# kangxiongbin/HyLight

Hardware: AMD Instinct MI355X
Metric: long-read all-vs-all overlaps/sec (higher is better)
Workload: dtype u8/int32

## Files before the change

hylight_amd/csrc/ava_align.hip:

```cpp
#include <algorithm>
#include <memory>
#include <type_traits>

#include "ava_internal.h"
#include "dev_prims.h"
#include "wave_ops.h"

namespace hlmi {

namespace {
constexpr int WG = 256;
constexpr int WAVES = WG / 64;
constexpr int SEQ_T_MAX = EXT_MAX + BAND_W;
constexpr int NR_SHORT = 128;
constexpr int WIDE_SHORT = 128;
inline dim3 grid1(size_t n) { return grid_for(n, WG); }

struct Task {
    uint32_t piece;
    uint16_t kind;
    uint16_t narrow;
    uint64_t qa, ta;
    int16_t m, n;
    int16_t dlo;
    int16_t trim;
};
constexpr uint16_t TASK_REV = 4;
constexpr uint16_t TASK_ONE = 8;
struct TaskOut {
    int32_t score;
    int32_t bi, bj;
    uint32_t runs_off, n_runs;
    uint32_t pad;
};
__device__ __forceinline__ uint32_t end_codes(uint32_t first_run, uint32_t last_run) { return (first_run & 15u) | (last_run & 15u) << 4; }

__global__ void piece_task_count_kernel(const Piece *pieces, size_t n, uint32_t *cnt) {
    size_t i = blockIdx.x * (size_t)blockDim.x + threadIdx.x;
    if (i < n) cnt[i] = pieces[i].n_fp + 1;
}

struct TaskRef { uint32_t pk, fp; };
struct PieceGeom {
    uint64_t qo, to;
    uint32_t ql, tl;
    uint32_t strand;
    uint32_t stub_cand;
};
struct TaskGeom {
    const TaskRef *ref;
    const PieceGeom *pg;
    const FixPt *fps;
};
__device__ __forceinline__ Task build_task(const PieceGeom &p, uint32_t piece, uint32_t kind, FixPt f0, FixPt f1, int ext_max) {
    const int ql = (int)p.ql, tl = (int)p.tl;
    const uint64_t qo = p.qo, to = p.to;
    const uint16_t rev = p.strand ? TASK_REV : 0;
    auto qaddr = [&](int pos) { return p.strand ? qo + (uint64_t)(ql - 1 - pos) : qo + (uint64_t)pos; };
    if (kind == 1) {
        const int qs = (int)f0.q, ts = (int)f0.t;
        const int m = qs < ext_max ? qs : ext_max, n2 = ts < m + BAND_W ? ts : m + BAND_W;
        return Task{piece, (uint16_t)(1u | rev), (uint16_t)(qs <= ext_max ? (qs + 1) << 1 : 0), qaddr(qs - 1),
                    to + (uint64_t)(ts - 1), (int16_t)m, (int16_t)n2, (int16_t)(-(BAND_W / 2 - 1)), 0};
    }
    if (kind == 2) {
        const int qe = (int)f0.q, te = (int)f0.t;
        const int m = ql - qe < ext_max ? ql - qe : ext_max, n2 = tl - te < m + BAND_W ? tl - te : m + BAND_W;
        return Task{piece, (uint16_t)(2u | rev), (uint16_t)(ql - qe <= ext_max ? (ql - qe + 1) << 1 : 0), qaddr(qe),
                    to + (uint64_t)te, (int16_t)m, (int16_t)n2, (int16_t)(-(BAND_W / 2 - 1)), 0};
    }
    const int q0 = (int)f0.q, t0 = (int)f0.t, m = (int)f1.q - q0, n2 = (int)f1.t - t0;
    const int delta = n2 - m, ad = delta < 0 ? -delta : delta;
    const bool lng = m > BLOCK_MAX || n2 > BLOCK_MAX;
    const bool narrow = !lng && ad <= NARROW_DELTA;
    const int lw = ad <= HALF_DELTA ? HALF_W : BAND_W;
    return Task{piece, rev, (uint16_t)(narrow ? 1 : 0), qaddr(q0), to + (uint64_t)t0, (int16_t)m, (int16_t)n2,
                (int16_t)((delta < 0 ? delta : 0) - (narrow ? NARROW_PAD : lng ? (lw - 1 - ad) / 2 : BAND_PAD)), 0};
}
__global__ __launch_bounds__(WG) void task_ref_kernel(const Piece *pieces, const uint32_t *task_off, size_t n, const uint32_t *qlen,
                                                       const uint32_t *tlen, const uint64_t *qoff, const uint64_t *toff,
                                                       const FixPt *fps, int stub_oh, int ext_max, TaskRef *task_ref, PieceGeom *pg) {
    const int lane = threadIdx.x & 63;
    const size_t wave = (blockIdx.x * (size_t)blockDim.x + threadIdx.x) >> 6;
    const size_t n_waves = ((size_t)gridDim.x * blockDim.x) >> 6;
    for (size_t i = wave; i < n; i += n_waves) {
        const Piece p = pieces[i];
        const uint32_t n_tasks = p.n_fp + 1;
        TaskRef *out = task_ref + task_off[i];
        for (uint32_t k = (uint32_t)lane; k < n_tasks; k += 64) {
            const uint32_t kind = k == 0 ? 1u : (k == p.n_fp ? 2u : 0u);
            out[k] = TaskRef{(uint32_t)i | kind << 30, p.fp_off + (k == 0 ? 0u : k - 1)};
        }
        if (lane == 0) {
            const uint32_t ql = qlen[p.q], tl = tlen[p.t];
            uint32_t cand = 0;
            if (stub_oh >= 0) {
                const FixPt a = fps[p.fp_off], b = fps[p.fp_off + p.n_fp - 1];
                const uint32_t dq = (uint32_t)(ext_max + stub_oh), dt = (uint32_t)(ext_max + BAND_W + stub_oh);
                cand = ((a.q > dq && a.t > dt) || (ql - b.q > dq && tl - b.t > dt)) ? 1u : 0u;
            }
            pg[i] = PieceGeom{qoff[p.q], toff[p.t], ql, tl, p.strand, cand};
        }
    }
}

__global__ __launch_bounds__(WG) void task_ref_lane_kernel(const Piece *pieces, const uint32_t *task_off, size_t n, const uint32_t *qlen,
                                                            const uint32_t *tlen, const uint64_t *qoff, const uint64_t *toff,
                                                            const FixPt *fps, int stub_oh, int ext_max, TaskRef *task_ref, PieceGeom *pg) {
    const size_t i = blockIdx.x * (size_t)blockDim.x + threadIdx.x;
    if (i >= n) return;
    const Piece p = pieces[i];
    const uint32_t n_tasks = p.n_fp + 1;
    TaskRef *out = task_ref + task_off[i];
    for (uint32_t k = 0; k < n_tasks; ++k) {
        const uint32_t kind = k == 0 ? 1u : (k == p.n_fp ? 2u : 0u);
        out[k] = TaskRef{(uint32_t)i | kind << 30, p.fp_off + (k == 0 ? 0u : k - 1)};
    }
    const uint32_t ql = qlen[p.q], tl = tlen[p.t];
    uint32_t cand = 0;
    if (stub_oh >= 0) {
        const FixPt a = fps[p.fp_off], b = fps[p.fp_off + p.n_fp - 1];
        const uint32_t dq = (uint32_t)(ext_max + stub_oh), dt = (uint32_t)(ext_max + BAND_W + stub_oh);
        cand = ((a.q > dq && a.t > dt) || (ql - b.q > dq && tl - b.t > dt)) ? 1u : 0u;
    }
    pg[i] = PieceGeom{qoff[p.q], toff[p.t], ql, tl, p.strand, cand};
}

struct AlignArgs {
    Task *tasks;
    TaskGeom geom;
    size_t n_tasks;
    const uint32_t *list;
    size_t n_list;
    const uint8_t *qcodes, *tcodes;
    long long q_total, t_total;
    const uint8_t *qpacked, *tpacked;
    const uint32_t *qnflag, *tnflag;
    int match, mismatch, go, ge, ambi;
    int go2, ge2;
    int end_bonus;
    int ext_max;
    int ext_all_long;
    int ungapped;
    int kmax;
    int kgap1;
    int kgap2;
    int one_ok;
    int kext_plain;
    int kext_bonus;
    int trim_ok;
    int kshift;
    TaskOut *out;
    uint32_t *runs;
    uint32_t cap_runs;
    uint32_t *counters;
    uint32_t run_buf_cap;
    uint8_t *cls_bare;
    uint8_t *defer_flag;
    const uint32_t *defer_list, *defer_count;
};

__device__ __forceinline__ uint32_t wave_excl_sum_u32(uint32_t v, int lane, uint32_t &total) {
    (void)lane;
    const uint32_t x = wave_prefix_sum_incl_dpp(v);
    total = (uint32_t)__builtin_amdgcn_readlane((int)x, 63);
    return x - v;
}

constexpr uint32_t RUN_CHUNK = 4096;
constexpr uint32_t RUN_CHUNK_SMALL = 256;
__device__ __forceinline__ uint32_t pool_take(const AlignArgs &a, uint32_t n, uint32_t &chunk_off, uint32_t &chunk_left,
                                              bool &ok, uint32_t chunk = RUN_CHUNK) {
    if (n > chunk_left) {
        const uint32_t want = n > chunk ? n : chunk;
        chunk_off = atomicAdd(&a.counters[0], want);
        chunk_left = want;
        if ((unsigned long long)chunk_off + want > a.cap_runs) { a.counters[1] = 1; chunk_left = 0; ok = false; return 0; }
    }
    const uint32_t off = chunk_off;
    chunk_off += n;
    chunk_left -= n;
    return off;
}

__device__ __forceinline__ uint32_t load_codes4(const uint8_t *base, long long idx, long long total) {
    if (idx >= 0 && idx + 4 <= total) {
        uint32_t v;
        __builtin_memcpy(&v, base + idx, 4);
        return v;
    }
    uint32_t v = 0;
    for (int k = 0; k < 4; ++k) v |= (uint32_t)(idx + k >= 0 && idx + k < total ? base[idx + k] : 4) << (8 * k);
    return v;
}
__device__ __forceinline__ uint32_t comp_codes4(uint32_t x) {
    const uint32_t n = x & 0x04040404u;
    return (x ^ 0x03030303u) & ~((n >> 1) | (n >> 2));
}
__device__ __forceinline__ uint32_t load_window4(const uint8_t *codes, long long total, long long a0, bool down, bool comp, int x) {
    uint32_t v = down ? __builtin_bswap32(load_codes4(codes, a0 - x - 3, total)) : load_codes4(codes, a0 + x, total);
    if (comp) v = comp_codes4(v);
    return v;
}

__device__ __forceinline__ uint32_t load_window4p(const uint8_t *codes, long long a0, bool down, bool comp, int x) {
    uint32_t v;
    __builtin_memcpy(&v, codes + (down ? a0 - x - 3 : a0 + x), 4);
    if (down) v = __builtin_bswap32(v);
    if (comp) v = comp_codes4(v);
    return v;
}


enum { ST_BASES = 0, ST_BASES_SQUARE, ST_BASES_NARROW, ST_BASES_WIDE, ST_FAST, ST_DP, ST_DP_ROWS, ST_NARROW_SMALL, ST_WIDE_ONE, ST_STUB_EXT, ST_EXT_CERT, ST_EXT_DP_ROW, ST_EXT_DP_K, ST_LONG, ST_BASES_LONG, ST_PACKED, N_ALIGN_STATS };
constexpr int NR_SMALL = 64;
constexpr uint8_t CLS_LONG = 5;
constexpr uint8_t CLS_LONG32 = 7;
constexpr uint8_t CLS_UNGAPPED = 6;

__device__ __forceinline__ uint64_t load_codes8(const uint8_t *base, long long idx, long long total) {
    if (idx >= 0 && idx + 8 <= total) {
        uint64_t v;
        __builtin_memcpy(&v, base + idx, 8);
        return v;
    }
    uint64_t v = 0;
    for (int k = 0; k < 8; ++k) v |= (uint64_t)(idx + k >= 0 && idx + k < total ? base[idx + k] : 4) << (8 * k);
    return v;
}
__device__ __forceinline__ uint64_t load_window8(const uint8_t *codes, long long total, long long a0, bool down, bool comp, int x) {
    uint64_t v = down ? __builtin_bswap64(load_codes8(codes, a0 - x - 7, total)) : load_codes8(codes, a0 + x, total);
    if (comp) {
        const uint64_t n = v & 0x0404040404040404ull;
        v = (v ^ 0x0303030303030303ull) & ~((n >> 1) | (n >> 2));
    }
    return v;
}

__device__ __forceinline__ uint64_t load_window8p(const uint8_t *codes, long long a0, bool down, bool comp, int x) {
    uint64_t v;
    __builtin_memcpy(&v, codes + (down ? a0 - x - 7 : a0 + x), 8);
    if (down) v = __builtin_bswap64(v);
    if (comp) {
        const uint64_t n = v & 0x0404040404040404ull;
        v = (v ^ 0x0303030303030303ull) & ~((n >> 1) | (n >> 2));
    }
    return v;
}

__device__ __forceinline__ uint64_t load_window32p(const uint8_t *packed, long long a0, bool down, bool comp, int x) {
    const long long s = down ? a0 - x - 31 : a0 + x;
    const uint8_t *p = packed + (s >> 2);
    uint64_t lo;
    __builtin_memcpy(&lo, p, 8);
    const int sh = 2 * (int)(s & 3);
    uint64_t v = lo >> sh | (uint64_t)p[8] << 1 << (63 - sh);
    if (down) {
        v = __builtin_bitreverse64(v);
        v = (v >> 1 & 0x5555555555555555ull) | (v & 0x5555555555555555ull) << 1;
    }
    return comp ? ~v : v;
}
__device__ __forceinline__ uint32_t ne_bits32(uint64_t q, uint64_t t) {
    const uint64_t d = q ^ t;
    auto even = [](uint32_t x) {
        x = (x | x >> 1) & 0x55555555u;
        x = (x | x >> 1) & 0x33333333u;
        x = (x | x >> 2) & 0x0f0f0f0fu;
        x = (x | x >> 4) & 0x00ff00ffu;
        return (x | x >> 8) & 0xffffu;
    };
    return even((uint32_t)d) | even((uint32_t)(d >> 32)) << 16;
}
__device__ __forceinline__ uint32_t squeeze8(uint64_t f) {
    return (((uint32_t)f * 0x10204080u) >> 28) | (((uint32_t)(f >> 32) * 0x10204080u) >> 28) << 4;
}
__device__ __forceinline__ uint32_t ne_bits8(uint64_t q, uint64_t t) {
    const uint64_t d = q ^ t;
    return squeeze8((d | d >> 1 | d >> 2) & 0x0101010101010101ull);
}
__device__ __forceinline__ uint32_t amb_bits8(uint64_t q, uint64_t t) { return squeeze8((q | t) >> 2 & 0x0101010101010101ull); }
__device__ __forceinline__ bool range_flagged(const uint32_t *nflag, long long lo, long long hi) {
    const uint32_t g0 = (uint32_t)((lo + (long long)DevReads::PAD) >> 5), g1 = (uint32_t)((hi + (long long)DevReads::PAD) >> 5);
    uint32_t any = 0;
    for (uint32_t w = g0 >> 5; w <= g1 >> 5; ++w) {
        uint32_t keep = ~0u;
        if (w == g0 >> 5) keep &= ~0u << (g0 & 31);
        if (w == g1 >> 5) keep &= ~0u >> (31 - (g1 & 31));
        any |= nflag[w] & keep;
    }
    return any != 0;
}
__device__ __forceinline__ bool window_flagged(const uint32_t *nflag, long long a0, bool down, int len) {
    return down ? range_flagged(nflag, a0 - (len - 1), a0) : range_flagged(nflag, a0, a0 + (len - 1));
}

template <int PASS>
__global__ __launch_bounds__(WG) __attribute__((amdgpu_waves_per_eu(PASS == 1 ? 4 : 5))) void classify_kernel(AlignArgs a, uint8_t *cls, unsigned long long *stats) {
    __shared__ unsigned long long s_stat[WAVES][N_ALIGN_STATS];
    constexpr int CMP_WORDS = PASS == 1 ? 64 * (BLOCK_MAX / 32) : 1;
    __shared__ uint32_t s_mm[WAVES][CMP_WORDS], s_up[WAVES][CMP_WORDS], s_dn[WAVES][CMP_WORDS];
    __shared__ uint64_t s_qa[WAVES][PASS == 1 ? 64 : 1], s_ta[WAVES][PASS == 1 ? 64 : 1];
    __shared__ uint32_t s_geo[WAVES][PASS == 1 ? 64 : 1], s_amb[WAVES][2];
    const int lane = threadIdx.x & 63;
    const size_t tid = blockIdx.x * (size_t)blockDim.x + threadIdx.x;
    const size_t n_thr = (size_t)gridDim.x * blockDim.x;
    uint32_t chunk_off = 0, chunk_left = 0;
    uint32_t st[N_ALIGN_STATS] = {};
    const size_t n_units = PASS == 1 ? a.n_tasks : (size_t)*a.defer_count;
    const size_t rounds = (n_units + n_thr - 1) / n_thr;
    TaskRef ref_n{0, 0};
    uint32_t ti_n = 0;
    if (PASS == 1) { if (tid < n_units) ref_n = a.geom.ref[tid]; }
    else if (tid < n_units) ti_n = a.defer_list[tid];
    for (size_t r = 0; r < rounds; ++r) {
        const size_t u = r * n_thr + tid;
        bool live = u < n_units;
        const size_t ti = PASS == 1 || !live ? u : (size_t)ti_n;
        TaskRef ref = ref_n;
        if (PASS == 2 && live) ref = a.geom.ref[ti];
        {
            const size_t un = u + n_thr;
            if (PASS == 1) { if (un < n_units) ref_n = a.geom.ref[un]; }
            else if (un < n_units) ti_n = a.defer_list[un];
        }
        Task tk{};
        bool held = false;
        bool bare = false;
        if (live) {
            const uint32_t pc = ref.pk & 0x3fffffffu, kind = ref.pk >> 30;
            const PieceGeom pg = a.geom.pg[pc];
            held = PASS == 1 && kind != 0 && pg.stub_cand != 0;
            bare = a.cls_bare != nullptr && pg.stub_cand != 0;
            const FixPt f0 = a.geom.fps[ref.fp];
            FixPt f1{0, 0};
            if (kind == 0) f1 = a.geom.fps[ref.fp + 1];
            tk = build_task(pg, pc, kind, f0, f1, a.ext_max);
        }
        const int m = tk.m, n = tk.n;
        uint8_t c = 2;
        bool try_fast = false;
        if (live) {
            if (m <= 0 || n <= 0 || held) c = 0;
            else if ((tk.kind & 3) == 0) {
                if (m > BLOCK_MAX || n > BLOCK_MAX)
                    c = (n > m ? n - m : m - n) <= HALF_DELTA ? CLS_LONG32 : CLS_LONG;
                else { c = tk.narrow ? (m <= NR_SHORT ? 1 : 3) : 2; try_fast = (m == n); }
            } else if ((m < n - tk.dlo ? m : n - tk.dlo) > EXT_MAX) { c = CLS_LONG32; tk.dlo = (int16_t)(-(HALF_W / 2 - 1)); }
            else if (a.ext_all_long) c = CLS_LONG;
            if (c == 2 && (m < n - tk.dlo ? m : n - tk.dlo) <= WIDE_SHORT) c = 4;
        }
        if (PASS == 1 && live) {
            const bool defer = c != 0 && a.kmax >= 0 && ((tk.kind & 3) != 0 || (m != n && c != CLS_LONG && c != CLS_LONG32));
            a.defer_flag[ti] = defer ? 1 : 0;
            if (defer) { live = false; try_fast = false; }
        }
        int k = 0, mpos[3] = {0, 0, 0}, last_x = -1;
        bool ambig = false, shift_ok = false;
        if constexpr (PASS == 1) {
            const int wv = threadIdx.x >> 6;
            bool flagged = false;
            if (try_fast && a.qpacked)
                flagged = window_flagged(a.qnflag, (long long)tk.qa, (tk.kind & TASK_REV) != 0, m) || window_flagged(a.tnflag, (long long)tk.ta, false, m);
            const bool use_packed = a.qpacked != nullptr && __ballot(flagged) == 0;
            uint32_t *mm = s_mm[wv], *mup = s_up[wv], *mdn = s_dn[wv];
            const uint32_t nch = try_fast ? (uint32_t)(m + 31) >> 5 : 0u;
            const uint32_t incl = wave_prefix_sum_incl_dpp(nch), tot = (uint32_t)__builtin_amdgcn_readlane((int)incl, 63);
            const uint32_t st0 = incl - nch;
            if (lane < 2) s_amb[wv][lane] = 0;
            s_qa[wv][lane] = tk.qa; s_ta[wv][lane] = tk.ta;
            auto compare = [&](auto packed_form) {
                constexpr bool PK = decltype(packed_form)::value;
                constexpr int PB = PK ? 32 : 8, PW = 32 / PB;
                constexpr uint32_t FIRST = PK ? 3u : 0xffu;
                using piece_t = std::conditional_t<PK, uint32_t, uint8_t>;
                piece_t *own = (piece_t *)mm, *pm = (piece_t *)mm, *pup = (piece_t *)mup, *pdn = (piece_t *)mdn;
                const uint32_t ptot = tot * PW, pst0 = st0 * PW;
                auto window = [&](bool query, int o, bool rv, int x) {
                    if constexpr (PK) return query ? load_window32p(a.qpacked, (long long)s_qa[wv][o], rv, rv, x) : load_window32p(a.tpacked, (long long)s_ta[wv][o], false, false, x);
                    else return query ? load_window8p(a.qcodes, (long long)s_qa[wv][o], rv, rv, x) : load_window8p(a.tcodes, (long long)s_ta[wv][o], false, false, x);
                };
                for (uint32_t c = (uint32_t)lane; c < ptot; c += 64) own[c] = 0;
                s_geo[wv][lane] = pst0 | (uint32_t)m << 16 | ((tk.kind & TASK_REV) ? 0x80000000u : 0u);
                __builtin_amdgcn_s_waitcnt(0xc07f);
                __builtin_amdgcn_wave_barrier();
                if (nch) own[pst0] = (piece_t)lane;
                __builtin_amdgcn_s_waitcnt(0xc07f);
                __builtin_amdgcn_wave_barrier();
                int carry = 0;
                constexpr int CU = 4;
                for (uint32_t c0 = 0; c0 < ptot; c0 += 64 * CU) {
                    int ow[CU], xs[CU], left[CU];
                    bool rv[CU];
#pragma unroll
                    for (int u = 0; u < CU; ++u) {
                        const uint32_t c = c0 + 64u * u + (uint32_t)lane;
                        int o = c < ptot ? (int)own[c] : 0;
                        o = wave_prefix_max_incl_dpp(o);
                        o = o > carry ? o : carry;
                        carry = __builtin_amdgcn_readlane(o, 63);
                        const uint32_t geo = s_geo[wv][o];
                        ow[u] = o;
                        xs[u] = (int)(c - (geo & 0xffffu)) * PB;
                        left[u] = c < ptot ? (int)(geo >> 16 & 0x7fffu) - xs[u] : 0;
                        rv[u] = (geo >> 31) != 0;
                    }
                    uint64_t qw[CU], tw[CU];
                    uint32_t q_end = 0, t_end = 0;
#pragma unroll
                    for (int u = 0; u < CU; ++u) {
                        qw[u] = tw[u] = 0;
                        if (left[u] > 0) {
                            qw[u] = window(true, ow[u], rv[u], xs[u]);
                            tw[u] = window(false, ow[u], false, xs[u]);
                            if (u == CU - 1 && lane == 63 && a.kshift) {
                                q_end = (uint32_t)window(true, ow[u], rv[u], xs[u] + PB) & FIRST;
                                t_end = (uint32_t)window(false, ow[u], false, xs[u] + PB) & FIRST;
                            }
                        }
                    }
                    int nq[CU], nt[CU];
                    if (a.kshift) {
#pragma unroll
                        for (int u = 0; u < CU; ++u) {
                            const int q_after = u + 1 < CU ? __builtin_amdgcn_readlane((int)((uint32_t)qw[u + 1 < CU ? u + 1 : u] & FIRST), 0) : (int)q_end;
                            const int t_after = u + 1 < CU ? __builtin_amdgcn_readlane((int)((uint32_t)tw[u + 1 < CU ? u + 1 : u] & FIRST), 0) : (int)t_end;
                            nq[u] = wave_shl1((int)((uint32_t)qw[u] & FIRST), q_after);
                            nt[u] = wave_shl1((int)((uint32_t)tw[u] & FIRST), t_after);
                        }
                    }
#pragma unroll
                    for (int u = 0; u < CU; ++u) {
                        if (left[u] <= 0) continue;
                        const uint32_t c = c0 + 64u * u + (uint32_t)lane;
                        if constexpr (PK) {
                            pm[c] = ne_bits32(qw[u], tw[u]) & (left[u] >= 32 ? ~0u : (1u << left[u]) - 1u);
                            if (a.kshift) {
                                const uint64_t q9 = qw[u] >> 2 | (uint64_t)(uint32_t)nq[u] << 62, t9 = tw[u] >> 2 | (uint64_t)(uint32_t)nt[u] << 62;
                                pup[c] = ne_bits32(q9, tw[u]);
                                pdn[c] = ne_bits32(qw[u], t9);
                            }
                        } else {
                            const uint64_t keep = left[u] >= 8 ? ~0ull : (1ull << (8 * left[u])) - 1ull;
                            if ((qw[u] | tw[u]) & keep & 0x0404040404040404ull) atomicOr(&s_amb[wv][ow[u] >> 5], 1u << (ow[u] & 31));
                            pm[c] = (uint8_t)ne_bits8(qw[u] & keep, tw[u] & keep);
                            if (a.kshift) {
                                const uint64_t q9 = qw[u] >> 8 | (uint64_t)(uint32_t)nq[u] << 56, t9 = tw[u] >> 8 | (uint64_t)(uint32_t)nt[u] << 56;
                                pup[c] = (uint8_t)ne_bits8(q9, tw[u]);
                                pdn[c] = (uint8_t)ne_bits8(qw[u], t9);
                            }
                        }
                    }
                }
            };
            if (use_packed) { compare(std::true_type{}); if (try_fast) ++st[ST_PACKED]; }
            else compare(std::false_type{});
            __builtin_amdgcn_s_waitcnt(0xc07f);
            __builtin_amdgcn_wave_barrier();
            if (try_fast) {
                ambig = (s_amb[wv][lane >> 5] >> (lane & 31)) & 1u;
                for (uint32_t j = 0; j < nch && k <= a.kmax + a.kshift; ++j) {
                    uint32_t bits = mm[st0 + j];
                    while (bits) {
                        const int y = __ffs((int)bits) - 1;
                        bits &= bits - 1;
                        if (k < 3) mpos[k] = (int)(32 * j) + y;
                        ++k;
                    }
                }
            }
            if (try_fast && !ambig && a.kshift && k == a.kmax + 1) {
                const int p1 = mpos[0], pk = mpos[k - 1];
                uint32_t any_up = 0, any_dn = 0;
                for (int j = p1 >> 5; j <= (pk - 1) >> 5; ++j) {
                    uint32_t keepb = ~0u;
                    if (j == p1 >> 5) keepb &= ~0u << (p1 & 31);
                    if (j == (pk - 1) >> 5) keepb &= ~0u >> (31 - ((pk - 1) & 31));
                    any_up |= mup[st0 + (uint32_t)j] & keepb;
                    any_dn |= mdn[st0 + (uint32_t)j] & keepb;
                }
                shift_ok = any_up != 0 && any_dn != 0;
            }
            if (try_fast && k > 0 && !ambig) {
                for (int j = (int)nch - 1; j >= 0; --j) {
                    const uint32_t bits = mm[st0 + (uint32_t)j];
                    if (bits) { last_x = 32 * j + 31 - __clz((int)bits); break; }
                }
            }
            __builtin_amdgcn_wave_barrier();
        }
        bool fast = try_fast && !ambig && k <= a.kmax;
        if (shift_ok) fast = true;
        uint32_t runs[7];
        uint32_t nr = 0;
        int fast_score = a.match * (m - k) - a.mismatch * k;
        uint32_t ext_flag = 0;
        int ext_take = -1;
        auto pairs = [&](auto packed_form, bool q_down, bool t_down, int xq, int xt, uint32_t &ne, uint32_t &amb) {
            const bool rev = (tk.kind & TASK_REV) != 0;
            if constexpr (decltype(packed_form)::value) {
                ne = ne_bits32(load_window32p(a.qpacked, (long long)tk.qa, q_down, rev, xq), load_window32p(a.tpacked, (long long)tk.ta, t_down, false, xt));
                amb = 0;
            } else {
                const uint64_t q8 = load_window8p(a.qcodes, (long long)tk.qa, q_down, rev, xq), t8 = load_window8p(a.tcodes, (long long)tk.ta, t_down, false, xt);
                ne = ne_bits8(q8, t8);
                amb = amb_bits8(q8, t8);
            }
        };
        auto low_bits = [](int n, int w) { return n >= w ? ~0u >> (32 - w) : (1u << n) - 1u; };
        if (PASS == 2 && live && c != 0 && (tk.kind & 3) != 0 && a.kmax >= 0) {
            const bool rev = (tk.kind & TASK_REV) != 0, left = (tk.kind & 3) == 1;
            const int L = m < n ? m : n;
            const int end_row = (int)(tk.narrow >> 1) - 1;
            const bool bonus_row = a.end_bonus != 0 && end_row >= 0 && end_row <= n + (BAND_W / 2 - 1);
            bool same = !bonus_row || L == end_row;
            int allow = -1, k_ext = 0;
            bool amb_ext = false;
            if (a.go2 > 0 && a.ge > a.ge2 && a.end_bonus == 0 && a.one_ok) {
                int g = (a.go2 - a.go + (a.ge - a.ge2) - 1) / (a.ge - a.ge2);
                g = g < 1 ? 1 : g;
                allow = (a.go2 + a.ge2 * g - 1) / (a.match + a.mismatch);
            }
            const int k_want = bonus_row ? (L == end_row ? a.kext_bonus : 0) : a.kext_plain;
            int x1 = -1, x2 = -1;
            auto more = [&]() { return same || (!amb_ext && (k_ext <= allow || k_ext <= k_want)); };
            auto scan = [&](auto packed_form) {
                constexpr int W = decltype(packed_form)::value ? 32 : 8;
                auto take = [&](int x, uint32_t ne, uint32_t amb) {
                    const uint32_t keep = low_bits(L - x, W);
                    ne &= keep;
                    amb_ext |= (amb & keep) != 0;
                    if (ne && x2 < 0) {
                        const int y1 = __ffs((int)ne) - 1;
                        if (x1 < 0) { x1 = x + y1; const uint32_t d2 = ne & (ne - 1); if (d2) x2 = x + __ffs((int)d2) - 1; }
                        else x2 = x + y1;
                    }
                    k_ext += __popc(ne);
                    same = same && ne == 0 && !amb_ext;
                };
                for (int x = 0; x < L && more(); x += 2 * W) {
                    uint32_t ne0, amb0, ne1 = 0, amb1 = 0;
                    pairs(packed_form, left != rev, left, x, x, ne0, amb0);
                    if (x + W < L) pairs(packed_form, left != rev, left, x + W, x + W, ne1, amb1);
                    take(x, ne0, amb0);
                    if (x + W < L && more()) take(x + W, ne1, amb1);
                }
            };
            if (a.qpacked && !window_flagged(a.qnflag, (long long)tk.qa, left != rev, L) && !window_flagged(a.tnflag, (long long)tk.ta, left, L)) { scan(std::true_type{}); ++st[ST_PACKED]; }
            else scan(std::false_type{});
            if (!same && !amb_ext && k_ext <= allow) { tk.kind |= TASK_ONE; ++st[ST_WIDE_ONE]; }
            if (same) {
                runs[nr++] = (uint32_t)L << 4 | OP_EQ;
                fast_score = a.match * L;
                ext_flag = L == end_row ? 0x80000000u : 0u;
                fast = true;
                c = 0;
            } else if (!amb_ext && k_ext >= 1 && k_ext <= k_want) {
                int take = L;
                if (!bonus_row && a.match * x1 >= a.match * (L - 1) - a.mismatch) take = x1;
                const int subs = take == L ? k_ext : 0;
                int prev = 0;
                if (take > 0) {
                    if (subs >= 1) {
                        if (x1 > 0) runs[nr++] = (uint32_t)x1 << 4 | OP_EQ;
                        if (subs == 2 && x2 == x1 + 1) { runs[nr++] = 2u << 4 | OP_X; prev = x2 + 1; }
                        else {
                            runs[nr++] = 1u << 4 | OP_X; prev = x1 + 1;
                            if (subs == 2) {
                                runs[nr++] = (uint32_t)(x2 - prev) << 4 | OP_EQ;
                                runs[nr++] = 1u << 4 | OP_X; prev = x2 + 1;
                            }
                        }
                    }
                    if (take > prev) runs[nr++] = (uint32_t)(take - prev) << 4 | OP_EQ;
                }
                if (left) for (uint32_t i = 0; i < nr / 2; ++i) { const uint32_t v = runs[i]; runs[i] = runs[nr - 1 - i]; runs[nr - 1 - i] = v; }
                fast_score = a.match * (take - subs) - a.mismatch * subs;
                ext_flag = bonus_row && take == end_row ? 0x80000000u : 0u;
                ext_take = take;
                fast = true;
                c = 0;
                ++st[ST_EXT_CERT];
            } else if (bonus_row && L != end_row) ++st[ST_EXT_DP_ROW];
            else ++st[ST_EXT_DP_K];
        } else if (PASS == 2 && live && c != 0 && (tk.kind & 3) == 0 && m != n && a.kmax >= 0) {
            const bool rev = (tk.kind & TASK_REV) != 0;
            const int mn = m < n ? m : n, gap = n > m ? n - m : m - n;
            const bool del = n > m;
            const int want = a.kgap1 && gap == 1 ? (a.kgap2 ? 3 : 2) : 1;
            int found_a = 0, found_b = 0, a1 = mn, a2 = mn, a3 = mn, b1 = -1, b2 = -1, b3 = -1;
            bool amb = false;
            const int sq = m > n ? m - n : 0, st_ = n > m ? n - m : 0;
            auto scan = [&](auto packed_form) {
                constexpr int W = decltype(packed_form)::value ? 32 : 8;
                for (int x = 0; x < mn && (found_a < want || found_b < want); x += W) {
                    const bool da = found_a < want, db = found_b < want;
                    const int e0 = mn - W - x;
                    uint32_t ne_a = 0, amb_a = 0, ne_b = 0, amb_b = 0;
                    if (da) pairs(packed_form, rev, false, x, x, ne_a, amb_a);
                    if (db) pairs(packed_form, rev, false, e0 + sq, e0 + st_, ne_b, amb_b);
                    const int left = mn - x;
                    if (da) {
                        const uint32_t keep = low_bits(left, W);
                        amb |= (amb_a & keep) != 0;
                        uint32_t d = ne_a & keep;
                        while (d && found_a < want) {
                            const int y = __ffs((int)d) - 1;
                            d &= d - 1;
                            if (found_a == 0) a1 = x + y; else if (found_a == 1) a2 = x + y; else a3 = x + y;
                            ++found_a;
                        }
                    }
                    if (db) {
                        const uint32_t keep = left >= W ? ~0u : low_bits(W, W) & ~low_bits(W - left, W);
                        amb |= (amb_b & keep) != 0;
                        uint32_t d = ne_b & keep;
                        while (d && found_b < want) {
                            const int z = 31 - __clz((int)d);
                            d &= ~(1u << z);
                            if (found_b == 0) b1 = e0 + z; else if (found_b == 1) b2 = e0 + z; else b3 = e0 + z;
                            ++found_b;
                        }
                    }
                }
            };
            const bool use_packed = a.qpacked && !window_flagged(a.qnflag, (long long)tk.qa, rev, m) && !window_flagged(a.tnflag, (long long)tk.ta, false, n);
            if (use_packed) { scan(std::true_type{}); ++st[ST_PACKED]; }
            else scan(std::false_type{});
            int p_star = -1, xpos = -1, xpos2 = -1;
            if (!amb) {
                if (b1 < a1) p_star = b1 + 1;
                else if (want >= 2 && b2 < a1) { p_star = b2 + 1; xpos = b1; }
                else if (want >= 2 && b1 < a2) { p_star = b1 + 1; xpos = a1; }
            }
            if (p_star < 0 && !amb && want == 3) {
                int ps = -1, x1 = -1, x2 = -1;
                const int mab = a1 < b2 ? a1 : b2, Mab = a1 > b2 ? a1 : b2, m2 = a2 < b1 ? a2 : b1, M2 = a2 > b1 ? a2 : b1;
                if (b2 >= 0 && b3 < mab) { ps = b3 + 1; x1 = b2; x2 = b1; }
                else if (a1 < mn && b1 >= 0 && Mab < m2) { ps = Mab + 1; x1 = a1; x2 = b1; }
                else if (a2 < mn && M2 < a3) { ps = M2 + 1; x1 = a1; x2 = a2; }
                if (ps >= 0 && a1 < b1) {
                    bool far_ne = false, near_ne = false, ambx = false;
                    auto shifted = [&](auto packed_form) {
                        constexpr int W = decltype(packed_form)::value ? 32 : 8;
                        uint32_t ne, ab;
                        for (int x = a1; x < b1 && !far_ne; x += W) {
                            pairs(packed_form, rev, false, del ? x : x + 2, del ? x + 2 : x, ne, ab);
                            const uint32_t keep = low_bits(b1 - x, W);
                            ambx |= (ab & keep) != 0;
                            far_ne = (ne & keep) != 0;
                        }
                        for (int x = a1 + 1; x <= b1 && !near_ne; x += W) {
                            pairs(packed_form, rev, false, del ? x : x - 1, del ? x - 1 : x, ne, ab);
                            const uint32_t keep = low_bits(b1 + 1 - x, W);
                            ambx |= (ab & keep) != 0;
                            near_ne = (ne & keep) != 0;
                        }
                    };
                    if (use_packed) shifted(std::true_type{});
                    else shifted(std::false_type{});
                    if (far_ne && near_ne && !ambx) { p_star = ps; xpos = x1; xpos2 = x2; }
                }
            }
            if (p_star < 0 && !amb && b1 >= 0) last_x = b1;
            if (p_star >= 0) {
                auto seg = [&](int from, int to) {
                    int prev = from;
                    for (int k = 0; k < 2; ++k) {
                        const int xp = k ? xpos2 : xpos;
                        if (xp < from || xp >= to) continue;
                        if (xp > prev) runs[nr++] = (uint32_t)(xp - prev) << 4 | OP_EQ;
                        if (nr && xp == prev && prev > from && (runs[nr - 1] & 15u) == OP_X) runs[nr - 1] += 1u << 4;
                        else runs[nr++] = 1u << 4 | OP_X;
                        prev = xp + 1;
                    }
                    if (to > prev) runs[nr++] = (uint32_t)(to - prev) << 4 | OP_EQ;
                };
                seg(0, p_star);
                runs[nr++] = (uint32_t)gap << 4 | (del ? OP_D : OP_I);
                seg(p_star, mn);
                const int subs = (xpos >= 0 ? 1 : 0) + (xpos2 >= 0 ? 1 : 0);
                int gap_cost = a.go + a.ge * gap;
                if (a.go2 && a.go2 + a.ge2 * gap < gap_cost) gap_cost = a.go2 + a.ge2 * gap;
                fast_score = a.match * (mn - subs) - a.mismatch * subs - gap_cost;
                fast = true;
                c = 0;
            }
        } else if (fast) {
            c = 0;
            int prev = 0, xs = -1, xe = -1;
            for (int i = 0; i < k; ++i) {
                const int x = mpos[i];
                if (x == xe) { xe = x + 1; continue; }
                if (xs >= 0) { runs[nr++] = (uint32_t)(xe - xs) << 4 | OP_X; prev = xe; }
                if (x > prev) runs[nr++] = (uint32_t)(x - prev) << 4 | OP_EQ;
                xs = x; xe = x + 1;
            }
            if (xs >= 0) { runs[nr++] = (uint32_t)(xe - xs) << 4 | OP_X; prev = xe; }
            if (m > prev) runs[nr++] = (uint32_t)(m - prev) << 4 | OP_EQ;
        }
        if (bare) nr = 0;
        uint32_t wave_total;
        const uint32_t mine = wave_excl_sum_u32(nr, lane, wave_total);
        uint32_t base = 0;
        bool ok = true;
        if (wave_total) {
            if (lane == 0) base = pool_take(a, wave_total, chunk_off, chunk_left, ok);
            base = (uint32_t)__shfl((int)base, 0, 64);
            ok = __shfl((int)ok, 0, 64) != 0;
        }
        if (fast) {
            if (ok) for (uint32_t q = 0; q < nr; ++q) a.runs[base + mine + q] = runs[q];
            const bool ext = (tk.kind & 3) != 0;
            const int L = ext_take >= 0 ? ext_take : (m < n ? m : n);
            a.out[ti] = TaskOut{fast_score, ext ? L : m, ext ? L : n, base + mine, ok ? nr : 0, (nr ? end_codes(runs[0], runs[nr - 1]) : 0u) | ext_flag};
        } else if (live && c == 0) {
            a.out[ti] = TaskOut{0, 0, 0, 0, 0, 0};
        }
        int m_dp = m;
        if (live && !fast && (c == 1 || c == 3) && a.kmax >= 0 && last_x >= 0 && a.trim_ok && !a.ungapped) {
            const int mn = m < n ? m : n;
            int T = mn - 1 - last_x;
            T = T < mn - 1 ? T : mn - 1;
            if (T > 0) {
                tk.m = (int16_t)(m - T); tk.n = (int16_t)(n - T); tk.trim = (int16_t)T;
                m_dp = m - T;
                c = m_dp <= NR_SHORT ? 1 : 3;
            }
        }
        if (live) {
            if (a.ungapped && c != 0) c = CLS_UNGAPPED;
            cls[ti] = bare ? 0 : c;
            if (a.cls_bare) a.cls_bare[ti] = bare ? c : 0;
            if (c != 0) a.tasks[ti] = tk;
            if (held) ++st[ST_STUB_EXT];
            else if (m > 0 && n > 0) {
                const uint32_t bases = (uint32_t)(m + n);
                st[ST_BASES] += bases;
                if ((tk.kind & 3) == 0 && m == n) st[ST_BASES_SQUARE] += bases;
                if (c == 0) ++st[ST_FAST];
                else {
                    ++st[ST_DP];
                    if (c == CLS_LONG || c == CLS_LONG32) { ++st[ST_LONG]; st[ST_BASES_LONG] += bases; st[ST_DP_ROWS] += (uint32_t)(m < n - tk.dlo ? m : n - tk.dlo); }
                    else if (c == 2 || c == 4) { st[ST_BASES_WIDE] += bases; st[ST_DP_ROWS] += (uint32_t)(m < n - tk.dlo ? m : n - tk.dlo); }
                    else { st[ST_BASES_NARROW] += bases; st[ST_DP_ROWS] += (uint32_t)m_dp; if (c == 1 && m_dp < NR_SMALL && !bare) ++st[ST_NARROW_SMALL]; }
                }
            }
        }
    }
#pragma unroll
    for (int k = 0; k < N_ALIGN_STATS; ++k) {
        unsigned long long v = st[k];
#pragma unroll
        for (int o = 32; o > 0; o >>= 1) v += __shfl_xor(v, o, 64);
        if (lane == 0) s_stat[threadIdx.x >> 6][k] = v;
    }
    __syncthreads();
    if (threadIdx.x < N_ALIGN_STATS) {
        unsigned long long v = 0;
        for (int w = 0; w < WAVES; ++w) v += s_stat[w][threadIdx.x];
        if (v) atomicAdd(&stats[threadIdx.x], v);
    }
}

__global__ void task_rows_key_kernel(const Task *tasks, const uint32_t *list, size_t n, uint32_t *key) {
    size_t i = blockIdx.x * (size_t)blockDim.x + threadIdx.x;
    if (i < n) key[i] = (uint32_t)tasks[list[i]].m >> 2;
}


__global__ void task_rows_desc_key_kernel(const Task *tasks, const uint32_t *list, size_t n, uint32_t *key) {
    size_t i = blockIdx.x * (size_t)blockDim.x + threadIdx.x;
    if (i >= n) return;
    const Task &t = tasks[list[i]];
    const int rows = (int)t.m < (int)t.n - (int)t.dlo ? (int)t.m : (int)t.n - (int)t.dlo;
    key[i] = 0xffffu - (uint32_t)(rows < 0 ? 0 : rows);
}

constexpr int DP_BIAS = 1 << 24;
constexpr int NT_PAD = 16;
constexpr int NT_EXTRA = NT_PAD + NARROW_DELTA + NARROW_W + 7;
enum { PL_DIAG = 0, PL_EGEF, PL_EEXT, PL_FEXT, PL_NE, N_PLANES };

__device__ __forceinline__ uint32_t shift_in(uint32_t acc, bool bit) {
#if defined(__HIP_DEVICE_COMPILE__)
    const unsigned long long m = __ballot(bit);
    unsigned long long co;
    asm("v_addc_co_u32 %0, %1, %2, %2, %3" : "=v"(acc), "=s"(co) : "v"(acc), "s"(m));
#endif
    return acc;
}

struct NarrowWalk {
    const uint32_t *pl;
    int chunks;
    int lb;
    int m, n, dlo;
    int wmask;
    bool keep_order;
    int trim;
    __device__ __forceinline__ uint32_t word(int plane, int c, int lane) const { return pl[(plane * chunks + c) * 64 + lane]; }
};
struct WalkScore {
    int match, mismatch, go, ge;
    int total;
};
__device__ uint32_t narrow_walk(const NarrowWalk &w, uint32_t *out, uint32_t total, uint32_t *buf = nullptr, uint32_t cap = 0,
                                WalkScore *ws = nullptr, uint32_t *ends = nullptr) {
    int i = w.m, j = w.n, state = 0;
    uint32_t cur_op = OP_EQ, cur_len = (uint32_t)w.trim, n_runs = 0, e_first = 0, e_last = 0;
    auto put = [&]() {
        if (!n_runs) e_first = cur_op;
        e_last = cur_op;
        if (out) out[w.keep_order ? n_runs : total - 1 - n_runs] = cur_len << 4 | cur_op;
        else if (n_runs < cap) buf[n_runs] = cur_len << 4 | cur_op;
        ++n_runs;
        if (ws) ws->total += cur_op == OP_EQ ? ws->match * (int)cur_len
                           : (cur_op == OP_X ? -ws->mismatch * (int)cur_len : -(ws->go + ws->ge * (int)cur_len));
    };
    for (int it = 0; (i > 0 || j > 0) && it < 4 * (EXT_MAX + SEQ_T_MAX); ++it) {
        uint32_t op, len;
        if (i == 0) {
            op = OP_D; len = (uint32_t)j; j = 0;
        } else {
            const int d = w.lb + ((j - i - w.dlo) & w.wmask);
            const int c = (i - 1) >> 5, sh = 31 - ((i - 1) & 31);
            const uint32_t dg = w.word(PL_DIAG, c, d) >> sh;
            const uint32_t ne = w.word(PL_NE, c, d) >> sh;
            const uint32_t eg = w.word(PL_EGEF, c, d) >> sh;
            const uint32_t ee = w.word(PL_EEXT, c, (d - 1) & 63) >> sh;
            const int i2 = i > 1 ? i - 2 : 0;
            const uint32_t fe = w.word(PL_FEXT, i2 >> 5, (d + 1) & 63) >> (31 - (i2 & 31));
            const int st = state != 0 ? state : ((dg & 1u) ? 0 : ((eg & 1u) ? 1 : 2));
            if (st == 0) {
                const uint32_t inv = ~dg;
                const int r = inv ? __ffs((int)inv) - 1 : 32;
                const bool isx = (ne & 1u) != 0;
                const uint32_t flip = isx ? ~ne : ne;
                int l = flip ? __ffs((int)flip) - 1 : 32;
                l = l < r ? l : r;
                op = isx ? OP_X : OP_EQ; len = (uint32_t)l;
                i -= l; j -= l;
                state = 0;
            } else if (st == 1) {
                op = OP_D; len = 1;
                state = (ee & 1u) ? 1 : 0;
                --j;
            } else {
                op = OP_I; len = 1;
                state = (i > 1 && (fe & 1u)) ? 2 : 0;
                --i;
            }
        }
        if (op == cur_op) cur_len += len;
        else { if (cur_len) put(); cur_op = op; cur_len = len; }
    }
    if (cur_len) put();
    if (ends) *ends = w.keep_order ? end_codes(e_first, e_last) : end_codes(e_last, e_first);
    return n_runs;
}
constexpr int RUN_BUF_NARROW = 48, RUN_BUF_WIDE = 128;

template <bool AMBI, int NR_CHUNKS>
__device__ __forceinline__ void narrow_rows(const AlignArgs &a, int rows, int m, int dlo, int l, const uint8_t *sq,
                                            const uint8_t *st, uint32_t (*pl)[NR_CHUNKS][64], int lane, int &Hend) {
    const int go = a.go, ge = a.ge, goe = go + ge, gel = ge * l, goel = go + ge * l;
    const int j0 = dlo + l;
    int H = j0 == 0 ? DP_BIAS : (j0 > 0 ? DP_BIAS - (go + ge * j0) : 0);
    int G = H - goe;
    uint32_t a0 = 0, a1 = 0, a2 = 0, a3 = 0, a4 = 0;
    const uint8_t *tp = st + NT_PAD + dlo + l - 1;
    int v_match = a.match, v_mis = -a.mismatch;
    asm volatile("" : "+v"(v_match), "+v"(v_mis));
    auto row = [&](int i, int qa, int t2) {
        const bool ne = qa != t2;
        int s = ne ? v_mis : v_match;
        if (AMBI) s = (qa | t2) > 3 ? -a.ambi : s;
        const int mm = H + s;
        const int f = row_shl1_z(G);
        const int ht = mm > f ? mm : f;
        const int e = row_shr1(row_prefix_max_incl_dpp(ht + gel), 0) - goel;
        const int h = ht > e ? ht : e;
        const int fo = h - goe, fe = f - ge;
        a0 = shift_in(a0, mm == h);
        a1 = shift_in(a1, e >= f);
        a2 = shift_in(a2, e + go > h);
        a3 = shift_in(a3, fe > fo);
        a4 = shift_in(a4, ne);
        G = fo > fe ? fo : fe;
        H = h;
        if (i == m) Hend = h;
    };
    int qa = sq[0], t2 = tp[1];
    int i = 1;
    for (; i < rows; i += 2) {
        const int qb = sq[i], tb = tp[i + 1], qc = sq[i + 1], tc = tp[i + 2];
        row(i, qa, t2);
        row(i + 1, qb, tb);
        qa = qc; t2 = tc;
        if (((i + 1) & 31) == 0) {
            const int c = ((i + 1) >> 5) - 1;
            pl[PL_DIAG][c][lane] = a0; pl[PL_EGEF][c][lane] = a1; pl[PL_EEXT][c][lane] = a2; pl[PL_FEXT][c][lane] = a3;
            pl[PL_NE][c][lane] = a4;
        }
    }
    if (i == rows) row(i, qa, t2);
    if (rows & 31) {
        const int c = rows >> 5, up = 32 - (rows & 31);
        pl[PL_DIAG][c][lane] = a0 << up; pl[PL_EGEF][c][lane] = a1 << up; pl[PL_EEXT][c][lane] = a2 << up;
        pl[PL_FEXT][c][lane] = a3 << up; pl[PL_NE][c][lane] = a4 << up;
    }
}

template <int NR_MAX>
__global__ __launch_bounds__(WG) void align_narrow_kernel(AlignArgs a) {
    constexpr int NR_CHUNKS = NR_MAX / 32, NQ_STEPS = NR_MAX / 64, NT_STEPS = NR_MAX / 64 + 1;
    __shared__ uint32_t s_pl[WAVES][N_PLANES][NR_CHUNKS][64];
    __shared__ __attribute__((aligned(4))) uint8_t s_q[WAVES * 4][NR_MAX + 4];
    __shared__ __attribute__((aligned(4))) uint8_t s_t[WAVES * 4][NR_MAX + NT_EXTRA];
    __shared__ uint32_t s_runs[WAVES * 4][RUN_BUF_NARROW];
    const int lane = threadIdx.x & 63, g = lane >> 4, l = lane & 15, wv = threadIdx.x >> 6;
    const size_t wave = (blockIdx.x * (size_t)blockDim.x + threadIdx.x) >> 6;
    const size_t n_waves = ((size_t)gridDim.x * blockDim.x) >> 6;
    uint32_t (*pl)[NR_CHUNKS][64] = s_pl[wv];
    uint8_t *sq = s_q[wv * 4 + g], *st = s_t[wv * 4 + g];
    uint32_t chunk_off = 0, chunk_left = 0;
    const size_t n_quads = (a.n_list + 3) / 4;
    for (size_t qd = wave; qd < n_quads; qd += n_waves) {
        const size_t li = qd * 4 + g;
        const bool live = li < a.n_list;
        size_t ti = 0;
        Task tk{};
        if (live) { ti = a.list[li]; tk = a.tasks[ti]; }
        const int m = tk.m, n = tk.n, dlo = tk.dlo;
        bool ambig = false;
        if (live) {
            const bool rev = (tk.kind & TASK_REV) != 0;
            uint32_t vq[NQ_STEPS], vt[NT_STEPS];
#pragma unroll
            for (int r = 0; r < NQ_STEPS; ++r) {
                const int x = 4 * (l + 16 * r);
                vq[r] = 0;
                if (x < m) vq[r] = load_window4p(a.qcodes, (long long)tk.qa, rev, rev, x);
            }
#pragma unroll
            for (int r = 0; r < NT_STEPS; ++r) {
                const int x = 4 * (l + 16 * r);
                vt[r] = 0;
                if (x < n) vt[r] = load_window4p(a.tcodes, (long long)tk.ta, false, false, x);
            }
#pragma unroll
            for (int r = 0; r < NQ_STEPS; ++r) {
                const int x = 4 * (l + 16 * r);
                if (x < m) { *(uint32_t *)(sq + x) = vq[r]; ambig |= (vq[r] & 0x04040404u) != 0; }
            }
#pragma unroll
            for (int r = 0; r < NT_STEPS; ++r) {
                const int x = 4 * (l + 16 * r);
                if (x < n) { *(uint32_t *)(st + NT_PAD + x) = vt[r]; ambig |= (vt[r] & 0x04040404u) != 0; }
            }
        }
        __builtin_amdgcn_s_waitcnt(0);
        __builtin_amdgcn_wave_barrier();
        const int rows = (int)wave_max_u32_dpp(live ? (uint32_t)m : 0u);
        int Hend = 0;
        if (__any(ambig)) narrow_rows<true, NR_CHUNKS>(a, rows, m, dlo, l, sq, st, pl, lane, Hend);
        else narrow_rows<false, NR_CHUNKS>(a, rows, m, dlo, l, sq, st, pl, lane, Hend);
        const int score = __shfl(Hend, g * 16 + ((n - m - dlo) & (NARROW_W - 1)), 64) - DP_BIAS + a.match * tk.trim;
        __builtin_amdgcn_s_waitcnt(0);
        __builtin_amdgcn_wave_barrier();
        uint32_t *rbuf = s_runs[wv * 4 + g];
        const uint32_t rcap = a.run_buf_cap < (uint32_t)RUN_BUF_NARROW ? a.run_buf_cap : (uint32_t)RUN_BUF_NARROW;
        uint32_t cp_n = 0, cp_off = 0;
        if (live && l == 0) {
            const NarrowWalk w{&pl[0][0][0], NR_CHUNKS, g * 16, m, n, dlo, NARROW_W - 1, false, tk.trim};
            uint32_t ends = 0;
            const uint32_t n_runs = narrow_walk(w, nullptr, 0, rbuf, rcap, nullptr, &ends);
            uint32_t off = 0;
            bool ok = true;
            if (n_runs) off = pool_take(a, n_runs, chunk_off, chunk_left, ok, RUN_CHUNK_SMALL);
            if (ok && n_runs) {
                if (n_runs <= rcap) { cp_n = n_runs; cp_off = off; }
                else narrow_walk(w, a.runs + off, n_runs);
            }
            a.out[ti] = TaskOut{score, m, n, off, ok ? n_runs : 0, ends};
        }
        __builtin_amdgcn_s_waitcnt(0);
        __builtin_amdgcn_wave_barrier();
        cp_n = (uint32_t)__shfl((int)cp_n, g * 16, 64); cp_off = (uint32_t)__shfl((int)cp_off, g * 16, 64);
        for (uint32_t k = (uint32_t)l; k < cp_n; k += 16) a.runs[cp_off + k] = rbuf[cp_n - 1 - k];
        __builtin_amdgcn_wave_barrier();
    }
}

typedef short s2 __attribute__((ext_vector_type(2)));
__device__ __forceinline__ s2 s2_of(int x) { return __builtin_bit_cast(s2, x); }
__device__ __forceinline__ int int_of(s2 x) { return __builtin_bit_cast(int, x); }
__device__ __forceinline__ s2 splat2(int v) { return s2{(short)v, (short)v}; }
__device__ __forceinline__ s2 max2(s2 a, s2 b) { return __builtin_elementwise_max(a, b); }
__device__ __forceinline__ s2 pk_min_u16(s2 x, s2 y) {
    s2 r = x;
#if defined(__HIP_DEVICE_COMPILE__)
    asm("v_pk_min_u16 %0, %1, %2" : "=v"(r) : "v"(x), "v"(y));
#endif
    return r;
}
__device__ __forceinline__ s2 pk_mad_i16(s2 x, s2 y, s2 z) {
    s2 r = x;
#if defined(__HIP_DEVICE_COMPILE__)
    asm("v_pk_mad_i16 %0, %1, %2, %3" : "=v"(r) : "v"(x), "v"(y), "v"(z));
#endif
    return r;
}
template <int CTRL>
__device__ __forceinline__ int dpp_z(int x) { return __builtin_amdgcn_mov_dpp(x, CTRL, 0xf, 0xf, true); }
constexpr int DP_BIAS16 = 1 << 13;
constexpr int PK_T0 = 12;

template <bool AMBI, int NR_CHUNKS, bool TB = true>
__device__ __forceinline__ void narrow_rows_pk(const AlignArgs &a, int rows, int mA, int mB, int dloA, int dloB, int l,
                                               const uint16_t *sq2, const uint16_t *st2, uint32_t (*plA)[NR_CHUNKS][64],
                                               uint32_t (*plB)[NR_CHUNKS][64], int lane, int &HendA, int &HendB) {
    const int go = a.go, ge = a.ge, goe = go + ge;
    const s2 v_goe = splat2(goe), v_ge = splat2(ge), v_go = splat2(go), v_gel = splat2(ge * l), v_goel = splat2(go + ge * l);
    auto h0 = [&](int j0) { return j0 == 0 ? DP_BIAS16 : (j0 > 0 ? DP_BIAS16 - (go + ge * j0) : 0); };
    s2 H = s2{(short)h0(dloA + l), (short)h0(dloB + l)};
    s2 G = H - v_goe;
    uint32_t a0A = 0, a1A = 0, a2A = 0, a3A = 0, a4A = 0, a0B = 0, a1B = 0, a2B = 0, a3B = 0, a4B = 0;
    const uint16_t *tp = st2 + PK_T0 + l - 1;
    s2 v_match = splat2(a.match), v_dm = splat2(-(a.match + a.mismatch)), v_one = splat2(1);
    const s2 v_ambi = splat2(a.ambi);
    asm volatile("" : "+v"(v_match), "+v"(v_dm), "+v"(v_one));
    auto row = [&](int i, int qb, int tb) {
        const s2 x = s2_of((int)__builtin_amdgcn_perm(0u, (uint32_t)(qb ^ tb), 0x0c010c00u));
        s2 s = pk_mad_i16(pk_min_u16(x, v_one), v_dm, v_match);
        if (AMBI) {
            const s2 amb01 = s2_of((int)__builtin_amdgcn_perm(0u, (uint32_t)(((qb | tb) >> 2) & 0x0101), 0x0c010c00u));
            s = s - amb01 * (s + v_ambi);
        }
        const s2 mm = H + s;
        const s2 f = s2_of(dpp_z<0x101>(int_of(G)));
        const s2 ht = max2(mm, f);
        s2 p = ht + v_gel;
        p = max2(p, s2_of(dpp_z<0x111>(int_of(p))));
        p = max2(p, s2_of(dpp_z<0x112>(int_of(p))));
        p = max2(p, s2_of(dpp_z<0x114>(int_of(p))));
        p = max2(p, s2_of(dpp_z<0x118>(int_of(p))));
        const s2 e = s2_of(dpp_z<0x111>(int_of(p))) - v_goel;
        const s2 h = max2(ht, e);
        const s2 fo = h - v_goe, fe = f - v_ge, eo = e + v_go;
        if (TB) {
            a0A = shift_in(a0A, mm.x == h.x);   a0B = shift_in(a0B, mm.y == h.y);
            a1A = shift_in(a1A, e.x >= f.x);    a1B = shift_in(a1B, e.y >= f.y);
            a2A = shift_in(a2A, eo.x > h.x);    a2B = shift_in(a2B, eo.y > h.y);
            a3A = shift_in(a3A, fe.x > fo.x);   a3B = shift_in(a3B, fe.y > fo.y);
            a4A = shift_in(a4A, x.x != 0);      a4B = shift_in(a4B, x.y != 0);
        }
        G = max2(fo, fe);
        H = h;
        if (AMBI || !TB) { if (i == mA) HendA = h.x; if (i == mB) HendB = h.y; }
    };
    auto flush = [&](int c, int up) {
        if (!TB) return;
        plA[PL_DIAG][c][lane] = a0A << up; plA[PL_EGEF][c][lane] = a1A << up; plA[PL_EEXT][c][lane] = a2A << up;
        plA[PL_FEXT][c][lane] = a3A << up; plA[PL_NE][c][lane] = a4A << up;
        plB[PL_DIAG][c][lane] = a0B << up; plB[PL_EGEF][c][lane] = a1B << up; plB[PL_EEXT][c][lane] = a2B << up;
        plB[PL_FEXT][c][lane] = a3B << up; plB[PL_NE][c][lane] = a4B << up;
    };
    int qa = sq2[0], ta = tp[1];
    int i = 1;
    for (; i < rows; i += 2) {
        const int qb = sq2[i], tb = tp[i + 1], qc = sq2[i + 1], tc = tp[i + 2];
        row(i, qa, ta);
        row(i + 1, qb, tb);
        qa = qc; ta = tc;
        if (((i + 1) & 31) == 0) flush(((i + 1) >> 5) - 1, 0);
    }
    if (i == rows) row(i, qa, ta);
    if (rows & 31) flush(rows >> 5, 32 - (rows & 31));
}

constexpr int PK_WAVES = 1;
template <int NR_MAX, bool TB = true>
__global__ __launch_bounds__(64 * PK_WAVES) void align_narrow_pk_kernel(AlignArgs a) {
    constexpr int NR_CHUNKS = TB ? NR_MAX / 32 : 1, NQ_STEPS = NR_MAX / 64, NT_STEPS = NR_MAX / 64 + 1;
    constexpr int T2_LEN = NR_MAX + PK_T0 + NARROW_W + NARROW_DELTA + 12;
    constexpr int Q2_LEN = NR_MAX + 4, RUN_BUF = NR_MAX >= 128 ? RUN_BUF_NARROW : 40;
    constexpr int SEQ_WORDS = 4 * (Q2_LEN + T2_LEN + 1) / 2 + 2;
    static_assert(8 * RUN_BUF <= SEQ_WORDS, "run buffers do not fit the sequence area");
    __shared__ uint32_t s_pl[PK_WAVES][2][N_PLANES][NR_CHUNKS][64];
    __shared__ uint32_t s_seq[PK_WAVES][SEQ_WORDS];
    const int lane = threadIdx.x & 63, g = lane >> 4, l = lane & 15, wv = threadIdx.x >> 6;
    uint16_t *const q2 = (uint16_t *)s_seq[wv] + g * Q2_LEN, *const t2 = (uint16_t *)s_seq[wv] + 4 * Q2_LEN + g * T2_LEN;
    uint32_t (*const s_runs)[RUN_BUF] = (uint32_t (*)[RUN_BUF])s_seq[wv];
    const size_t wave = (blockIdx.x * (size_t)blockDim.x + threadIdx.x) >> 6;
    const size_t n_waves = ((size_t)gridDim.x * blockDim.x) >> 6;
    uint32_t chunk_off = 0, chunk_left = 0;
    const size_t n_octs = (a.n_list + 7) / 8;
    uint8_t *q2b = (uint8_t *)q2, *t2b = (uint8_t *)t2;
    for (size_t oc = wave; oc < n_octs; oc += n_waves) {
        const size_t liA = oc * 8 + (size_t)g * 2, liB = liA + 1;
        const bool liveA = liA < a.n_list, liveB = liB < a.n_list;
        size_t tiA = 0, tiB = 0;
        Task tA{}, tB{};
        if (liveA) { tiA = a.list[liA]; tA = a.tasks[tiA]; }
        if (liveB) { tiB = a.list[liB]; tB = a.tasks[tiB]; }
        bool ambig = false;
        auto stage = [&](const Task &t, int hf) {
            const bool rev = (t.kind & TASK_REV) != 0;
            uint32_t vq[NQ_STEPS], vt[NT_STEPS];
#pragma unroll
            for (int r = 0; r < NQ_STEPS; ++r) {
                const int x = 4 * (l + 16 * r);
                vq[r] = 0;
                if (x < t.m) vq[r] = load_window4p(a.qcodes, (long long)t.qa, rev, rev, x);
            }
#pragma unroll
            for (int r = 0; r < NT_STEPS; ++r) {
                const int x = 4 * (l + 16 * r);
                vt[r] = 0;
                if (x < t.n) vt[r] = load_window4p(a.tcodes, (long long)t.ta, false, false, x);
            }
#pragma unroll
            for (int r = 0; r < NQ_STEPS; ++r) {
                const int x = 4 * (l + 16 * r);
                if (x < t.m) {
#pragma unroll
                    for (int k = 0; k < 4; ++k) q2b[2 * (x + k) + hf] = (uint8_t)(vq[r] >> (8 * k));
                    ambig |= (vq[r] & 0x04040404u) != 0;
                }
            }
            const int t0 = PK_T0 - t.dlo;
#pragma unroll
            for (int r = 0; r < NT_STEPS; ++r) {
                const int x = 4 * (l + 16 * r);
                if (x < t.n) {
#pragma unroll
                    for (int k = 0; k < 4; ++k) t2b[2 * (t0 + x + k) + hf] = (uint8_t)(vt[r] >> (8 * k));
                    ambig |= (vt[r] & 0x04040404u) != 0;
                }
            }
        };
        if (liveA) stage(tA, 0);
        if (liveB) stage(tB, 1);
        __builtin_amdgcn_s_waitcnt(0);
        __builtin_amdgcn_wave_barrier();
        const int mA = tA.m, mB = tB.m;
        const int rows = (int)wave_max_u32_dpp((uint32_t)(mA > mB ? mA : mB));
        int HendA = 0, HendB = 0;
        const bool amb = __any(ambig);
        if (amb) narrow_rows_pk<true, NR_CHUNKS, TB>(a, rows, mA, mB, tA.dlo, tB.dlo, l, q2, t2, s_pl[wv][0], s_pl[wv][1], lane, HendA, HendB);
        else narrow_rows_pk<false, NR_CHUNKS, TB>(a, rows, mA, mB, tA.dlo, tB.dlo, l, q2, t2, s_pl[wv][0], s_pl[wv][1], lane, HendA, HendB);
        const int endA = __shfl(HendA, g * 16 + ((tA.n - mA - tA.dlo) & (NARROW_W - 1)), 64) - DP_BIAS16;
        const int endB = __shfl(HendB, g * 16 + ((tB.n - mB - tB.dlo) & (NARROW_W - 1)), 64) - DP_BIAS16;
        __builtin_amdgcn_s_waitcnt(0);
        __builtin_amdgcn_wave_barrier();
        if constexpr (!TB) {
            const int hf = l & 1;
            if (l < 2 && (hf ? liveB : liveA)) {
                const Task &t = hf ? tB : tA;
                a.out[hf ? tiB : tiA] = TaskOut{(hf ? endB : endA) + a.match * t.trim, t.m, t.n, 0, 0, 0};
            }
            __builtin_amdgcn_wave_barrier();
            continue;
        }
        const int hf = l & 1;
        const bool walker = l < 2 && (hf ? liveB : liveA);
        const int wm = hf ? tB.m : tA.m, wn = hf ? tB.n : tA.n, wd = hf ? tB.dlo : tA.dlo, wtrim = hf ? tB.trim : tA.trim;
        uint32_t *rbuf = s_runs[g * 2 + hf];
        const uint32_t rcap = a.run_buf_cap < (uint32_t)RUN_BUF ? a.run_buf_cap : (uint32_t)RUN_BUF;
        uint32_t cp_n = 0, cp_off = 0;
        if (walker) {
            const NarrowWalk w{&s_pl[wv][0][0][0][0] + hf * (N_PLANES * NR_CHUNKS * 64), NR_CHUNKS, g * 16, wm, wn, wd, NARROW_W - 1, false, wtrim};
            WalkScore ws{a.match, a.mismatch, a.go, a.ge, 0};
            uint32_t ends = 0;
            const uint32_t n_runs = narrow_walk(w, nullptr, 0, rbuf, rcap, &ws, &ends);
            uint32_t off = 0;
            bool ok = true;
            if (n_runs) off = pool_take(a, n_runs, chunk_off, chunk_left, ok, RUN_CHUNK_SMALL);
            if (ok && n_runs) {
                if (n_runs <= rcap) { cp_n = n_runs; cp_off = off; }
                else narrow_walk(w, a.runs + off, n_runs);
            }
            const int score = amb ? (hf ? endB : endA) + a.match * wtrim : ws.total;
            a.out[hf ? tiB : tiA] = TaskOut{score, wm, wn, off, ok ? n_runs : 0, ends};
        }
        __builtin_amdgcn_s_waitcnt(0);
        __builtin_amdgcn_wave_barrier();
#pragma unroll
        for (int h2 = 0; h2 < 2; ++h2) {
            const uint32_t n2 = (uint32_t)__shfl((int)cp_n, g * 16 + h2, 64), o2 = (uint32_t)__shfl((int)cp_off, g * 16 + h2, 64);
            const uint32_t *rb = s_runs[g * 2 + h2];
            for (uint32_t k = (uint32_t)l; k < n2; k += 16) a.runs[o2 + k] = rb[n2 - 1 - k];
        }
        __builtin_amdgcn_s_waitcnt(0);
        __builtin_amdgcn_wave_barrier();
    }
}

constexpr int WT_PAD = 64;
constexpr int WT_LEN = WT_PAD + SEQ_T_MAX + 64;

enum { WP_DIAG = 0, WP_EGEF, WP_EP, WP_FP, WP_EX1, WP_EX2, WP_FX1, WP_FX2, WP_NE, N_WPLANES };

template <bool AMBI, bool EXT, bool TWO, int W_CHUNKS, bool TB = true>
__device__ __forceinline__ void wide_rows(const AlignArgs &a, int m, int n, int dlo, int lane, int end_row,
                                          const uint8_t *sq, const uint8_t *st, uint32_t (*pl)[W_CHUNKS][64], int &Hend,
                                          int &best_h, int &best_i) {
    const int go = a.go, ge = a.ge, goe = go + ge, gel = ge * lane, goel = go + ge * lane;
    const int go2 = a.go2, ge2 = a.ge2, goe2 = go2 + ge2, gel2 = ge2 * lane, goel2 = go2 + ge2 * lane;
    const int j0 = dlo + lane;
    int gap0 = go + ge * j0;
    if (TWO && go2 + ge2 * j0 < gap0) gap0 = go2 + ge2 * j0;
    int H = j0 == 0 ? DP_BIAS : (j0 > 0 ? DP_BIAS - gap0 : 0);
    int G = H - goe, G2 = TWO ? H - goe2 : 0;
    uint32_t a0 = 0, a1 = 0, a2 = 0, a3 = 0, a4 = 0, b0 = 0, b1 = 0, b2 = 0, b3 = 0;
    int v_match = a.match, v_mis = -a.mismatch;
    asm volatile("" : "+v"(v_match), "+v"(v_mis));
    const uint8_t *tp = st + WT_PAD + dlo + lane - 1;
    const int imin = -j0, span = n - j0 - imin;
    best_h = 0; best_i = 0;
    if (EXT && j0 >= 0 && j0 <= n) best_h = H;
    int qa = sq[0], t2 = tp[1];
    for (int i = 1; i <= m; ++i) {
        const int qa_next = sq[i], t2_next = tp[i + 1];
        const bool ne = qa != t2;
        int s = ne ? v_mis : v_match;
        if (AMBI) s = (qa | t2) > 3 ? -a.ambi : s;
        const int mm = H + s;
        const int f1 = wave_shl1_z(G);
        const int f2 = TWO ? wave_shl1_z(G2) : 0;
        const int f = TWO && f2 > f1 ? f2 : f1;
        const int ht = mm > f ? mm : f;
        const int e1 = wave_shr1(wave_prefix_max_incl_dpp(ht + gel), 0) - goel;
        const int e2 = TWO ? wave_shr1(wave_prefix_max_incl_dpp(ht + gel2), 0) - goel2 : 0;
        const int e = TWO && e2 > e1 ? e2 : e1;
        const int h = ht > e ? ht : e;
        const int fo = h - goe, fe = f1 - ge;
        if (TB) {
            a0 = shift_in(a0, mm == h);
            a1 = shift_in(a1, e >= f);
            a2 = shift_in(a2, e1 + go > h);
            a3 = shift_in(a3, fe > fo);
            a4 = shift_in(a4, ne);
        }
        G = fo > fe ? fo : fe;
        if (TWO) {
            const int fo2 = h - goe2, fe2 = f2 - ge2;
            if (TB) {
                b0 = shift_in(b0, e2 > e1);
                b1 = shift_in(b1, f2 > f1);
                b2 = shift_in(b2, e2 + go2 > h);
                b3 = shift_in(b3, fe2 > fo2);
            }
            G2 = fo2 > fe2 ? fo2 : fe2;
        }
        H = h;
        qa = qa_next; t2 = t2_next;
        if (EXT) {
            const int hb = h + (i == end_row ? a.end_bonus : 0);
            if ((uint32_t)(i - imin) <= (uint32_t)span && span >= 0 && hb > best_h) { best_h = hb; best_i = i; }
        }
        if (TB && (i & 31) == 0) {
            const int c = (i >> 5) - 1;
            pl[WP_DIAG][c][lane] = a0; pl[WP_EGEF][c][lane] = a1; pl[WP_EX1][c][lane] = a2; pl[WP_FX1][c][lane] = a3;
            pl[WP_NE][c][lane] = a4;
            if (TWO) { pl[WP_EP][c][lane] = b0; pl[WP_FP][c][lane] = b1; pl[WP_EX2][c][lane] = b2; pl[WP_FX2][c][lane] = b3; }
        }
    }
    Hend = H;
    if (TB && (m & 31)) {
        const int c = m >> 5, up = 32 - (m & 31);
        pl[WP_DIAG][c][lane] = a0 << up; pl[WP_EGEF][c][lane] = a1 << up; pl[WP_EX1][c][lane] = a2 << up;
        pl[WP_FX1][c][lane] = a3 << up; pl[WP_NE][c][lane] = a4 << up;
        if (TWO) { pl[WP_EP][c][lane] = b0 << up; pl[WP_FP][c][lane] = b1 << up; pl[WP_EX2][c][lane] = b2 << up; pl[WP_FX2][c][lane] = b3 << up; }
    }
}

template <bool TWO>
__device__ uint32_t wide_walk(const uint32_t *pl, int chunks, int m0, int n0, int dlo, bool keep_order, uint32_t *out, uint32_t total,
                              uint32_t *buf, uint32_t cap, uint32_t *ends = nullptr, int max_it = 4 * (EXT_MAX + SEQ_T_MAX)) {
    auto word = [&](int plane, int c, int lane) { return pl[(plane * chunks + c) * 64 + lane]; };
    int i = m0, j = n0, state = 0;
    uint32_t cur_op = 0, cur_len = 0, n_runs = 0, e_first = 0, e_last = 0;
    auto put = [&]() {
        if (!n_runs) e_first = cur_op;
        e_last = cur_op;
        if (out) out[keep_order ? n_runs : total - 1 - n_runs] = cur_len << 4 | cur_op;
        else if (n_runs < cap) buf[n_runs] = cur_len << 4 | cur_op;
        ++n_runs;
    };
    for (int it = 0; (i > 0 || j > 0) && it < max_it; ++it) {
        uint32_t op, len;
        if (i == 0) {
            op = OP_D; len = (uint32_t)j; j = 0;
        } else {
            const int d = (j - i - dlo) & (BAND_W - 1);
            const int c = (i - 1) >> 5, sh = 31 - ((i - 1) & 31);
            const int i2 = i > 1 ? i - 2 : 0, c2 = i2 >> 5, sh2 = 31 - (i2 & 31);
            int st = state;
            if (st == 0) {
                const uint32_t dg = word(WP_DIAG, c, d) >> sh;
                if (dg & 1u) st = 0;
                else if ((word(WP_EGEF, c, d) >> sh) & 1u) st = TWO && ((word(WP_EP, c, d) >> sh) & 1u) ? 3 : 1;
                else st = TWO && ((word(WP_FP, c, d) >> sh) & 1u) ? 4 : 2;
                if (st == 0) {
                    const uint32_t ne = word(WP_NE, c, d) >> sh;
                    const uint32_t inv = ~dg;
                    const int r = inv ? __ffs((int)inv) - 1 : 32;
                    const bool isx = (ne & 1u) != 0;
                    const uint32_t flip = isx ? ~ne : ne;
                    int l = flip ? __ffs((int)flip) - 1 : 32;
                    l = l < r ? l : r;
                    op = isx ? OP_X : OP_EQ; len = (uint32_t)l;
                    i -= l; j -= l;
                    state = 0;
                    if (op == cur_op) cur_len += len;
                    else { if (cur_len) put(); cur_op = op; cur_len = len; }
                    continue;
                }
            }
            if (st == 1 || st == 3) {
                const uint32_t ex = word(st == 1 ? WP_EX1 : WP_EX2, c, (d - 1) & 63) >> sh;
                op = OP_D; len = 1;
                state = (ex & 1u) ? st : 0;
                --j;
            } else {
                const uint32_t fx = word(st == 2 ? WP_FX1 : WP_FX2, c2, (d + 1) & 63) >> sh2;
                op = OP_I; len = 1;
                state = (i > 1 && (fx & 1u)) ? st : 0;
                --i;
            }
        }
        if (op == cur_op) cur_len += len;
        else { if (cur_len) put(); cur_op = op; cur_len = len; }
    }
    if (cur_len) put();
    if (ends) *ends = keep_order ? end_codes(e_first, e_last) : end_codes(e_last, e_first);
    return n_runs;
}

template <bool TWO, int W = BAND_W>
__device__ uint32_t long_walk(const uint32_t *pl, int chunks, int m0, int n0, int dlo, bool keep_order, uint32_t *buf, uint32_t cap,
                              uint32_t *ends, int max_it) {
    auto word = [&](int plane, int c, int lane) { return pl[((size_t)plane * chunks + c) * W + lane]; };
    int i = m0, j = n0, state = 0;
    uint32_t cur_op = 0, cur_len = 0, n_runs = 0, e_first = 0, e_last = 0;
    auto put = [&]() {
        if (!n_runs) e_first = cur_op;
        e_last = cur_op;
        if (n_runs < cap) buf[n_runs] = cur_len << 4 | cur_op;
        ++n_runs;
    };
    for (int it = 0; (i > 0 || j > 0) && it < max_it; ++it) {
        uint32_t op, len;
        if (i == 0) {
            op = OP_D; len = (uint32_t)j; j = 0;
        } else {
            const int d = (j - i - dlo) & (W - 1);
            const int c = (i - 1) >> 5, sh = 31 - ((i - 1) & 31);
            const int i2 = i > 1 ? i - 2 : 0, c2 = i2 >> 5, sh2 = 31 - (i2 & 31);
            const int dl = (d - 1) & (W - 1), dr = (d + 1) & (W - 1);
            const uint32_t w_dg = word(WP_DIAG, c, d), w_ne = word(WP_NE, c, d), w_eg = word(WP_EGEF, c, d);
            const uint32_t w_ep = TWO ? word(WP_EP, c, d) : 0u, w_fp = TWO ? word(WP_FP, c, d) : 0u;
            const uint32_t w_ex1 = word(WP_EX1, c, dl), w_ex2 = TWO ? word(WP_EX2, c, dl) : 0u;
            const uint32_t w_fx1 = word(WP_FX1, c2, dr), w_fx2 = TWO ? word(WP_FX2, c2, dr) : 0u;
            int st = state;
            if (st == 0) {
                const uint32_t dg = w_dg >> sh;
                if (dg & 1u) st = 0;
                else if ((w_eg >> sh) & 1u) st = TWO && ((w_ep >> sh) & 1u) ? 3 : 1;
                else st = TWO && ((w_fp >> sh) & 1u) ? 4 : 2;
                if (st == 0) {
                    const uint32_t ne = w_ne >> sh;
                    const uint32_t inv = ~dg;
                    const int r = inv ? __ffs((int)inv) - 1 : 32;
                    const bool isx = (ne & 1u) != 0;
                    const uint32_t flip = isx ? ~ne : ne;
                    int l = flip ? __ffs((int)flip) - 1 : 32;
                    l = l < r ? l : r;
                    op = isx ? OP_X : OP_EQ; len = (uint32_t)l;
                    i -= l; j -= l;
                    state = 0;
                    if (op == cur_op) cur_len += len;
                    else { if (cur_len) put(); cur_op = op; cur_len = len; }
                    continue;
                }
            }
            if (st == 1 || st == 3) {
                const uint32_t ex = (st == 1 ? w_ex1 : w_ex2) >> sh;
                op = OP_D; len = 1;
                state = (ex & 1u) ? st : 0;
                --j;
            } else {
                const uint32_t fx = (st == 2 ? w_fx1 : w_fx2) >> sh2;
                op = OP_I; len = 1;
                state = (i > 1 && (fx & 1u)) ? st : 0;
                --i;
            }
        }
        if (op == cur_op) cur_len += len;
        else { if (cur_len) put(); cur_op = op; cur_len = len; }
    }
    if (cur_len) put();
    if (ends) *ends = keep_order ? end_codes(e_first, e_last) : end_codes(e_last, e_first);
    return n_runs;
}

template <int ROWS_MAX, bool TB = true>
__global__ __launch_bounds__(WG) __attribute__((amdgpu_waves_per_eu(TB && ROWS_MAX <= 128 ? 4 : 1, 8))) void align_kernel(AlignArgs a) {
    constexpr int RUN_BUF = TB && ROWS_MAX <= 128 ? 96 : RUN_BUF_WIDE;
    constexpr int W_CHUNKS = TB ? ROWS_MAX / 32 : 1;
    __shared__ uint32_t s_pl[WAVES][TB ? N_WPLANES : 1][W_CHUNKS][64];
    __shared__ __attribute__((aligned(4))) uint8_t s_q[WAVES][ROWS_MAX + 4];
    __shared__ __attribute__((aligned(4))) uint8_t s_t[WAVES][WT_LEN];
    __shared__ uint32_t s_runs[WAVES][RUN_BUF];
    const int lane = threadIdx.x & 63, wv = threadIdx.x >> 6;
    const size_t wave = (blockIdx.x * (size_t)blockDim.x + threadIdx.x) >> 6;
    const size_t n_waves = ((size_t)gridDim.x * blockDim.x) >> 6;
    uint32_t (*pl)[W_CHUNKS][64] = s_pl[wv];
    uint8_t *sq = s_q[wv], *st = s_t[wv];
    uint32_t chunk_off = 0, chunk_left = 0;
    for (size_t li = wave; li < a.n_list; li += n_waves) {
        const size_t ti = a.list[li];
        const Task tk = a.tasks[ti];
        const int n = tk.n, dlo = tk.dlo;
        const int m = tk.m < n - dlo ? tk.m : n - dlo;
        if (m <= 0 || n <= 0) {
            if (lane == 0) a.out[ti] = TaskOut{0, 0, 0, 0, 0, 0};
            continue;
        }
        const int kind = tk.kind & 3;
        bool ambig = false;
        {
            const bool rev = (tk.kind & TASK_REV) != 0, left = kind == 1;
            uint32_t vq = 0, vt[2] = {0, 0};
            if (4 * lane < m) vq = load_window4p(a.qcodes, (long long)tk.qa, left != rev, rev, 4 * lane);
#pragma unroll
            for (int r = 0; r < 2; ++r)
                if (4 * (lane + 64 * r) < n) vt[r] = load_window4p(a.tcodes, (long long)tk.ta, left, false, 4 * (lane + 64 * r));
            if (4 * lane < m) { *(uint32_t *)(sq + 4 * lane) = vq; ambig |= (vq & 0x04040404u) != 0; }
#pragma unroll
            for (int r = 0; r < 2; ++r)
                if (4 * (lane + 64 * r) < n) {
                    *(uint32_t *)(st + WT_PAD + 4 * (lane + 64 * r)) = vt[r];
                    ambig |= (vt[r] & 0x04040404u) != 0;
                }
        }
        __builtin_amdgcn_s_waitcnt(0);
        __builtin_amdgcn_wave_barrier();
        const int end_row = kind != 0 ? (int)(tk.narrow >> 1) - 1 : -1;
        int Hend = 0, best_h = 0, best_i = 0;
        const bool amb = __any(ambig);
        const bool two = a.go2 > 0 && !(tk.kind & TASK_ONE);
        auto rows_of = [&](auto AMB, auto EXTN, auto TW) {
            wide_rows<decltype(AMB)::value, decltype(EXTN)::value, decltype(TW)::value, W_CHUNKS, TB>(a, m, n, dlo, lane, end_row, sq, st, pl, Hend,
                                                                                                    best_h, best_i);
        };
        using T_ = std::true_type; using F_ = std::false_type;
        if (kind == 0) {
            if (two) { if (amb) rows_of(T_{}, F_{}, T_{}); else rows_of(F_{}, F_{}, T_{}); }
            else { if (amb) rows_of(T_{}, F_{}, F_{}); else rows_of(F_{}, F_{}, F_{}); }
        } else {
            if (two) { if (amb) rows_of(T_{}, T_{}, T_{}); else rows_of(F_{}, T_{}, T_{}); }
            else { if (amb) rows_of(T_{}, T_{}, F_{}); else rows_of(F_{}, T_{}, F_{}); }
        }
        int ei, ej, score;
        if (kind == 0) {
            ei = m; ej = n;
            score = __shfl(Hend, n - m - dlo, 64) - DP_BIAS;
        } else {
            unsigned long long best = 0;
            if (best_h > DP_BIAS / 2)
                best = (unsigned long long)(uint32_t)(best_h - DP_BIAS + (1 << 20)) << 32 |
                       (unsigned long long)(0xffffu - (uint32_t)(2 * best_i + dlo + lane)) << 16 |
                       (unsigned long long)(0xffffu - (uint32_t)best_i);
#pragma unroll
            for (int o = 32; o > 0; o >>= 1) {
                const unsigned long long u = __shfl_xor(best, o, 64);
                best = u > best ? u : best;
            }
            ei = (int)(0xffffu - (uint32_t)(best & 0xffff));
            ej = (int)(0xffffu - (uint32_t)((best >> 16) & 0xffff)) - ei;
            score = (int)(uint32_t)(best >> 32) - (1 << 20) - (ei == end_row ? a.end_bonus : 0);
        }
        __builtin_amdgcn_s_waitcnt(0);
        __builtin_amdgcn_wave_barrier();
        if constexpr (!TB) {
            if (lane == 0) a.out[ti] = TaskOut{score, ei, ej, 0, 0, kind != 0 && ei == end_row ? 0x80000000u : 0u};
            continue;
        }
        uint32_t *rbuf = s_runs[wv];
        const uint32_t rcap = a.run_buf_cap < (uint32_t)RUN_BUF ? a.run_buf_cap : (uint32_t)RUN_BUF;
        uint32_t cp_n = 0, cp_off = 0;
        if (lane == 0) {
            const uint32_t *planes = &pl[0][0][0];
            uint32_t ends = 0;
            const uint32_t n_runs = two ? wide_walk<true>(planes, W_CHUNKS, ei, ej, dlo, kind == 1, nullptr, 0, rbuf, rcap, &ends)
                                        : wide_walk<false>(planes, W_CHUNKS, ei, ej, dlo, kind == 1, nullptr, 0, rbuf, rcap, &ends);
            uint32_t off = 0;
            bool ok = true;
            if (n_runs) off = pool_take(a, n_runs, chunk_off, chunk_left, ok);
            if (ok && n_runs) {
                if (n_runs <= rcap) { cp_n = n_runs; cp_off = off; }
                else if (two) wide_walk<true>(planes, W_CHUNKS, ei, ej, dlo, kind == 1, a.runs + off, n_runs, nullptr, 0);
                else wide_walk<false>(planes, W_CHUNKS, ei, ej, dlo, kind == 1, a.runs + off, n_runs, nullptr, 0);
            }
            a.out[ti] = TaskOut{score, ei, ej, off, ok ? n_runs : 0, ends | (kind != 0 && ei == end_row ? 0x80000000u : 0u)};
        }
        __builtin_amdgcn_s_waitcnt(0);
        __builtin_amdgcn_wave_barrier();
        cp_n = (uint32_t)__builtin_amdgcn_readfirstlane((int)cp_n); cp_off = (uint32_t)__builtin_amdgcn_readfirstlane((int)cp_off);
        for (uint32_t k = (uint32_t)lane; k < cp_n; k += 64)
            a.runs[cp_off + k] = rbuf[kind == 1 ? k : cp_n - 1 - k];
        __builtin_amdgcn_wave_barrier();
    }
}

constexpr int LONG_TILE = 256;
constexpr int LT_LEN = LONG_TILE + BAND_W + 8;
struct LongArgs {
    uint32_t *planes;
    uint32_t *run_scratch;
    uint32_t chunks_cap;
    uint32_t runs_cap;
    int zdrop;
    uint32_t *next;
    uint32_t *too_long;
    unsigned long long *rows_run;
};

template <bool TWO, bool TB>
__global__ __launch_bounds__(WG) void align_long_kernel(AlignArgs a, LongArgs la) {
    __shared__ __attribute__((aligned(4))) uint8_t s_q[WAVES][LONG_TILE + 8];
    __shared__ __attribute__((aligned(4))) uint8_t s_t[WAVES][LT_LEN];
    const int lane = threadIdx.x & 63, wv = threadIdx.x >> 6;
    const size_t wave = (blockIdx.x * (size_t)blockDim.x + threadIdx.x) >> 6;
    uint32_t *const pl = TB ? la.planes + wave * ((size_t)N_WPLANES * la.chunks_cap * 64) : nullptr;
    uint32_t *const rs = TB ? la.run_scratch + wave * (size_t)la.runs_cap : nullptr;
    uint8_t *sq = s_q[wv], *st = s_t[wv];
    uint32_t chunk_off = 0, chunk_left = 0;
    const int go = a.go, ge = a.ge, goe = go + ge, gel = ge * lane, goel = go + ge * lane;
    const int go2 = a.go2, ge2 = a.ge2, goe2 = go2 + ge2, gel2 = ge2 * lane, goel2 = go2 + ge2 * lane;
    __builtin_amdgcn_s_setprio(3);
    for (;;) {
        uint32_t li = 0;
        if (lane == 0) li = atomicAdd(la.next, 1u);
        li = (uint32_t)__builtin_amdgcn_readfirstlane((int)li);
        if (li >= a.n_list) break;
        const size_t ti = a.list[li];
        const Task tk = a.tasks[ti];
        const int n = tk.n, dlo = tk.dlo;
        const int m = tk.m < n - dlo ? tk.m : n - dlo;
        const int kind = tk.kind & 3;
        const int chunks = (m + 31) >> 5;
        if (m <= 0 || n <= 0 || (TB && ((uint32_t)chunks > la.chunks_cap || (uint32_t)(m + n + 2) > la.runs_cap))) {
            if (lane == 0) {
                a.out[ti] = TaskOut{0, 0, 0, 0, 0, 0};
                if (m > 0 && n > 0) *la.too_long = 1;
            }
            continue;
        }
        const bool ext = kind != 0, rev = (tk.kind & TASK_REV) != 0, left = kind == 1;
        const int end_row = ext ? (int)(tk.narrow >> 1) - 1 : -1;
        const int j0 = dlo + lane;
        int gap0 = go + ge * j0;
        if (TWO && go2 + ge2 * j0 < gap0) gap0 = go2 + ge2 * j0;
        int H = j0 == 0 ? DP_BIAS : (j0 > 0 ? DP_BIAS - gap0 : 0);
        int G = H - goe, G2 = TWO ? H - goe2 : 0;
        uint32_t a0 = 0, a1 = 0, a2 = 0, a3 = 0, a4 = 0, b0 = 0, b1 = 0, b2 = 0, b3 = 0;
        int best_h = 0, best_i = 0;
        if (ext && j0 >= 0 && j0 <= n) best_h = H;
        int rows_done = m;
        bool stop = false;
        for (int r0 = 0; r0 < m && !stop; r0 += LONG_TILE) {
            const int R = m - r0 < LONG_TILE ? m - r0 : LONG_TILE;
            {
                __builtin_amdgcn_wave_barrier();
                const int xq = r0 + 4 * lane;
                uint32_t vq = 0x04040404u;
                if (4 * lane < R) vq = load_window4p(a.qcodes, (long long)tk.qa, left != rev, rev, xq);
                const int eb = r0 + dlo;
                uint32_t vt[2];
#pragma unroll
                for (int r = 0; r < 2; ++r) {
                    const int k = 4 * (lane + 64 * r), x = eb + k;
                    vt[r] = 0x04040404u;
                    if (k < R + 64 && x + 3 >= 0 && x < n) vt[r] = load_window4p(a.tcodes, (long long)tk.ta, left, false, x);
                }
                *(uint32_t *)(sq + 4 * lane) = vq;
#pragma unroll
                for (int r = 0; r < 2; ++r) {
                    const int k = 4 * (lane + 64 * r);
                    if (k < LT_LEN - 3) *(uint32_t *)(st + k) = vt[r];
                }
                __builtin_amdgcn_s_waitcnt(0);
                __builtin_amdgcn_wave_barrier();
            }
            const uint8_t *tp = st + lane;
            int qa = sq[0], t2 = tp[0];
            for (int ii = 1; ii <= R; ++ii) {
                const int i = r0 + ii;
                const int qa_next = sq[ii], t2_next = tp[ii];
                const bool ne = qa != t2;
                int s = ne ? -a.mismatch : a.match;
                s = (qa | t2) > 3 ? -a.ambi : s;
                const int mm = H + s;
                const int f1 = wave_shl1_z(G);
                const int f2 = TWO ? wave_shl1_z(G2) : 0;
                const int f = TWO && f2 > f1 ? f2 : f1;
                const int ht = mm > f ? mm : f;
                const int e1 = wave_shr1(wave_prefix_max_incl_dpp(ht + gel), 0) - goel;
                const int e2 = TWO ? wave_shr1(wave_prefix_max_incl_dpp(ht + gel2), 0) - goel2 : 0;
                const int e = TWO && e2 > e1 ? e2 : e1;
                const int h = ht > e ? ht : e;
                const int fo = h - goe, fe = f1 - ge;
                if (TB) {
                    a0 = shift_in(a0, mm == h);
                    a1 = shift_in(a1, e >= f);
                    a2 = shift_in(a2, e1 + go > h);
                    a3 = shift_in(a3, fe > fo);
                    a4 = shift_in(a4, ne);
                }
                G = fo > fe ? fo : fe;
                if (TWO) {
                    const int fo2 = h - goe2, fe2 = f2 - ge2;
                    if (TB) {
                        b0 = shift_in(b0, e2 > e1);
                        b1 = shift_in(b1, f2 > f1);
                        b2 = shift_in(b2, e2 + go2 > h);
                        b3 = shift_in(b3, fe2 > fo2);
                    }
                    G2 = fo2 > fe2 ? fo2 : fe2;
                }
                H = h;
                qa = qa_next; t2 = t2_next;
                const bool inside = (uint32_t)(i + j0) <= (uint32_t)n;
                if (ext) {
                    const int hb = h + (i == end_row ? a.end_bonus : 0);
                    if (inside && hb > best_h) { best_h = hb; best_i = i; }
                }
                if ((i & 31) == 0) {
                    if (TB) {
                        const size_t c = (size_t)(i >> 5) - 1;
                        pl[((size_t)WP_DIAG * chunks + c) * 64 + lane] = a0; pl[((size_t)WP_EGEF * chunks + c) * 64 + lane] = a1;
                        pl[((size_t)WP_EX1 * chunks + c) * 64 + lane] = a2; pl[((size_t)WP_FX1 * chunks + c) * 64 + lane] = a3;
                        pl[((size_t)WP_NE * chunks + c) * 64 + lane] = a4;
                        if (TWO) {
                            pl[((size_t)WP_EP * chunks + c) * 64 + lane] = b0; pl[((size_t)WP_FP * chunks + c) * 64 + lane] = b1;
                            pl[((size_t)WP_EX2 * chunks + c) * 64 + lane] = b2; pl[((size_t)WP_FX2 * chunks + c) * 64 + lane] = b3;
                        }
                    }
                    if (ext && la.zdrop > 0) {
                        const int row_max = (int)wave_max_u32_dpp(inside ? (uint32_t)h : 0u);
                        const int so_far = (int)wave_max_u32_dpp((uint32_t)best_h);
                        if (row_max == 0 || so_far - row_max > la.zdrop) { rows_done = i; stop = true; break; }
                    }
                }
            }
        }
        if (TB && (rows_done & 31)) {
            const size_t c = (size_t)(rows_done >> 5);
            const int up = 32 - (rows_done & 31);
            pl[((size_t)WP_DIAG * chunks + c) * 64 + lane] = a0 << up; pl[((size_t)WP_EGEF * chunks + c) * 64 + lane] = a1 << up;
            pl[((size_t)WP_EX1 * chunks + c) * 64 + lane] = a2 << up; pl[((size_t)WP_FX1 * chunks + c) * 64 + lane] = a3 << up;
            pl[((size_t)WP_NE * chunks + c) * 64 + lane] = a4 << up;
            if (TWO) {
                pl[((size_t)WP_EP * chunks + c) * 64 + lane] = b0 << up; pl[((size_t)WP_FP * chunks + c) * 64 + lane] = b1 << up;
                pl[((size_t)WP_EX2 * chunks + c) * 64 + lane] = b2 << up; pl[((size_t)WP_FX2 * chunks + c) * 64 + lane] = b3 << up;
            }
        }
        int ei, ej, score;
        if (!ext) {
            ei = m; ej = n;
            score = __shfl(H, n - m - dlo, 64) - DP_BIAS;
        } else {
            unsigned long long best = 0;
            if (best_h > DP_BIAS / 2)
                best = (unsigned long long)(uint32_t)(best_h - DP_BIAS + (1 << 20)) << 32 |
                       (unsigned long long)(0xffffu - (uint32_t)(2 * best_i + dlo + lane)) << 16 |
                       (unsigned long long)(0xffffu - (uint32_t)best_i);
#pragma unroll
            for (int o = 32; o > 0; o >>= 1) {
                const unsigned long long u = __shfl_xor(best, o, 64);
                best = u > best ? u : best;
            }
            ei = (int)(0xffffu - (uint32_t)(best & 0xffff));
            ej = (int)(0xffffu - (uint32_t)((best >> 16) & 0xffff)) - ei;
            score = (int)(uint32_t)(best >> 32) - (1 << 20) - (ei == end_row ? a.end_bonus : 0);
        }
        const uint32_t flag = ext && ei == end_row ? 0x80000000u : 0u;
        if (lane == 0) atomicAdd(la.rows_run, (unsigned long long)rows_done);
        if constexpr (!TB) {
            if (lane == 0) a.out[ti] = TaskOut{score, ei, ej, 0, 0, flag};
            continue;
        } else {
            __threadfence_block();
            __builtin_amdgcn_wave_barrier();
            uint32_t n_runs = 0, off = 0, ends = 0;
            bool ok = true;
            if (lane == 0) {
                n_runs = long_walk<TWO>(pl, chunks, ei, ej, dlo, left, rs, la.runs_cap, &ends, 2 * (m + n) + 8);
                if (n_runs) off = pool_take(a, n_runs, chunk_off, chunk_left, ok);
                a.out[ti] = TaskOut{score, ei, ej, off, ok ? n_runs : 0, ends | flag};
            }
            __threadfence_block();
            __builtin_amdgcn_wave_barrier();
            n_runs = (uint32_t)__builtin_amdgcn_readfirstlane((int)n_runs);
            off = (uint32_t)__builtin_amdgcn_readfirstlane((int)off);
            ok = __builtin_amdgcn_readfirstlane((int)ok) != 0;
            if (ok) for (uint32_t k = (uint32_t)lane; k < n_runs; k += 64)
                a.runs[off + k] = rs[left ? k : n_runs - 1 - k];
            __builtin_amdgcn_s_waitcnt(0);
            __builtin_amdgcn_wave_barrier();
        }
    }
}

constexpr int LT32_LEN = LONG_TILE + HALF_W + 8;
__device__ __forceinline__ int half_prefix_max_incl_dpp(int x) {
    constexpr int ident = DPP_MAX_IDENT;
    auto mx = [](int a, int b) { return a > b ? a : b; };
    x = mx(x, dpp_i32<0x111>(ident, x));
    x = mx(x, dpp_i32<0x112>(ident, x));
    x = mx(x, dpp_i32<0x114>(ident, x));
    x = mx(x, dpp_i32<0x118>(ident, x));
    x = mx(x, dpp_i32<0x142, 0xa>(ident, x));
    return x;
}
__device__ __forceinline__ uint32_t half_max_u32(uint32_t v, int hf) {
    int x = (int)v;
    auto mx = [](int a, int b) { return (int)((uint32_t)a > (uint32_t)b ? (uint32_t)a : (uint32_t)b); };
    x = mx(x, dpp_i32<0x111>(0, x));
    x = mx(x, dpp_i32<0x112>(0, x));
    x = mx(x, dpp_i32<0x114>(0, x));
    x = mx(x, dpp_i32<0x118>(0, x));
    x = mx(x, dpp_i32<0x142, 0xa>(0, x));
    return (uint32_t)__shfl(x, 32 * hf + 31, 64);
}

template <bool TWO, bool TB>
__global__ __launch_bounds__(WG) void align_long32_kernel(AlignArgs a, LongArgs la) {
    __shared__ __attribute__((aligned(4))) uint8_t s_q[WAVES][2][LONG_TILE + 8];
    __shared__ __attribute__((aligned(4))) uint8_t s_t[WAVES][2][LT32_LEN];
    const int lane = threadIdx.x & 63, wv = threadIdx.x >> 6, hf = lane >> 5, hl = lane & 31;
    const size_t wave = (blockIdx.x * (size_t)blockDim.x + threadIdx.x) >> 6;
    uint32_t *const pl = TB ? la.planes + wave * ((size_t)N_WPLANES * la.chunks_cap * 64) + (size_t)hf * ((size_t)N_WPLANES * la.chunks_cap * 32) : nullptr;
    uint32_t *const rs = TB ? la.run_scratch + (wave * 2 + (size_t)hf) * (size_t)la.runs_cap : nullptr;
    uint8_t *sq = s_q[wv][hf], *st = s_t[wv][hf];
    uint32_t chunk_off = 0, chunk_left = 0;
    const int go = a.go, ge = a.ge, goe = go + ge, gel = ge * hl, goel = go + ge * hl;
    const int go2 = a.go2, ge2 = a.ge2, goe2 = go2 + ge2, gel2 = ge2 * hl, goel2 = go2 + ge2 * hl;
    __builtin_amdgcn_s_setprio(3);
    for (;;) {
        uint32_t pi = 0;
        if (lane == 0) pi = atomicAdd(la.next, 1u);
        pi = (uint32_t)__builtin_amdgcn_readfirstlane((int)pi);
        if (2 * (size_t)pi >= a.n_list) break;
        const size_t li = 2 * (size_t)pi + (size_t)hf;
        bool live = li < a.n_list;
        size_t ti = 0;
        Task tk{};
        if (live) { ti = a.list[li]; tk = a.tasks[ti]; }
        const int n = tk.n, dlo = tk.dlo;
        int m = live ? (tk.m < n - dlo ? (int)tk.m : n - dlo) : 0;
        if (m < 0) m = 0;
        const int kind = tk.kind & 3;
        const int chunks = (m + 31) >> 5;
        if (live && (m <= 0 || n <= 0 || (TB && ((uint32_t)chunks > la.chunks_cap || (uint32_t)(m + n + 2) > la.runs_cap)))) {
            if (hl == 0) {
                a.out[ti] = TaskOut{0, 0, 0, 0, 0, 0};
                if (m > 0 && n > 0) *la.too_long = 1;
            }
            live = false;
            m = 0;
        }
        const int m0 = m;
        const bool ext = kind != 0, rev = (tk.kind & TASK_REV) != 0, left = kind == 1;
        const int end_row = ext ? (int)(tk.narrow >> 1) - 1 : -1;
        const int j0 = dlo + hl;
        int gap0 = go + ge * j0;
        if (TWO && go2 + ge2 * j0 < gap0) gap0 = go2 + ge2 * j0;
        int H = j0 == 0 ? DP_BIAS : (j0 > 0 ? DP_BIAS - gap0 : 0);
        int G = H - goe, G2 = TWO ? H - goe2 : 0, Hend = 0;
        uint32_t a0 = 0, a1 = 0, a2 = 0, a3 = 0, a4 = 0, b0 = 0, b1 = 0, b2 = 0, b3 = 0;
        int best_h = 0, best_i = 0;
        if (live && ext && j0 >= 0 && j0 <= n) best_h = H;
        for (int r0 = 0;; r0 += LONG_TILE) {
            const int mA = __builtin_amdgcn_readlane(m, 0), mB = __builtin_amdgcn_readlane(m, 32);
            const int rows_max = mA > mB ? mA : mB;
            if (r0 >= rows_max) break;
            const int R_all = rows_max - r0 < LONG_TILE ? rows_max - r0 : LONG_TILE;
            {
                __builtin_amdgcn_wave_barrier();
                const int R = m - r0 < 0 ? 0 : (m - r0 < LONG_TILE ? m - r0 : LONG_TILE);
                uint32_t vq[2], vt[3];
#pragma unroll
                for (int r = 0; r < 2; ++r) {
                    const int k = 4 * (hl + 32 * r);
                    vq[r] = 0x04040404u;
                    if (k < R) vq[r] = load_window4p(a.qcodes, (long long)tk.qa, left != rev, rev, r0 + k);
                }
                const int eb = r0 + dlo;
#pragma unroll
                for (int r = 0; r < 3; ++r) {
                    const int k = 4 * (hl + 32 * r), x = eb + k;
                    vt[r] = 0x04040404u;
                    if (R > 0 && k < R + HALF_W && x + 3 >= 0 && x < n) vt[r] = load_window4p(a.tcodes, (long long)tk.ta, left, false, x);
                }
#pragma unroll
                for (int r = 0; r < 2; ++r) *(uint32_t *)(sq + 4 * (hl + 32 * r)) = vq[r];
#pragma unroll
                for (int r = 0; r < 3; ++r) {
                    const int k = 4 * (hl + 32 * r);
                    if (k < LT32_LEN - 3) *(uint32_t *)(st + k) = vt[r];
                }
                __builtin_amdgcn_s_waitcnt(0);
                __builtin_amdgcn_wave_barrier();
            }
            const uint8_t *tp = st + hl;
            int qa = sq[0], t2 = tp[0];
            for (int ii = 1; ii <= R_all; ++ii) {
                const int i = r0 + ii;
                const int qa_next = sq[ii], t2_next = tp[ii];
                const bool ne = qa != t2;
                int s = ne ? -a.mismatch : a.match;
                s = (qa | t2) > 3 ? -a.ambi : s;
                const int mm = H + s;
                int f1 = wave_shl1_z(G);
                f1 = hl == 31 ? 0 : f1;
                int f2 = 0;
                if (TWO) { f2 = wave_shl1_z(G2); f2 = hl == 31 ? 0 : f2; }
                const int f = TWO && f2 > f1 ? f2 : f1;
                const int ht = mm > f ? mm : f;
                int p1 = wave_shr1(half_prefix_max_incl_dpp(ht + gel), 0);
                p1 = hl == 0 ? 0 : p1;
                const int e1 = p1 - goel;
                int e2 = 0;
                if (TWO) {
                    int p2 = wave_shr1(half_prefix_max_incl_dpp(ht + gel2), 0);
                    p2 = hl == 0 ? 0 : p2;
                    e2 = p2 - goel2;
                }
                const int e = TWO && e2 > e1 ? e2 : e1;
                const int h = ht > e ? ht : e;
                const int fo = h - goe, fe = f1 - ge;
                if (TB) {
                    a0 = shift_in(a0, mm == h);
                    a1 = shift_in(a1, e >= f);
                    a2 = shift_in(a2, e1 + go > h);
                    a3 = shift_in(a3, fe > fo);
                    a4 = shift_in(a4, ne);
                }
                G = fo > fe ? fo : fe;
                if (TWO) {
                    const int fo2 = h - goe2, fe2 = f2 - ge2;
                    if (TB) {
                        b0 = shift_in(b0, e2 > e1);
                        b1 = shift_in(b1, f2 > f1);
                        b2 = shift_in(b2, e2 + go2 > h);
                        b3 = shift_in(b3, fe2 > fo2);
                    }
                    G2 = fo2 > fe2 ? fo2 : fe2;
                }
                H = h;
                qa = qa_next; t2 = t2_next;
                const bool run = i <= m;
                const bool inside = run && (uint32_t)(i + j0) <= (uint32_t)n;
                if (i == m0) Hend = h;
                if (ext) {
                    const int hb = h + (i == end_row ? a.end_bonus : 0);
                    if (inside && hb > best_h) { best_h = hb; best_i = i; }
                }
                if ((i & 31) == 0) {
                    if (TB && run) {
                        const size_t c = (size_t)(i >> 5) - 1;
                        pl[((size_t)WP_DIAG * chunks + c) * 32 + hl] = a0; pl[((size_t)WP_EGEF * chunks + c) * 32 + hl] = a1;
                        pl[((size_t)WP_EX1 * chunks + c) * 32 + hl] = a2; pl[((size_t)WP_FX1 * chunks + c) * 32 + hl] = a3;
                        pl[((size_t)WP_NE * chunks + c) * 32 + hl] = a4;
                        if (TWO) {
                            pl[((size_t)WP_EP * chunks + c) * 32 + hl] = b0; pl[((size_t)WP_FP * chunks + c) * 32 + hl] = b1;
                            pl[((size_t)WP_EX2 * chunks + c) * 32 + hl] = b2; pl[((size_t)WP_FX2 * chunks + c) * 32 + hl] = b3;
                        }
                    }
                    if (la.zdrop > 0) {
                        const int row_max = (int)half_max_u32(inside ? (uint32_t)h : 0u, hf);
                        const int so_far = (int)half_max_u32((uint32_t)best_h, hf);
                        if (ext && run && i < m && (row_max == 0 || so_far - row_max > la.zdrop)) m = i;
                    }
                } else if (TB && i == m) {
                    const size_t c = (size_t)(i >> 5);
                    const int up = 32 - (i & 31);
                    pl[((size_t)WP_DIAG * chunks + c) * 32 + hl] = a0 << up; pl[((size_t)WP_EGEF * chunks + c) * 32 + hl] = a1 << up;
                    pl[((size_t)WP_EX1 * chunks + c) * 32 + hl] = a2 << up; pl[((size_t)WP_FX1 * chunks + c) * 32 + hl] = a3 << up;
                    pl[((size_t)WP_NE * chunks + c) * 32 + hl] = a4 << up;
                    if (TWO) {
                        pl[((size_t)WP_EP * chunks + c) * 32 + hl] = b0 << up; pl[((size_t)WP_FP * chunks + c) * 32 + hl] = b1 << up;
                        pl[((size_t)WP_EX2 * chunks + c) * 32 + hl] = b2 << up; pl[((size_t)WP_FX2 * chunks + c) * 32 + hl] = b3 << up;
                    }
                }
            }
        }
        int ei, ej, score;
        if (!ext) {
            ei = m0; ej = n;
            score = __shfl(Hend, 32 * hf + ((n - m0 - dlo) & (HALF_W - 1)), 64) - DP_BIAS;
        } else {
            unsigned long long best = 0;
            if (best_h > DP_BIAS / 2)
                best = (unsigned long long)(uint32_t)(best_h - DP_BIAS + (1 << 20)) << 32 |
                       (unsigned long long)(0xffffu - (uint32_t)(2 * best_i + dlo + hl)) << 16 |
                       (unsigned long long)(0xffffu - (uint32_t)best_i);
#pragma unroll
            for (int o = 16; o > 0; o >>= 1) {
                const unsigned long long u = __shfl_xor(best, o, 64);
                best = u > best ? u : best;
            }
            ei = (int)(0xffffu - (uint32_t)(best & 0xffff));
            ej = (int)(0xffffu - (uint32_t)((best >> 16) & 0xffff)) - ei;
            score = (int)(uint32_t)(best >> 32) - (1 << 20) - (ei == end_row ? a.end_bonus : 0);
        }
        const uint32_t flag = ext && ei == end_row ? 0x80000000u : 0u;
        if (live && hl == 0) atomicAdd(la.rows_run, (unsigned long long)m);
        if constexpr (!TB) {
            if (live && hl == 0) a.out[ti] = TaskOut{score, ei, ej, 0, 0, flag};
            continue;
        } else {
            __threadfence_block();
            __builtin_amdgcn_wave_barrier();
            uint32_t n_runs = 0, off = 0, ends = 0;
            bool ok = true;
            if (live && hl == 0) {
                n_runs = long_walk<TWO, HALF_W>(pl, chunks, ei, ej, dlo, left, rs, la.runs_cap, &ends, 2 * (m0 + n) + 8);
                if (n_runs) off = pool_take(a, n_runs, chunk_off, chunk_left, ok);
                a.out[ti] = TaskOut{score, ei, ej, off, ok ? n_runs : 0, ends | flag};
            }
            __threadfence_block();
            __builtin_amdgcn_wave_barrier();
            n_runs = (uint32_t)__shfl((int)n_runs, 32 * hf, 64);
            off = (uint32_t)__shfl((int)off, 32 * hf, 64);
            ok = __shfl((int)ok, 32 * hf, 64) != 0;
            if (ok) for (uint32_t k = (uint32_t)hl; k < n_runs; k += 32)
                a.runs[off + k] = rs[left ? k : n_runs - 1 - k];
            __builtin_amdgcn_s_waitcnt(0);
            __builtin_amdgcn_wave_barrier();
        }
    }
}

template <bool TB>
__global__ __launch_bounds__(WG) void align_ungapped_kernel(AlignArgs a, int zdrop) {
    const int lane = threadIdx.x & 63;
    const size_t tid = blockIdx.x * (size_t)blockDim.x + threadIdx.x, n_thr = (size_t)gridDim.x * blockDim.x;
    const size_t rounds = (a.n_list + n_thr - 1) / n_thr;
    uint32_t chunk_off = 0, chunk_left = 0;
    for (size_t r = 0; r < rounds; ++r) {
        const size_t u = r * n_thr + tid;
        const bool live = u < a.n_list;
        size_t ti = 0;
        Task tk{};
        if (live) { ti = a.list[u]; tk = a.tasks[ti]; }
        const int kind = tk.kind & 3;
        const bool ext = kind != 0, rev = (tk.kind & TASK_REV) != 0, left = kind == 1;
        const int L = live ? (tk.m < tk.n ? tk.m : tk.n) : 0;
        const int end_row = ext ? (int)(tk.narrow >> 1) - 1 : -1;
        auto pair_at = [&](int x, uint64_t &q8, uint64_t &t8) {
            q8 = load_window8p(a.qcodes, (long long)tk.qa, left != rev, rev, x);
            t8 = load_window8p(a.tcodes, (long long)tk.ta, left, false, x);
        };
        int score = 0, best = 0, best_i = 0, best_s = 0, cur = -1;
        uint32_t nr = 0, nr_best = 0, first_op = 0, last_op_best = 0;
        bool stop = false;
        for (int x = 0; x < L && !stop; x += 8) {
            uint64_t q8, t8;
            pair_at(x, q8, t8);
            const int lim = L - x < 8 ? L - x : 8;
            for (int y = 0; y < lim; ++y) {
                const int qc = (int)(q8 >> (8 * y)) & 0xff, tc = (int)(t8 >> (8 * y)) & 0xff, i = x + y + 1;
                score += (qc | tc) > 3 ? -a.ambi : (qc == tc ? a.match : -a.mismatch);
                const int op = qc == tc ? (int)OP_EQ : (int)OP_X;
                if (op != cur) { if (!nr) first_op = (uint32_t)op; ++nr; cur = op; }
                if (ext) {
                    const int rank = score + (i == end_row ? a.end_bonus : 0);
                    if (rank > best) { best = rank; best_i = i; best_s = score; nr_best = nr; last_op_best = (uint32_t)op; }
                    if (zdrop > 0 && (i & (ZDROP_STEP - 1)) == 0 && best - score > zdrop) { stop = true; break; }
                }
            }
        }
        const int take = ext ? best_i : L;
        const int out_score = ext ? best_s : score;
        uint32_t n_runs = ext ? nr_best : nr, last_op = ext ? last_op_best : (uint32_t)cur;
        if (!TB || take == 0) n_runs = 0;
        uint32_t wave_total;
        const uint32_t mine = wave_excl_sum_u32(n_runs, lane, wave_total);
        uint32_t base = 0;
        bool ok = true;
        if (wave_total) {
            if (lane == 0) base = pool_take(a, wave_total, chunk_off, chunk_left, ok);
            base = (uint32_t)__shfl((int)base, 0, 64);
            ok = __shfl((int)ok, 0, 64) != 0;
        }
        if (live && ok && n_runs) {
            uint32_t k = 0, len = 0;
            int op_cur = -1;
            uint32_t *dst = a.runs + base + mine;
            auto put = [&]() { dst[left ? n_runs - 1 - k : k] = len << 4 | (uint32_t)op_cur; ++k; };
            for (int x = 0; x < take; x += 8) {
                uint64_t q8, t8;
                pair_at(x, q8, t8);
                const int lim = take - x < 8 ? take - x : 8;
                for (int y = 0; y < lim; ++y) {
                    const int op = ((q8 >> (8 * y)) & 0xff) == ((t8 >> (8 * y)) & 0xff) ? (int)OP_EQ : (int)OP_X;
                    if (op != op_cur) { if (len) put(); op_cur = op; len = 0; }
                    ++len;
                }
            }
            if (len) put();
        }
        if (live) {
            const uint32_t ends = n_runs ? (left ? end_codes(last_op, first_op) : end_codes(first_op, last_op)) : 0u;
            a.out[ti] = TaskOut{out_score, ext ? take : (int)tk.m, ext ? take : (int)tk.n, base + mine, ok ? n_runs : 0,
                                ends | (ext && take == end_row ? 0x80000000u : 0u)};
        }
    }
}

struct AsmArgs {
    const Piece *pieces;
    const FixPt *fps;
    const uint32_t *task_off;
    const TaskOut *tout;
    const uint32_t *runs;
    size_t n_pieces;
    const uint32_t *qlen, *tlen, *rank_q, *rank_t, *chunk_of_t;
    int min_dp_score, end_bonus;
    const uint32_t *plist;
    const PieceGeom *pg;
    uint8_t *late;
    int stub_score;
    int bare;
    uint32_t stage_cap;
};

constexpr uint32_t ASM_MID = 4;
constexpr int ASM_STAGE = 1024;
template <bool WRITE>
__global__ __launch_bounds__(WG) void assemble_kernel(AsmArgs a, uint32_t *n_ops, uint8_t *valid, const uint64_t *ops_off,
                                                       uint32_t *ops, PafRec *recs, uint64_t *ord_hi, uint64_t *ord_lo) {
    __shared__ uint32_t s_stage[WRITE ? WAVES : 1][WRITE ? ASM_STAGE : 1];
    uint32_t *const stage = s_stage[WRITE ? (threadIdx.x >> 6) : 0];
    const int lane = threadIdx.x & 63;
    const size_t wave = (blockIdx.x * (size_t)blockDim.x + threadIdx.x) >> 6;
    const size_t n_waves = ((size_t)gridDim.x * blockDim.x) >> 6;
    for (size_t idx = wave; idx < a.n_pieces; idx += n_waves) {
        const size_t i = !WRITE && a.plist ? (size_t)a.plist[idx] : idx;
        if (WRITE && !valid[i]) continue;
        const Piece p = a.pieces[i];
        const FixPt *fp = a.fps + p.fp_off;
        const TaskOut *to = a.tout + a.task_off[i];
        const uint32_t n_tasks = p.n_fp + 1;
        const bool bare = a.bare && a.pg[i].stub_cand != 0;
        uint32_t *w = WRITE ? ops + ops_off[i] : nullptr;
        long long score = 0;
        unsigned long long nmatch = 0, blen = 0;
        uint32_t slots = 0;
        uint32_t carry_code = 99;
        constexpr uint32_t NO_SLOT = 0xffffffffu;
        uint32_t open_idx = NO_SLOT, open_val = 0;
        int ext_l_i = 0, ext_l_j = 0, ext_r_i = 0, ext_r_j = 0;
        TaskOut r_next{0, 0, 0, 0, 0, 0};
        if ((uint32_t)lane < n_tasks) r_next = to[lane];
        for (uint32_t t0 = 0; t0 < n_tasks; t0 += 64) {
            const uint32_t t = t0 + (uint32_t)lane;
            TaskOut r = r_next;
            r_next = TaskOut{0, 0, 0, 0, 0, 0};
            if (t + 64 < n_tasks) r_next = to[t + 64];
            bool keep = false;
            if (t < n_tasks) {
                keep = true;
                if (t == 0 || t == n_tasks - 1)
                    keep = !(r.score + ((r.pad & 0x80000000u) ? a.end_bonus : 0) <= 0 || (r.n_runs == 0 && !bare));
            }
            if (keep && t == 0) { ext_l_i = r.bi; ext_l_j = r.bj; }
            if (keep && t == n_tasks - 1 && t != 0) { ext_r_i = r.bi; ext_r_j = r.bj; }
            long long sc = keep ? r.score : 0;
            const uint32_t nr = keep && !bare ? r.n_runs : 0;
            const uint32_t first = r.pad & 15u, last = (r.pad >> 4) & 15u;
            const unsigned long long ne_mask = __ballot(nr != 0);
            const unsigned long long below = ne_mask & ((1ull << lane) - 1ull);
            const int prev_lane = below ? 63 - __clzll((long long)below) : 0;
            const uint32_t prev_last = (uint32_t)__shfl((int)last, prev_lane, 64);
            const uint32_t prev_code = below ? (prev_last & 15u) : carry_code;
            const bool mrg = nr != 0 && (first & 15u) == prev_code;
            uint32_t tot_runs, tot_mrg;
            const uint32_t S = wave_excl_sum_u32(nr, lane, tot_runs);
            const uint32_t Mx = wave_excl_sum_u32(mrg ? 1u : 0u, lane, tot_mrg);
            if (WRITE) {
                const uint32_t F = nr ? a.runs[r.runs_off] : 0u;
                const uint32_t L = nr >= 2 ? a.runs[r.runs_off + nr - 1] : F;
                uint32_t mid[ASM_MID];
#pragma unroll
                for (uint32_t u = 0; u < ASM_MID; ++u) mid[u] = u + 3 <= nr ? a.runs[r.runs_off + 1 + u] : 0u;
                const uint32_t P = wave_prefix_sum_incl_dpp(mrg ? F >> 4 : 0u);
                const bool opens = nr != 0 && (!mrg || nr >= 2);
                const unsigned long long om = __ballot(opens);
                const uint32_t P_end = (uint32_t)__builtin_amdgcn_readlane((int)P, 63);
                const uint32_t T0 = om ? (uint32_t)__shfl((int)P, __ffsll((long long)om) - 1, 64) : P_end;
                open_val += T0 << 4;
                if (om && open_idx != NO_SLOT && lane == 0) w[open_idx] = open_val;
                const unsigned long long above = lane == 63 ? 0ull : om & ~((2ull << lane) - 1ull);
                const uint32_t P_next = (uint32_t)__shfl((int)P, above ? __ffsll((long long)above) - 1 : 63, 64);
                const uint32_t base = slots + S - (Mx + (mrg ? 1u : 0u));
                const uint32_t own_slot = base + (nr ? nr - 1 : 0u);
                const uint32_t own_val = L + ((P_next - P) << 4);
                const uint32_t n_out = tot_runs - tot_mrg;
                const bool staged = n_out <= a.stage_cap;
                auto put = [&](uint32_t slot, uint32_t v) { if (staged) stage[slot - slots] = v; else w[slot] = v; };
                if (om) {
                    const int lb = 63 - __clzll((long long)om);
                    open_idx = (uint32_t)__builtin_amdgcn_readlane((int)own_slot, lb);
                    open_val = (uint32_t)__builtin_amdgcn_readlane((int)own_val, lb);
                    if (opens && lane != lb) put(own_slot, own_val);
                }
                if (nr) {
                    blen += F >> 4;
                    if ((F & 15u) == OP_EQ) nmatch += F >> 4;
                }
                if (nr >= 2) {
                    blen += L >> 4;
                    if ((L & 15u) == OP_EQ) nmatch += L >> 4;
                    if (!mrg) put(base, F);
#pragma unroll
                    for (uint32_t u = 0; u < ASM_MID; ++u)
                        if (u + 3 <= nr) {
                            blen += mid[u] >> 4;
                            if ((mid[u] & 15u) == OP_EQ) nmatch += mid[u] >> 4;
                            put(base + 1 + u, mid[u]);
                        }
                    for (uint32_t x = 1 + ASM_MID; x + 1 < nr; ++x) {
                        const uint32_t run = a.runs[r.runs_off + x];
                        blen += run >> 4;
                        if ((run & 15u) == OP_EQ) nmatch += run >> 4;
                        put(base + x, run);
                    }
                }
                if (staged) {
                    __builtin_amdgcn_s_waitcnt(0xc07f);
                    __builtin_amdgcn_wave_barrier();
                    for (uint32_t k = (uint32_t)lane; k < n_out; k += 64)
                        if (slots + k != open_idx) w[slots + k] = stage[k];
                    __builtin_amdgcn_s_waitcnt(0xc07f);
                    __builtin_amdgcn_wave_barrier();
                }
            }
            slots += tot_runs - tot_mrg;
            if (ne_mask) carry_code = (uint32_t)__shfl((int)last, 63 - __clzll((long long)ne_mask), 64) & 15u;
#pragma unroll
            for (int o = 32; o > 0; o >>= 1) sc += __shfl_xor(sc, o, 64);
            score += sc;
        }
        const int li = __shfl(ext_l_i, 0, 64), lj = __shfl(ext_l_j, 0, 64);
        const int last_lane = (int)((n_tasks - 1) & 63u);
        const int ri = __shfl(ext_r_i, last_lane, 64), rj = __shfl(ext_r_j, last_lane, 64);
        if (!WRITE) {
            if (lane == 0) {
                const bool ok = (slots > 0 || bare) && score >= a.min_dp_score;
                valid[i] = ok ? 1 : 0;
                n_ops[i] = ok ? slots : 0;
                if (a.late) a.late[i] = a.pg[i].stub_cand && !((slots > 0 || bare) && score >= a.stub_score) ? 1 : 0;
            }
            continue;
        }
#pragma unroll
        for (int o = 32; o > 0; o >>= 1) { nmatch += __shfl_xor(nmatch, o, 64); blen += __shfl_xor(blen, o, 64); }
        if (lane == 0) {
            if (open_idx != NO_SLOT) w[open_idx] = open_val;
            const int qs = (int)fp[0].q - li, ts = (int)fp[0].t - lj;
            const int qe = (int)fp[p.n_fp - 1].q + ri, te = (int)fp[p.n_fp - 1].t + rj;
            const uint32_t ql = a.qlen[p.q];
            PafRec r{};
            r.qid = a.rank_q[p.q]; r.tid = a.rank_t[p.t];
            r.qlen = ql; r.tlen = a.tlen[p.t];
            r.qs = p.strand ? ql - (uint32_t)qe : (uint32_t)qs;
            r.qe = p.strand ? ql - (uint32_t)qs : (uint32_t)qe;
            r.ts = (uint32_t)ts; r.te = (uint32_t)te;
            r.nmatch = (uint32_t)nmatch; r.blen = (uint32_t)blen;
            r.flags = p.strand ? PF_REV : 0;
            r.chunk = a.chunk_of_t[p.t];
            r.cig_off = ops_off[i]; r.cig_n = slots; r.tie = 0;
            recs[i] = r;
            ord_hi[i] = (uint64_t)r.chunk << 32 | p.q;
            ord_lo[i] = (uint64_t)p.t << 43 | (uint64_t)p.strand << 42 | (uint64_t)(p.chain & 0x3fffffu) << 20 | (p.piece & 0xfffffu);
        }
    }
}

template <bool WRITE>
__global__ __launch_bounds__(WG) void assemble_lane_kernel(AsmArgs a, uint32_t *n_ops, uint8_t *valid, const uint64_t *ops_off,
                                                            uint32_t *ops, PafRec *recs, uint64_t *ord_hi, uint64_t *ord_lo) {
    const size_t idx = blockIdx.x * (size_t)blockDim.x + threadIdx.x;
    if (idx >= a.n_pieces) return;
    const size_t i = !WRITE && a.plist ? (size_t)a.plist[idx] : idx;
    if (WRITE && !valid[i]) return;
    const Piece p = a.pieces[i];
    const FixPt *fp = a.fps + p.fp_off;
    const TaskOut *to = a.tout + a.task_off[i];
    const uint32_t n_tasks = p.n_fp + 1;
    const bool bare = a.bare && a.pg[i].stub_cand != 0;
    uint32_t *w = WRITE ? ops + ops_off[i] : nullptr;
    long long score = 0;
    unsigned long long nmatch = 0, blen = 0;
    uint32_t slots = 0;
    uint32_t pend = 0;
    uint32_t carry_code = 99;
    int li = 0, lj = 0, ri = 0, rj = 0;
    for (uint32_t t = 0; t < n_tasks; ++t) {
        const TaskOut r = to[t];
        bool keep = true;
        if (t == 0 || t == n_tasks - 1)
            keep = !(r.score + ((r.pad & 0x80000000u) ? a.end_bonus : 0) <= 0 || (r.n_runs == 0 && !bare));
        if (!keep) continue;
        if (t == 0) { li = r.bi; lj = r.bj; }
        else if (t == n_tasks - 1) { ri = r.bi; rj = r.bj; }
        score += r.score;
        const uint32_t nr = bare ? 0u : r.n_runs;
        if (!nr) continue;
        const uint32_t first = r.pad & 15u, last = (r.pad >> 4) & 15u;
        const bool mrg = first == carry_code;
        carry_code = last;
        if (!WRITE) {
            slots += nr - (mrg ? 1u : 0u);
            continue;
        }
        for (uint32_t x = 0; x < nr; ++x) {
            const uint32_t run = a.runs[r.runs_off + x];
            blen += run >> 4;
            if ((run & 15u) == OP_EQ) nmatch += run >> 4;
            if (x == 0 && mrg) pend += (run >> 4) << 4;
            else {
                if (pend) w[slots++] = pend;
                pend = run;
            }
        }
    }
    if (!WRITE) {
        const bool ok = (slots > 0 || bare) && score >= a.min_dp_score;
        valid[i] = ok ? 1 : 0;
        n_ops[i] = ok ? slots : 0;
        if (a.late) a.late[i] = a.pg[i].stub_cand && !((slots > 0 || bare) && score >= a.stub_score) ? 1 : 0;
        return;
    }
    if (pend) w[slots++] = pend;
    const int qs = (int)fp[0].q - li, ts = (int)fp[0].t - lj;
    const int qe = (int)fp[p.n_fp - 1].q + ri, te = (int)fp[p.n_fp - 1].t + rj;
    const uint32_t ql = a.qlen[p.q];
    PafRec r{};
    r.qid = a.rank_q[p.q]; r.tid = a.rank_t[p.t];
    r.qlen = ql; r.tlen = a.tlen[p.t];
    r.qs = p.strand ? ql - (uint32_t)qe : (uint32_t)qs;
    r.qe = p.strand ? ql - (uint32_t)qs : (uint32_t)qe;
    r.ts = (uint32_t)ts; r.te = (uint32_t)te;
    r.nmatch = (uint32_t)nmatch; r.blen = (uint32_t)blen;
    r.flags = p.strand ? PF_REV : 0;
    r.chunk = a.chunk_of_t[p.t];
    r.cig_off = ops_off[i]; r.cig_n = slots; r.tie = 0;
    recs[i] = r;
    ord_hi[i] = (uint64_t)r.chunk << 32 | p.q;
    ord_lo[i] = (uint64_t)p.t << 43 | (uint64_t)p.strand << 42 | (uint64_t)(p.chain & 0x3fffffu) << 20 | (p.piece & 0xfffffu);
}

__global__ void late_tasks_kernel(const uint32_t *plist, size_t n, const Piece *pieces, const uint32_t *task_off, uint32_t *tasks,
                                  uint32_t *count) {
    size_t j = blockIdx.x * (size_t)blockDim.x + threadIdx.x;
    if (j == 0) *count = (uint32_t)(2 * n);
    if (j >= n) return;
    const uint32_t i = plist[j];
    tasks[2 * j] = task_off[i];
    tasks[2 * j + 1] = task_off[i] + pieces[i].n_fp;
}

__global__ __launch_bounds__(WG) void class_bases_kernel(const uint8_t *cls, const uint8_t *cls_bare, const Task *tasks, size_t n,
                                                          unsigned long long *out) {
    __shared__ unsigned long long s_sum[14];
    if (threadIdx.x < 14) s_sum[threadIdx.x] = 0;
    __syncthreads();
    for (size_t i = blockIdx.x * (size_t)blockDim.x + threadIdx.x; i < n; i += (size_t)gridDim.x * blockDim.x) {
        const int c = cls[i], cb = cls_bare ? cls_bare[i] : 0;
        if (!c && !cb) continue;
        const Task &t = tasks[i];
        int slot;
        if (c) slot = c == 1 ? ((int)t.m < NR_SMALL ? 0 : 1) : c == 3 ? 2 : c == 2 ? 3 : c == 4 ? 4 : c == CLS_LONG ? 5 : c == CLS_LONG32 ? 12 : 11;
        else slot = cb == 1 ? 6 : cb == 3 ? 7 : cb == 2 ? 8 : cb == 4 ? 9 : cb == CLS_LONG ? 10 : cb == CLS_LONG32 ? 13 : 11;
        atomicAdd(&s_sum[slot], (unsigned long long)((int)t.m + (int)t.n));
    }
    __syncthreads();
    if (threadIdx.x < 14 && s_sum[threadIdx.x]) atomicAdd(&out[threadIdx.x], s_sum[threadIdx.x]);
}

__global__ __launch_bounds__(WG) void list_ext_kernel(const Task *tasks, const uint32_t *list, size_t n, unsigned long long *out) {
    unsigned long long c = 0, r = 0;
    for (size_t i = blockIdx.x * (size_t)blockDim.x + threadIdx.x; i < n; i += (size_t)gridDim.x * blockDim.x) {
        const Task &t = tasks[list[i]];
        if (t.kind & 3) { ++c; r += (unsigned long long)(int)t.m; }
    }
#pragma unroll
    for (int o = 32; o > 0; o >>= 1) { c += __shfl_xor(c, o, 64); r += __shfl_xor(r, o, 64); }
    if ((threadIdx.x & 63) == 0 && c) { atomicAdd(out, c); atomicAdd(out + 1, r); }
}

__global__ void class_flag_kernel(const uint8_t *cls, size_t n, uint8_t v, uint8_t *flag) {
    size_t i = blockIdx.x * (size_t)blockDim.x + threadIdx.x;
    if (i < n) flag[i] = cls[i] == v ? 1 : 0;
}

__global__ void compact_rows_kernel(const uint32_t *idx, size_t n, const PafRec *recs, const uint64_t *hi,
                                    const uint64_t *lo, PafRec *orecs, uint64_t *ohi, uint64_t *olo) {
    size_t i = blockIdx.x * (size_t)blockDim.x + threadIdx.x;
    if (i >= n) return;
    orecs[i] = recs[idx[i]];
    ohi[i] = hi[idx[i]];
    olo[i] = lo[idx[i]];
}

__global__ __launch_bounds__(WG) void piece_long_flag_kernel(const Piece *pieces, size_t n, const FixPt *fps, const uint32_t *qlen,
                                                              const uint32_t *tlen, int ext_max, uint8_t *flag) {
    const int lane = threadIdx.x & 63;
    const size_t wave = (blockIdx.x * (size_t)blockDim.x + threadIdx.x) >> 6;
    const size_t n_waves = ((size_t)gridDim.x * blockDim.x) >> 6;
    for (size_t i = wave; i < n; i += n_waves) {
        const Piece p = pieces[i];
        const FixPt *fp = fps + p.fp_off;
        bool lng = false;
        if (lane == 0) {
            const FixPt a = fp[0], b = fp[p.n_fp - 1];
            const int ql = (int)qlen[p.q], tl = (int)tlen[p.t];
            auto rows = [&](int aq, int at) {
                const int m = aq < ext_max ? aq : ext_max, nn = at < m + BAND_W ? at : m + BAND_W;
                return m < nn + (BAND_W / 2 - 1) ? m : nn + (BAND_W / 2 - 1);
            };
            lng = rows((int)a.q, (int)a.t) > EXT_MAX || rows(ql - (int)b.q, tl - (int)b.t) > EXT_MAX;
        }
        for (uint32_t k = (uint32_t)lane; k + 1 < p.n_fp && !__any(lng); k += 64) {
            const FixPt f0 = fp[k], f1 = fp[k + 1];
            lng = lng || (int)(f1.q - f0.q) > BLOCK_MAX || (int)(f1.t - f0.t) > BLOCK_MAX;
        }
        const bool any = __any(lng);
        if (lane == 0) flag[i] = any ? 1 : 0;
    }
}
__global__ __launch_bounds__(WG) void piece_long_flag_lane_kernel(const Piece *pieces, size_t n, const FixPt *fps, const uint32_t *qlen,
                                                                   const uint32_t *tlen, int ext_max, uint8_t *flag) {
    const size_t i = blockIdx.x * (size_t)blockDim.x + threadIdx.x;
    if (i >= n) return;
    const Piece p = pieces[i];
    const FixPt *fp = fps + p.fp_off;
    FixPt f0 = fp[0];
    const FixPt b = fp[p.n_fp - 1];
    const int ql = (int)qlen[p.q], tl = (int)tlen[p.t];
    auto rows = [&](int aq, int at) {
        const int m = aq < ext_max ? aq : ext_max, nn = at < m + BAND_W ? at : m + BAND_W;
        return m < nn + (BAND_W / 2 - 1) ? m : nn + (BAND_W / 2 - 1);
    };
    bool lng = rows((int)f0.q, (int)f0.t) > EXT_MAX || rows(ql - (int)b.q, tl - (int)b.t) > EXT_MAX;
    for (uint32_t k = 1; k < p.n_fp && !lng; ++k) {
        const FixPt f1 = fp[k];
        lng = (int)(f1.q - f0.q) > BLOCK_MAX || (int)(f1.t - f0.t) > BLOCK_MAX;
        f0 = f1;
    }
    flag[i] = lng ? 1 : 0;
}
__global__ void gather_pieces_kernel(const Piece *src, const uint32_t *idx, size_t n, Piece *dst, uint32_t *n_fp) {
    size_t i = blockIdx.x * (size_t)blockDim.x + threadIdx.x;
    if (i >= n) return;
    const Piece p = src[idx[i]];
    dst[i] = p;
    if (n_fp) n_fp[i] = p.n_fp;
}
__global__ __launch_bounds__(WG) void move_fixed_points_kernel(Piece *pieces, size_t n, const uint32_t *off, uint32_t fp_base, const FixPt *src,
                                                                FixPt *dst) {
    const int lane = threadIdx.x & 63;
    const size_t wave = (blockIdx.x * (size_t)blockDim.x + threadIdx.x) >> 6;
    const size_t n_waves = ((size_t)gridDim.x * blockDim.x) >> 6;
    for (size_t i = wave; i < n; i += n_waves) {
        const Piece p = pieces[i];
        const uint32_t to = off[i];
        for (uint32_t k = (uint32_t)lane; k < p.n_fp; k += 64) dst[to + k] = src[p.fp_off + k];
        if (lane == 0) pieces[i].fp_off = fp_base + to;
    }
}
}

struct PieceSpan { struct { const Piece *p; } pieces; size_t n_pieces, n_fp; struct { const FixPt *p; } fps; };
static void align_span(const AvaInput &in, const hlmi_ava_opts &o, const uint32_t *d_qlen, const uint32_t *d_tlen,
                       const PieceSpan &ch, AlignOut &out) {
    out = AlignOut();
    const size_t P = ch.n_pieces;
    if (!P) return;
    DBuf<uint32_t> tcnt(P), toff(P);
    hipLaunchKernelGGL(piece_task_count_kernel, grid1(P), dim3(WG), 0, stream(), ch.pieces.p, P, tcnt.p);
    exclusive_scan_u32(tcnt.p, toff.p, P);
    const size_t NT = ch.n_fp + P;
    DBuf<Task> tasks(NT);
    if (P >= (1u << 30)) fail(HLMI_EINVAL, "more than 2^30 alignment pieces in one batch");
    DBuf<TaskRef> task_ref(NT);
    DBuf<PieceGeom> pgeom(P);
    if (NT <= 17 * P)
        hipLaunchKernelGGL(task_ref_lane_kernel, grid1(P), dim3(WG), 0, stream(), ch.pieces.p, toff.p, P, d_qlen, d_tlen, in.Q->off.p, in.T->off.p,
                           ch.fps.p, o.stub_oh, ext_rows(o), task_ref.p, pgeom.p);
    else
    hipLaunchKernelGGL(task_ref_kernel, dim3((unsigned)std::min<size_t>(cdiv(P, (size_t)WAVES), 256 * 32)), dim3(WG), 0, stream(),
                       ch.pieces.p, toff.p, P, d_qlen, d_tlen, in.Q->off.p, in.T->off.p, ch.fps.p, o.stub_oh, ext_rows(o), task_ref.p, pgeom.p);
    HIP_CHECK(hipGetLastError());
    DBuf<TaskOut> tout(NT);
    DBuf<uint32_t> counters(2);
    DBuf<unsigned long long> astats(N_ALIGN_STATS);
    constexpr size_t MAX_BLOCKS = 256 * 16;
    const size_t open_chunks = MAX_BLOCKS * (4 * WAVES * RUN_CHUNK + 2 * 4 * WAVES * RUN_CHUNK_SMALL) +
                               (size_t)3 * 256 * 32 * 8 * PK_WAVES * RUN_CHUNK_SMALL;
    size_t run_share = std::max<size_t>(NT * 12, 1 << 16);
    DBuf<uint32_t> runs;
    AsmArgs as{};
    as.pieces = ch.pieces.p; as.fps = ch.fps.p; as.task_off = toff.p; as.tout = tout.p; as.n_pieces = P;
    as.min_dp_score = o.min_dp_score; as.end_bonus = o.end_bonus;
    as.qlen = d_qlen; as.tlen = d_tlen; as.rank_q = in.d_rank_q; as.rank_t = in.d_rank_t; as.chunk_of_t = in.d_chunk_of_t;
    as.pg = pgeom.p; as.stub_score = o.min_dp_score + std::max(0, o.end_bonus);
    as.stage_cap = (uint32_t)ASM_STAGE;
    if (const char *e = hook("HLMI_ASM_STAGE_CAP")) as.stage_cap = (uint32_t)std::min(ASM_STAGE, std::max(0, atoi(e)));
    DBuf<uint32_t> nops(P);
    DBuf<uint8_t> valid(P), late(o.stub_oh >= 0 ? P : 0);
    DBuf<uint32_t> late_idx(o.stub_oh >= 0 ? P : 0);
    size_t n_late = 0;
    const unsigned nba = (unsigned)std::min<size_t>(cdiv(P, (size_t)WAVES), 256 * 32);
    const bool small_pieces = NT <= 17 * P && !hook("HLMI_ASM_WAVE");
    const int worst = std::max(std::max(o.match, o.mismatch), std::max(o.ambi, o.gap_open + o.gap_ext));
    const bool packed = worst > 0 && (long long)worst * (BLOCK_MAX + NARROW_W + 2) <= 4000 && o.match >= 0 && o.mismatch >= 0 &&
                        o.ambi >= 0 && o.gap_open >= 0 && o.gap_ext >= 0 && !hook("HLMI_NARROW_UNPACKED");
    const bool bare = o.stub_oh >= 0 && packed && !hook("HLMI_STUB_FULL_ROWS");
    as.bare = bare ? 1 : 0;
    if (long_rows_cap(o) > 32000) fail(HLMI_EINVAL, "max_gap %d: alignment tasks are limited to 32 000 rows", o.max_gap);
    bool ext_all_long = false;
    if (o.zdrop > 0) {
        const int D = std::max(std::max(o.mismatch, o.ambi), o.gap_open + o.gap_ext);
        const int rows_down = D > 0 ? (o.zdrop + D - 1) / D : EXT_MAX;
        ext_all_long = (long long)o.match * (EXT_MAX - rows_down) + std::max(o.end_bonus, 0) > o.zdrop;
    }
    const uint32_t long_chunks_cap = (uint32_t)(long_rows_cap(o) + 31) / 32, long_runs_cap = (uint32_t)(2 * long_rows_cap(o) + 64);
    constexpr unsigned LONG_BLOCKS_MAX = 256 * 8;
    struct LongLaunch { DBuf<uint32_t> list, planes, runs, ctl; };
    std::vector<std::unique_ptr<LongLaunch>> long_launches;
    struct LongReady { AlignArgs al; LongArgs la; unsigned nb; bool half, tb; const char *timer; };
    std::vector<LongReady> long_ready;
    hipEvent_t long_done = nullptr;
    bool long_pending = false, long_on_side = false;
    struct SideGuard {
        ~SideGuard() { if (hipStream_t s = side_stream_if_created()) (void)hipStreamSynchronize(s); }
    } side_guard;
    auto join_long = [&]() {
        if (!long_pending) return;
        if (long_on_side) {
            if (!long_done) HIP_CHECK(hipEventCreateWithFlags(&long_done, hipEventDisableTiming));
            HIP_CHECK(hipEventRecord(long_done, side_stream()));
            HIP_CHECK(hipStreamWaitEvent(stream(), long_done, 0));
            long_on_side = false;
        }
        long_pending = false;
    };
    DBuf<uint8_t> long_flag;
    DBuf<uint32_t> long_list, long_n(1);
    size_t n_long_tb = 0, n_long_bare = 0;
    double long_rows_run = 0;
    static const char *const LB_NAMES[] = {"align_narrow_small", "align_narrow", "align_narrow_long", "align_wide", "align_wide_short",
                                           "align_long", "align_score_narrow", "align_score_narrow_long", "align_score_wide",
                                           "align_score_wide_short", "align_score_long", "align_ungapped", "align_long32",
                                           "align_score_long32"};
    constexpr int N_LB = 14;
    DBuf<unsigned long long> lb_bases(N_LB + 2);
    std::vector<double> lb_n(N_LB, 0.0);
    lb_bases.zero();
    auto note_list = [&](const char *timer, const Task *tk, const uint32_t *lst, size_t n) {
        if (!n) return;
        int slot = 0;
        while (slot < N_LB && strcmp(LB_NAMES[slot], timer) != 0) ++slot;
        if (slot == N_LB) return;
        lb_n[slot] += (double)n;
        (void)tk; (void)lst;
    };
    for (int attempt = 0;; ++attempt) {
        const size_t cap_runs = run_share + open_chunks;
        if (cap_runs >= (1ull << 32)) fail(HLMI_ENOMEM, "CIGAR run pool exceeds 4G entries");
        runs.alloc(cap_runs);
        counters.zero();
        lb_bases.zero();
        std::fill(lb_n.begin(), lb_n.end(), 0.0);
        AlignArgs aa{};
        aa.tasks = tasks.p; aa.n_tasks = NT;
        aa.geom = TaskGeom{task_ref.p, pgeom.p, ch.fps.p};
        aa.qcodes = in.Q->codes(); aa.tcodes = in.T->codes();
        aa.q_total = (long long)in.Q->total; aa.t_total = (long long)in.T->total;
        if (!hook("HLMI_CLASSIFY_BYTES")) {
            if (!in.Q->packed_store.p || !in.T->packed_store.p) fail(HLMI_ESTATE, "alignment of a read set without its 2-bit copy (DevReads::pack)");
            aa.qpacked = in.Q->packed(); aa.tpacked = in.T->packed();
            aa.qnflag = in.Q->nflag.p; aa.tnflag = in.T->nflag.p;
        }
        aa.end_bonus = o.end_bonus;
        aa.ext_max = ext_rows(o);
        aa.ext_all_long = ext_all_long ? 1 : 0;
        aa.ungapped = o.bandwidth == 0 ? 1 : 0;
        aa.match = o.match; aa.mismatch = o.mismatch; aa.go = o.gap_open; aa.ge = o.gap_ext; aa.ambi = o.ambi;
        aa.go2 = o.gap_open2 > 0 ? o.gap_open2 : 0; aa.ge2 = o.gap_open2 > 0 ? o.gap_ext2 : 0;
        if (aa.go2 && aa.go2 + aa.ge2 * (NARROW_W - 1) < aa.go + aa.ge * (NARROW_W - 1))
            fail(HLMI_EINVAL, "two-piece gap cost: the second piece must not be the cheaper one below %d bases", NARROW_W);
        {
            const int den = o.match + o.mismatch, num = o.match + 2 * (o.gap_open + o.gap_ext);
            aa.kmax = den > 0 && num > 0 ? std::min(3, (num - 1) / den) : 0;
            if (o.match <= 0 || o.gap_open < 0 || o.gap_ext <= 0) aa.kmax = -1;
            const int k = aa.kmax + 1, U = den, T = num;
            aa.kgap1 = aa.kmax >= 0 && U < o.gap_open + 2 * o.gap_ext + o.match && !hook("HLMI_NO_GAP1_CERT") ? 1 : 0;
            {
                auto c = [&](int L) { int v = o.gap_open + o.gap_ext * L; if (o.gap_open2 > 0) v = std::min(v, o.gap_open2 + o.gap_ext2 * L); return v; };
                aa.kgap2 = aa.kgap1 && U < o.match + c(2) && 2 * U < o.match + 2 * c(1) && 2 * U < 2 * o.match + c(2) + c(3) - c(1) &&
                           c(2) == o.gap_open + 2 * o.gap_ext && c(1) == o.gap_open + o.gap_ext && !hook("HLMI_NO_GAP2_CERT") ? 1 : 0;
            }
            aa.kshift = aa.kmax >= 0 && k <= 3 && k * U > T && k * U < T + o.match + std::min(2 * o.gap_ext, o.gap_open + o.gap_ext) &&
                        !hook("HLMI_NO_SHIFT_CERT") ? 1 : 0;
        }
        aa.trim_ok = hook("HLMI_NO_SUFFIX_TRIM") ? 0 : 1;
        aa.one_ok = hook("HLMI_NO_ONE_PIECE_CERT") ? 0 : 1;
        {
            const int U = o.match + o.mismatch;
            int G = o.gap_open + o.gap_ext;
            if (aa.go2 > 0) G = std::min(G, aa.go2 + aa.ge2);
            const bool sane = aa.kmax >= 0 && o.match > 0 && o.mismatch >= 0 && !hook("HLMI_NO_EXT_CERT");
            aa.kext_plain = sane && G >= U && U < 2 * G + o.match ? 1 : 0;
            aa.kext_bonus = 0;
            for (int k = 1; k <= 2; ++k)
                if (sane && o.end_bonus > 0 && k * U < G && k * U < o.end_bonus + o.match && k * U < 2 * G + o.match) aa.kext_bonus = k;
        }
        aa.out = tout.p; aa.runs = runs.p; aa.cap_runs = (uint32_t)cap_runs; aa.counters = counters.p;
        as.runs = runs.p;
        aa.run_buf_cap = 0xffffffffu;
        if (const char *e = hook("HLMI_RUN_BUF_CAP")) aa.run_buf_cap = (uint32_t)std::max(0, atoi(e));
        DBuf<uint8_t> cls(NT), f1(NT), cls_bare(bare ? NT : 0);
        DBuf<uint32_t> list1(NT), list2(NT), list3(NT), list4(NT);
        DBuf<uint32_t> list_n(4);
        aa.cls_bare = bare ? cls_bare.p : nullptr;
        auto class_list = [&](const uint8_t *cls_arr, uint8_t v) -> size_t {
            if (long_flag.n < NT) { long_flag.alloc(NT); long_list.alloc(NT); }
            hipLaunchKernelGGL(class_flag_kernel, grid1(NT), dim3(WG), 0, stream(), cls_arr, NT, v, long_flag.p);
            select_flagged_indices_async(long_flag.p, long_list.p, NT, long_n.p);
            return (size_t)long_n.download(1)[0];
        };
        auto run_ungapped = [&](const uint8_t *cls_arr, bool tb) -> size_t {
            if (!aa.ungapped) return 0;
            const size_t nl = class_list(cls_arr, CLS_UNGAPPED);
            if (!nl) return 0;
            aa.list = long_list.p; aa.n_list = nl;
            note_list("align_ungapped", tasks.p, long_list.p, nl);
            KTimer kt("align_ungapped");
            const unsigned nb = (unsigned)std::min<size_t>(cdiv(nl, (size_t)WG), MAX_BLOCKS);
            if (tb) hipLaunchKernelGGL(align_ungapped_kernel<true>, dim3(nb), dim3(WG), 0, stream(), aa, o.zdrop);
            else hipLaunchKernelGGL(align_ungapped_kernel<false>, dim3(nb), dim3(WG), 0, stream(), aa, o.zdrop);
            HIP_CHECK(hipGetLastError());
            return nl;
        };
        auto run_long_class = [&](const uint8_t *cls_arr, bool tb, uint8_t cv) -> size_t {
            const bool half = cv == CLS_LONG32;
            const char *timer = half ? (tb ? "align_long32" : "align_score_long32") : (tb ? "align_long" : "align_score_long");
            const size_t nl = class_list(cls_arr, cv);
            if (!nl) return 0;
            note_list(timer, tasks.p, long_list.p, nl);
            hipLaunchKernelGGL(list_ext_kernel, dim3((unsigned)std::min<size_t>(cdiv(nl, (size_t)WG), 1024)), dim3(WG), 0, stream(), tasks.p,
                               long_list.p, nl, lb_bases.p + N_LB);
            long_launches.emplace_back(new LongLaunch());
            LongLaunch &L = *long_launches.back();
            {
                DBuf<uint32_t> key(nl);
                hipLaunchKernelGGL(task_rows_desc_key_kernel, grid1(nl), dim3(WG), 0, stream(), tasks.p, long_list.p, nl, key.p);
                L.list.alloc(nl);
                HIP_CHECK(hipMemcpyAsync(L.list.p, long_list.p, nl * 4, hipMemcpyDeviceToDevice, stream()));
                sort_pairs_u32_u32(key, L.list, nl, 0, 16);
            }
            const size_t units = half ? (nl + 1) / 2 : nl;
            const unsigned nb = (unsigned)std::min<size_t>((units + WAVES - 1) / WAVES, LONG_BLOCKS_MAX);
            const size_t n_waves = (size_t)nb * WAVES;
            LongArgs la{};
            if (tb) {
                L.planes.alloc(n_waves * (size_t)N_WPLANES * long_chunks_cap * 64);
                L.runs.alloc(n_waves * (size_t)long_runs_cap * (half ? 2 : 1));
                la.planes = L.planes.p; la.run_scratch = L.runs.p;
            }
            la.chunks_cap = long_chunks_cap; la.runs_cap = long_runs_cap; la.zdrop = o.zdrop;
            L.ctl.alloc(4);
            L.ctl.zero();
            la.next = L.ctl.p; la.too_long = L.ctl.p + 1; la.rows_run = (unsigned long long *)(L.ctl.p + 2);
            AlignArgs al = aa;
            al.list = L.list.p; al.n_list = nl;
            long_ready.push_back(LongReady{al, la, nb, half, tb, timer});
            return nl;
        };
        auto launch_long_ready = [&]() {
            if (long_ready.empty()) return;
            sync();
            const bool on_side = hook("HLMI_LONG_SIDE_STREAM") != nullptr;
            hipStream_t ls = on_side ? side_stream() : stream();
            long_on_side = long_on_side || on_side;
            for (const LongReady &r : long_ready) {
                KTimer kt(r.timer, ls);
                const bool two = aa.go2 > 0;
                auto go = [&](auto kern) { hipLaunchKernelGGL(kern, dim3(r.nb), dim3(WG), 0, ls, r.al, r.la); };
                if (r.half) {
                    if (r.tb) go(align_long32_kernel<false, true>); else go(align_long32_kernel<false, false>);
                } else {
                    if (r.tb) { if (two) go(align_long_kernel<true, true>); else go(align_long_kernel<false, true>); }
                    else { if (two) go(align_long_kernel<true, false>); else go(align_long_kernel<false, false>); }
                }
            }
            HIP_CHECK(hipGetLastError());
            long_ready.clear();
            long_pending = true;
        };
        auto run_long = [&](const uint8_t *cls_arr, bool tb) -> size_t {
            if (aa.ungapped) return run_ungapped(cls_arr, tb);
            const size_t n32 = run_long_class(cls_arr, tb, CLS_LONG32);
            return n32 + run_long_class(cls_arr, tb, CLS_LONG);
        };
        auto check_long = [&]() {
            for (auto &L : long_launches) {
                if (!L->ctl.n) continue;
                const std::vector<uint32_t> c = L->ctl.download(4);
                if (c[1]) fail(HLMI_EINVAL, "an alignment task exceeds the scratch area of align_long_kernel");
                long_rows_run += (double)((unsigned long long)c[3] << 32 | c[2]);
                L->ctl.release(); L->planes.release(); L->runs.release(); L->list.release();
            }
        };
        size_t n_bare_tasks = 0;
        auto run_bare_long = [&]() {
            if (!bare) return;
            const size_t nl = run_long(cls_bare.p, false);
            n_bare_tasks += nl; n_long_bare += nl;
        };
        auto run_bare = [&](bool with_long) {
            if (!bare) return;
            if (with_long) { run_bare_long(); launch_long_ready(); }
            select_classes4_async(cls_bare.p, NT, list1.p, list2.p, list3.p, list4.p, list_n.p);
            const std::vector<uint32_t> hb = list_n.download(4);
            n_bare_tasks += (size_t)hb[0] + hb[1] + hb[2] + hb[3];
            for (int which = 0; which < 2; ++which) {
                DBuf<uint32_t> &lst = which ? list3 : list1;
                const size_t nl = which ? hb[2] : hb[0];
                if (nl < 8) continue;
                DBuf<uint32_t> key(nl);
                hipLaunchKernelGGL(task_rows_key_kernel, grid1(nl), dim3(WG), 0, stream(), tasks.p, lst.p, nl, key.p);
                sort_pairs_u32_u32(key, lst, nl, 0, 7);
            }
            auto pk_grid = [](size_t n) { return dim3((unsigned)std::max<size_t>(1, std::min<size_t>(((n + 7) / 8 + PK_WAVES - 1) / PK_WAVES, 256 * 32))); };
            auto w_grid = [](size_t n) { return dim3((unsigned)std::max<size_t>(1, std::min<size_t>((n + WAVES - 1) / WAVES, 256 * 16))); };
            if (hb[0]) {
                note_list("align_score_narrow", tasks.p, list1.p, hb[0]);
                KTimer kt("align_score_narrow");
                aa.list = list1.p; aa.n_list = hb[0];
                hipLaunchKernelGGL((align_narrow_pk_kernel<NR_SHORT, false>), pk_grid(hb[0]), dim3(64 * PK_WAVES), 0, stream(), aa);
            }
            if (hb[2]) {
                note_list("align_score_narrow_long", tasks.p, list3.p, hb[2]);
                KTimer kt("align_score_narrow_long");
                aa.list = list3.p; aa.n_list = hb[2];
                hipLaunchKernelGGL((align_narrow_pk_kernel<BLOCK_MAX, false>), pk_grid(hb[2]), dim3(64 * PK_WAVES), 0, stream(), aa);
            }
            if (hb[1]) {
                note_list("align_score_wide", tasks.p, list2.p, hb[1]);
                KTimer kt("align_score_wide");
                aa.list = list2.p; aa.n_list = hb[1];
                hipLaunchKernelGGL((align_kernel<EXT_MAX, false>), w_grid(hb[1]), dim3(WG), 0, stream(), aa);
            }
            if (hb[3]) {
                note_list("align_score_wide_short", tasks.p, list4.p, hb[3]);
                KTimer kt("align_score_wide_short");
                aa.list = list4.p; aa.n_list = hb[3];
                hipLaunchKernelGGL((align_kernel<WIDE_SHORT, false>), w_grid(hb[3]), dim3(WG), 0, stream(), aa);
            }
        };
        {
            KTimer kt("align_classify");
            const unsigned nbc = (unsigned)std::min<size_t>(cdiv(NT, (size_t)WG), MAX_BLOCKS);
            astats.zero();
            aa.defer_flag = f1.p;
            aa.defer_list = list1.p; aa.defer_count = list_n.p;
            hipLaunchKernelGGL(classify_kernel<1>, dim3(nbc ? nbc : 1), dim3(WG), 0, stream(), aa, cls.p, astats.p);
            select_flagged_indices_async(f1.p, list1.p, NT, list_n.p);
            const unsigned nb2 = std::max(1u, nbc / 4);
            hipLaunchKernelGGL(classify_kernel<2>, dim3(nb2), dim3(WG), 0, stream(), aa, cls.p, astats.p);
        }
        HIP_CHECK(hipGetLastError());
        hipLaunchKernelGGL(class_bases_kernel, dim3((unsigned)std::min<size_t>(cdiv(NT, (size_t)WG), 2048)), dim3(WG), 0, stream(), cls.p,
                           bare ? cls_bare.p : nullptr, tasks.p, NT, lb_bases.p);
        select_classes4_async(cls.p, NT, list1.p, list2.p, list3.p, list4.p, list_n.p);
        const std::vector<uint32_t> hn = list_n.download(4);
        const size_t n1 = hn[0], n2 = hn[1], n3 = hn[2], n4 = hn[3];
        for (int which = 0; which < 2; ++which) {
            DBuf<uint32_t> &lst = which ? list3 : list1;
            const size_t nl = which ? n3 : n1;
            if (nl < 8) continue;
            DBuf<uint32_t> key(nl);
            hipLaunchKernelGGL(task_rows_key_kernel, grid1(nl), dim3(WG), 0, stream(), tasks.p, lst.p, nl, key.p);
            sort_pairs_u32_u32(key, lst, nl, 0, 7);
        }
        unsigned long long long_seen = astats.download(N_ALIGN_STATS)[ST_LONG];
        if (long_seen || aa.ungapped) {
            run_bare_long();
            n_long_tb += run_long(cls.p, true);
            launch_long_ready();
        }
        if (n1 && packed) {
            size_t n_small = 0;
            if (n1 >= 8) n_small = std::min<size_t>(n1, (size_t)astats.download(N_ALIGN_STATS)[ST_NARROW_SMALL]);
            if (n_small) {
                note_list("align_narrow_small", tasks.p, list1.p, n_small);
                KTimer kt("align_narrow_small");
                aa.list = list1.p; aa.n_list = n_small;
                const unsigned nb = (unsigned)std::min<size_t>(((n_small + 7) / 8 + PK_WAVES - 1) / PK_WAVES, 256 * 32);
                hipLaunchKernelGGL(align_narrow_pk_kernel<NR_SMALL>, dim3(nb ? nb : 1), dim3(64 * PK_WAVES), 0, stream(), aa);
            }
            if (n1 > n_small) {
                note_list("align_narrow", tasks.p, list1.p + n_small, n1 - n_small);
                KTimer kt("align_narrow");
                aa.list = list1.p + n_small; aa.n_list = n1 - n_small;
                const unsigned nb = (unsigned)std::min<size_t>(((aa.n_list + 7) / 8 + PK_WAVES - 1) / PK_WAVES, 256 * 32);
                hipLaunchKernelGGL(align_narrow_pk_kernel<NR_SHORT>, dim3(nb ? nb : 1), dim3(64 * PK_WAVES), 0, stream(), aa);
            }
        } else if (n1) {
            note_list("align_narrow", tasks.p, list1.p, n1);
            KTimer kt("align_narrow");
            aa.list = list1.p; aa.n_list = n1;
            const unsigned nb = (unsigned)std::min<size_t>(((n1 + 3) / 4 + WAVES - 1) / WAVES, 256 * 16);
            hipLaunchKernelGGL(align_narrow_kernel<NR_SHORT>, dim3(nb ? nb : 1), dim3(WG), 0, stream(), aa);
        }
        if (n3 && packed && !hook("HLMI_NARROW_LONG_UNPACKED")) {
            note_list("align_narrow_long", tasks.p, list3.p, n3);
            KTimer kt("align_narrow_long");
            aa.list = list3.p; aa.n_list = n3;
            const unsigned nb = (unsigned)std::min<size_t>(((n3 + 7) / 8 + PK_WAVES - 1) / PK_WAVES, 256 * 32);
            hipLaunchKernelGGL(align_narrow_pk_kernel<BLOCK_MAX>, dim3(nb ? nb : 1), dim3(64 * PK_WAVES), 0, stream(), aa);
        } else if (n3) {
            note_list("align_narrow_long", tasks.p, list3.p, n3);
            KTimer kt("align_narrow_long");
            aa.list = list3.p; aa.n_list = n3;
            const unsigned nb = (unsigned)std::min<size_t>(((n3 + 3) / 4 + WAVES - 1) / WAVES, 256 * 16);
            hipLaunchKernelGGL(align_narrow_kernel<BLOCK_MAX>, dim3(nb ? nb : 1), dim3(WG), 0, stream(), aa);
        }
        auto run_wide = [&](size_t n_long, size_t n_short) {
            if (n_long) {
                note_list("align_wide", tasks.p, list2.p, n_long);
                KTimer kt("align_wide");
                aa.list = list2.p; aa.n_list = n_long;
                const unsigned nb = (unsigned)std::min<size_t>((n_long + WAVES - 1) / WAVES, 256 * 16);
                hipLaunchKernelGGL(align_kernel<EXT_MAX>, dim3(nb ? nb : 1), dim3(WG), 0, stream(), aa);
            }
            if (n_short) {
                note_list("align_wide_short", tasks.p, list4.p, n_short);
                KTimer kt("align_wide_short");
                aa.list = list4.p; aa.n_list = n_short;
                const unsigned nb = (unsigned)std::min<size_t>((n_short + WAVES - 1) / WAVES, 256 * 16);
                hipLaunchKernelGGL(align_kernel<WIDE_SHORT>, dim3(nb ? nb : 1), dim3(WG), 0, stream(), aa);
            }
        };
        run_wide(n2, n4);
        run_bare(false);
        size_t n_wide_late = 0;
        if (o.stub_oh >= 0) {
            as.plist = nullptr; as.n_pieces = P; as.late = late.p;
            join_long();
            {
                KTimer kt("assemble_count");
                if (small_pieces) hipLaunchKernelGGL(assemble_lane_kernel<false>, grid1(as.n_pieces), dim3(WG), 0, stream(), as, nops.p, valid.p,
                                                     nullptr, nullptr, nullptr, nullptr, nullptr);
                else
                hipLaunchKernelGGL(assemble_kernel<false>, dim3(nba), dim3(WG), 0, stream(), as, nops.p, valid.p, nullptr, nullptr,
                                   nullptr, nullptr, nullptr);
            }
            as.late = nullptr;
            n_late = select_flagged_indices(late.p, late_idx.p, P);
            if (n_late) {
                hipLaunchKernelGGL(late_tasks_kernel, grid1(n_late), dim3(WG), 0, stream(), late_idx.p, n_late, ch.pieces.p, toff.p,
                                   list1.p, list_n.p);
                HIP_CHECK(hipMemsetAsync(cls.p, 0, NT, stream()));
                if (bare) HIP_CHECK(hipMemsetAsync(cls_bare.p, 0, NT, stream()));
                {
                    KTimer kt("align_classify");
                    aa.defer_list = list1.p; aa.defer_count = list_n.p;
                    const unsigned nb2 = (unsigned)std::min<size_t>(cdiv(2 * n_late, (size_t)WG), MAX_BLOCKS);
                    hipLaunchKernelGGL(classify_kernel<2>, dim3(nb2 ? nb2 : 1), dim3(WG), 0, stream(), aa, cls.p, astats.p);
                }
                hipLaunchKernelGGL(class_bases_kernel, dim3((unsigned)std::min<size_t>(cdiv(NT, (size_t)WG), 2048)), dim3(WG), 0, stream(), cls.p,
                                   bare ? cls_bare.p : nullptr, tasks.p, NT, lb_bases.p);
                if (bare) {
                    const size_t before = n_bare_tasks;
                    const bool more_long = astats.download(N_ALIGN_STATS)[ST_LONG] > long_seen || aa.ungapped;
                    run_bare(more_long);
                    n_wide_late = n_bare_tasks - before;
                } else {
                    select_classes4_async(cls.p, NT, list1.p, list2.p, list3.p, list4.p, list_n.p);
                    const std::vector<uint32_t> hl = list_n.download(4);
                    run_wide(hl[1], hl[3]);
                    const bool more_long = astats.download(N_ALIGN_STATS)[ST_LONG] > long_seen || aa.ungapped;
                    const size_t nl = more_long ? run_long(cls.p, true) : 0;
                    launch_long_ready();
                    n_long_tb += nl;
                    n_wide_late = (size_t)hl[1] + hl[3] + nl;
                }
                as.plist = late_idx.p; as.n_pieces = n_late;
                const unsigned nbl = (unsigned)std::min<size_t>(cdiv(n_late, (size_t)WAVES), 256 * 32);
                join_long();
                {
                    KTimer kt("assemble_count");
                    if (small_pieces) hipLaunchKernelGGL(assemble_lane_kernel<false>, grid1(as.n_pieces), dim3(WG), 0, stream(), as, nops.p, valid.p,
                                                         nullptr, nullptr, nullptr, nullptr, nullptr);
                    else
                    hipLaunchKernelGGL(assemble_kernel<false>, dim3(nbl), dim3(WG), 0, stream(), as, nops.p, valid.p, nullptr, nullptr,
                                       nullptr, nullptr, nullptr);
                }
                as.plist = nullptr; as.n_pieces = P;
            }
        }
        if (attempt == 0) {
            stat_add("align_tasks_narrow", (double)(n1 + n3)); stat_add("align_tasks_wide", (double)(n2 + n4 + (bare ? 0 : n_wide_late)));
            stat_add("align_tasks_score_only", (double)n_bare_tasks);
            stat_add("align_tasks_long", (double)n_long_tb); stat_add("align_tasks_long_score_only", (double)n_long_bare);
        }
        HIP_CHECK(hipGetLastError());
        join_long();
        std::vector<uint32_t> hc = counters.download(2);
        check_long();
        if (!hc[1]) break;
        if (attempt >= 3) fail(HLMI_ENOMEM, "CIGAR run pool overflow");
        run_share *= 4;
    }
    stat_add("align_tasks", (double)NT);
    {
        std::vector<unsigned long long> h = astats.download(N_ALIGN_STATS);
        stat_add("align_tasks_fast", (double)h[ST_FAST]);
        stat_add("align_tasks_packed", (double)h[ST_PACKED]);
        stat_add("align_tasks_dp", (double)h[ST_DP]);
        stat_add("align_dp_rows", (double)h[ST_DP_ROWS]);
        stat_add("align_dp_bases", (double)h[ST_BASES]);
        stat_add("align_bases_classify", (double)h[ST_BASES_SQUARE]);
        stat_add("align_bases_narrow", (double)h[ST_BASES_NARROW]);
        stat_add("align_bases_wide", (double)h[ST_BASES_WIDE]);
        stat_add("align_bases_long", (double)h[ST_BASES_LONG]);
        const std::vector<unsigned long long> lb = lb_bases.download(N_LB + 2);
        stat_add("align_long_rows_run", long_rows_run);
        stat_add("align_long_ext", (double)lb[N_LB]);
        stat_add("align_long_ext_rows", (double)lb[N_LB + 1]);
        for (int k = 0; k < N_LB; ++k)
            if (lb_n[k] > 0) {
                stat_add(std::string("align_n.") + LB_NAMES[k], lb_n[k]);
                stat_add(std::string("align_bases.") + LB_NAMES[k], (double)lb[k]);
            }
        stat_add("align_tasks_wide_one_piece", (double)h[ST_WIDE_ONE]);
        stat_add("align_ext_certified", (double)h[ST_EXT_CERT]);
        stat_add("align_ext_dp_bonus_row_elsewhere", (double)h[ST_EXT_DP_ROW]);
        stat_add("align_ext_dp_substitutions", (double)h[ST_EXT_DP_K]);
        stat_add("align_ext_held", (double)h[ST_STUB_EXT]);
        stat_add("align_ext_late", (double)(2 * n_late));
    }
    if (o.stub_oh < 0) {
        KTimer kt("assemble_count");
        if (small_pieces) hipLaunchKernelGGL(assemble_lane_kernel<false>, grid1(as.n_pieces), dim3(WG), 0, stream(), as, nops.p, valid.p,
                                             nullptr, nullptr, nullptr, nullptr, nullptr);
        else
        hipLaunchKernelGGL(assemble_kernel<false>, dim3(nba), dim3(WG), 0, stream(), as, nops.p, valid.p, nullptr, nullptr,
                           nullptr, nullptr, nullptr);
    }
    HIP_CHECK(hipGetLastError());
    DBuf<uint64_t> ooff(P);
    exclusive_scan_u32_to_u64(nops.p, ooff.p, P);
    const size_t n_ops = (size_t)(download_one(ooff.p + (P - 1)) + download_one(nops.p + (P - 1)));
    DBuf<uint32_t> vidx(P);
    const size_t R = select_flagged_indices(valid.p, vidx.p, P);
    if (!R) return;
    out.ops.alloc(n_ops ? n_ops : 1);
    DBuf<PafRec> recs(P);
    DBuf<uint64_t> hi(P), lo(P);
    {
        KTimer kt("assemble_write");
        if (small_pieces) hipLaunchKernelGGL(assemble_lane_kernel<true>, grid1(as.n_pieces), dim3(WG), 0, stream(), as, nullptr, valid.p, ooff.p,
                                             out.ops.p, recs.p, hi.p, lo.p);
        else
        hipLaunchKernelGGL(assemble_kernel<true>, dim3(nba), dim3(WG), 0, stream(), as, nullptr, valid.p, ooff.p, out.ops.p,
                           recs.p, hi.p, lo.p);
    }
    HIP_CHECK(hipGetLastError());
    out.recs.alloc(R);
    out.ord_hi.alloc(R);
    out.ord_lo.alloc(R);
    hipLaunchKernelGGL(compact_rows_kernel, grid1(R), dim3(WG), 0, stream(), vidx.p, R, recs.p, hi.p, lo.p, out.recs.p,
                       out.ord_hi.p, out.ord_lo.p);
    HIP_CHECK(hipGetLastError());
    sync();
    out.n_rows = R;
    out.n_ops = n_ops;
}

}

namespace hlmi {
void align_pieces(const AvaInput &in, const hlmi_ava_opts &o, const uint32_t *d_qlen, const uint32_t *d_tlen,
                  const ChainOut &ch_in, std::vector<AlignOut> &outs, DeferredPieces *defer) {
    if (!ch_in.n_pieces) return;
    ChainOut kept;
    const ChainOut *chp = &ch_in;
    if (defer && o.bandwidth != 0) {
        const size_t P0 = ch_in.n_pieces;
        DBuf<uint8_t> flag(P0), nflag(P0);
        if (ch_in.n_fp <= 16 * P0)
            hipLaunchKernelGGL(piece_long_flag_lane_kernel, grid1(P0), dim3(WG), 0, stream(), ch_in.pieces.p, P0, ch_in.fps.p, d_qlen, d_tlen,
                               ext_rows(o), flag.p);
        else
        hipLaunchKernelGGL(piece_long_flag_kernel, dim3((unsigned)std::min<size_t>(cdiv(P0, (size_t)WAVES), 256 * 32)), dim3(WG), 0, stream(),
                           ch_in.pieces.p, P0, ch_in.fps.p, d_qlen, d_tlen, ext_rows(o), flag.p);
        DBuf<uint32_t> lidx(P0);
        const size_t n_long = select_flagged_indices(flag.p, lidx.p, P0);
        if (n_long && n_long * 10 <= P0) {
            DeferredPieces::Part part;
            part.pieces.alloc(n_long);
            DBuf<uint32_t> nfp(n_long), off(n_long);
            hipLaunchKernelGGL(gather_pieces_kernel, grid1(n_long), dim3(WG), 0, stream(), ch_in.pieces.p, lidx.p, n_long, part.pieces.p, nfp.p);
            exclusive_scan_u32(nfp.p, off.p, n_long);
            const size_t n_fp_long = (size_t)download_one(off.p + (n_long - 1)) + (size_t)download_one(nfp.p + (n_long - 1));
            part.fps.alloc(n_fp_long);
            if (defer->n_fp + n_fp_long >= (1ull << 32)) fail(HLMI_EINVAL, "more than 2^32 fixed points in the set-aside alignment pieces");
            hipLaunchKernelGGL(move_fixed_points_kernel, dim3((unsigned)std::min<size_t>(cdiv(n_long, (size_t)WAVES), 256 * 32)), dim3(WG), 0, stream(),
                               part.pieces.p, n_long, off.p, (uint32_t)defer->n_fp, ch_in.fps.p, part.fps.p);
            part.n_pieces = n_long; part.n_fp = n_fp_long; part.fp_base = defer->n_fp;
            defer->n_pieces += n_long; defer->n_fp += n_fp_long;
            defer->parts.push_back(std::move(part));
            hipLaunchKernelGGL(class_flag_kernel, grid1(P0), dim3(WG), 0, stream(), flag.p, P0, (uint8_t)0, nflag.p);
            DBuf<uint32_t> kidx(P0);
            const size_t n_keep = select_flagged_indices(nflag.p, kidx.p, P0);
            kept.pieces.alloc(n_keep ? n_keep : 1);
            if (n_keep) hipLaunchKernelGGL(gather_pieces_kernel, grid1(n_keep), dim3(WG), 0, stream(), ch_in.pieces.p, kidx.p, n_keep, kept.pieces.p,
                                           (uint32_t *)nullptr);
            HIP_CHECK(hipGetLastError());
            sync();
            kept.n_pieces = n_keep; kept.n_fp = ch_in.n_fp - n_fp_long;
            stat_add("align_pieces_deferred", (double)n_long);
            if (!n_keep) return;
            chp = &kept;
        }
    }
    const ChainOut &ch = *chp;
    const FixPt *fps_base = ch_in.fps.p;
    const size_t P = ch.n_pieces;
    size_t span_tasks = 64u << 20;
    if (const char *e = hook("HLMI_ALIGN_SPAN_TASKS")) span_tasks = (size_t)std::max(64, atoi(e));
    const size_t NT = ch.n_fp + P;
    if (NT <= span_tasks) {
        AlignOut ao;
        align_span(in, o, d_qlen, d_tlen, PieceSpan{{ch.pieces.p}, P, ch.n_fp, {fps_base}}, ao);
        if (ao.n_rows) outs.push_back(std::move(ao));
        return;
    }
    DBuf<uint32_t> tcnt(P), toff(P);
    hipLaunchKernelGGL(piece_task_count_kernel, dim3((unsigned)cdiv(P, (size_t)256)), dim3(256), 0, stream(), ch.pieces.p, P, tcnt.p);
    exclusive_scan_u32(tcnt.p, toff.p, P);
    const size_t n_spans = (NT + span_tasks - 1) / span_tasks;
    size_t p0 = 0, t0 = 0;
    for (size_t k = 1; k <= n_spans && p0 < P; ++k) {
        size_t p1 = P, t1 = NT;
        if (k < n_spans) {
            const size_t want = NT / n_spans * k;
            size_t lo = p0 + 1, hi = P;
            while (lo < hi) {
                const size_t mid = (lo + hi) / 2;
                if ((size_t)download_one(toff.p + mid) < want) lo = mid + 1; else hi = mid;
            }
            p1 = lo;
            t1 = p1 < P ? (size_t)download_one(toff.p + p1) : NT;
        }
        AlignOut ao;
        align_span(in, o, d_qlen, d_tlen, PieceSpan{{ch.pieces.p + p0}, p1 - p0, (t1 - t0) - (p1 - p0), {fps_base}}, ao);
        if (ao.n_rows) outs.push_back(std::move(ao));
        p0 = p1; t0 = t1;
    }
    stat_add("align_spans", (double)n_spans);
}
}
```

Before: 3688.

## Compact per-task output to three words and inline single-run CIGARs

Shrinks the per-task TaskOut record from 24 to 12 bytes by packing run count, end op codes and the query-end flag into one meta word. Extension end coordinates move to a separate per-piece ExtEnd array, written only for edge tasks. Tasks with a single CIGAR run keep that run inline instead of taking space in the global run pool, which avoids pool atomics, scatter writes and later indirect reads for the common ungapped case. The cost is extra scattered writes to the ExtEnd array, a 20-bit cap on run count that sets an overflow flag, and a new one-run counter stat.

After: 3703 (median of 6 runs). No clear change (+0.4%).

```diff
diff --git a/hylight_amd/csrc/ava_align.hip b/hylight_amd/csrc/ava_align.hip
--- a/hylight_amd/csrc/ava_align.hip
+++ b/hylight_amd/csrc/ava_align.hip
@@ -4,6 +4,7 @@
 
 #include "ava_internal.h"
 #include "dev_prims.h"
+#include "task_out.h"
 #include "wave_ops.h"
 
 namespace hlmi {
@@ -27,13 +28,7 @@
 };
 constexpr uint16_t TASK_REV = 4;
 constexpr uint16_t TASK_ONE = 8;
-struct TaskOut {
-    int32_t score;
-    int32_t bi, bj;
-    uint32_t runs_off, n_runs;
-    uint32_t pad;
-};
-__device__ __forceinline__ uint32_t end_codes(uint32_t first_run, uint32_t last_run) { return (first_run & 15u) | (last_run & 15u) << 4; }
+struct RunEnds { uint32_t first, last; };
 
 __global__ void piece_task_count_kernel(const Piece *pieces, size_t n, uint32_t *cnt) {
     size_t i = blockIdx.x * (size_t)blockDim.x + threadIdx.x;
@@ -151,6 +146,7 @@
     int trim_ok;
     int kshift;
     TaskOut *out;
+    ExtEnd *ext;
     uint32_t *runs;
     uint32_t cap_runs;
     uint32_t *counters;
@@ -182,6 +178,14 @@
     chunk_left -= n;
     return off;
 }
+__device__ __forceinline__ void runs_fit(const AlignArgs &a, uint32_t n_runs, bool &ok) {
+    if (!task_out_runs_fit(n_runs)) { a.counters[1] = 1; ok = false; }
+}
+__device__ __forceinline__ void put_ext_end(const AlignArgs &a, uint32_t piece, int kind, int bi, int bj) {
+    if (kind == 0) return;
+    int32_t *e = &a.ext[piece].li + (kind == 2 ? 2 : 0);
+    e[0] = bi; e[1] = bj;
+}
 
 __device__ __forceinline__ uint32_t load_codes4(const uint8_t *base, long long idx, long long total) {
     if (idx >= 0 && idx + 4 <= total) {
@@ -212,7 +216,7 @@
 }
 
 
-enum { ST_BASES = 0, ST_BASES_SQUARE, ST_BASES_NARROW, ST_BASES_WIDE, ST_FAST, ST_DP, ST_DP_ROWS, ST_NARROW_SMALL, ST_WIDE_ONE, ST_STUB_EXT, ST_EXT_CERT, ST_EXT_DP_ROW, ST_EXT_DP_K, ST_LONG, ST_BASES_LONG, ST_PACKED, N_ALIGN_STATS };
+enum { ST_BASES = 0, ST_BASES_SQUARE, ST_BASES_NARROW, ST_BASES_WIDE, ST_FAST, ST_DP, ST_DP_ROWS, ST_NARROW_SMALL, ST_WIDE_ONE, ST_STUB_EXT, ST_EXT_CERT, ST_EXT_DP_ROW, ST_EXT_DP_K, ST_LONG, ST_BASES_LONG, ST_PACKED, ST_ONE_RUN, N_ALIGN_STATS };
 constexpr int NR_SMALL = 64;
 constexpr uint8_t CLS_LONG = 5;
 constexpr uint8_t CLS_LONG32 = 7;
@@ -307,6 +311,7 @@
     const size_t n_thr = (size_t)gridDim.x * blockDim.x;
     uint32_t chunk_off = 0, chunk_left = 0;
     uint32_t st[N_ALIGN_STATS] = {};
+    uint32_t n_one_run = 0;
     const size_t n_units = PASS == 1 ? a.n_tasks : (size_t)*a.defer_count;
     const size_t rounds = (n_units + n_thr - 1) / n_thr;
     TaskRef ref_n{0, 0};
@@ -700,8 +705,9 @@
             if (m > prev) runs[nr++] = (uint32_t)(m - prev) << 4 | OP_EQ;
         }
         if (bare) nr = 0;
+        const uint32_t pooled = nr >= 2 ? nr : 0u;
         uint32_t wave_total;
-        const uint32_t mine = wave_excl_sum_u32(nr, lane, wave_total);
+        const uint32_t mine = wave_excl_sum_u32(pooled, lane, wave_total);
         uint32_t base = 0;
         bool ok = true;
         if (wave_total) {
@@ -710,13 +716,15 @@
             ok = __shfl((int)ok, 0, 64) != 0;
         }
         if (fast) {
-            if (ok) for (uint32_t q = 0; q < nr; ++q) a.runs[base + mine + q] = runs[q];
-            const bool ext = (tk.kind & 3) != 0;
+            if (ok) for (uint32_t q = 0; q < pooled; ++q) a.runs[base + mine + q] = runs[q];
             const int L = ext_take >= 0 ? ext_take : (m < n ? m : n);
-            a.out[ti] = TaskOut{fast_score, ext ? L : m, ext ? L : n, base + mine, ok ? nr : 0, (nr ? end_codes(runs[0], runs[nr - 1]) : 0u) | ext_flag};
+            a.out[ti] = task_out(fast_score, base + mine, ok ? nr : 0, nr ? runs[0] : 0u, nr ? runs[nr - 1] : 0u, ext_flag);
+            put_ext_end(a, tk.piece, tk.kind & 3, L, L);
         } else if (live && c == 0) {
-            a.out[ti] = TaskOut{0, 0, 0, 0, 0, 0};
-        }
+            a.out[ti] = task_out(0, 0, 0, 0, 0, 0);
+            put_ext_end(a, tk.piece, tk.kind & 3, 0, 0);
+        }
+        n_one_run += (uint32_t)__popcll(__ballot(fast && nr == 1));
         int m_dp = m;
         if (live && !fast && (c == 1 || c == 3) && a.kmax >= 0 && last_x >= 0 && a.trim_ok && !a.ungapped) {
             const int mn = m < n ? m : n;
@@ -748,6 +756,7 @@
             }
         }
     }
+    st[ST_ONE_RUN] = lane == 0 ? n_one_run : 0u;
 #pragma unroll
     for (int k = 0; k < N_ALIGN_STATS; ++k) {
         unsigned long long v = st[k];
@@ -806,12 +815,12 @@
     int total;
 };
 __device__ uint32_t narrow_walk(const NarrowWalk &w, uint32_t *out, uint32_t total, uint32_t *buf = nullptr, uint32_t cap = 0,
-                                WalkScore *ws = nullptr, uint32_t *ends = nullptr) {
+                                WalkScore *ws = nullptr, RunEnds *ends = nullptr) {
     int i = w.m, j = w.n, state = 0;
     uint32_t cur_op = OP_EQ, cur_len = (uint32_t)w.trim, n_runs = 0, e_first = 0, e_last = 0;
     auto put = [&]() {
-        if (!n_runs) e_first = cur_op;
-        e_last = cur_op;
+        if (!n_runs) e_first = cur_len << 4 | cur_op;
+        e_last = cur_len << 4 | cur_op;
         if (out) out[w.keep_order ? n_runs : total - 1 - n_runs] = cur_len << 4 | cur_op;
         else if (n_runs < cap) buf[n_runs] = cur_len << 4 | cur_op;
         ++n_runs;
@@ -856,7 +865,7 @@
         else { if (cur_len) put(); cur_op = op; cur_len = len; }
     }
     if (cur_len) put();
-    if (ends) *ends = w.keep_order ? end_codes(e_first, e_last) : end_codes(e_last, e_first);
+    if (ends) *ends = w.keep_order ? RunEnds{e_first, e_last} : RunEnds{e_last, e_first};
     return n_runs;
 }
 constexpr int RUN_BUF_NARROW = 48, RUN_BUF_WIDE = 128;
@@ -974,16 +983,17 @@
         uint32_t cp_n = 0, cp_off = 0;
         if (live && l == 0) {
             const NarrowWalk w{&pl[0][0][0], NR_CHUNKS, g * 16, m, n, dlo, NARROW_W - 1, false, tk.trim};
-            uint32_t ends = 0;
+            RunEnds ends{0, 0};
             const uint32_t n_runs = narrow_walk(w, nullptr, 0, rbuf, rcap, nullptr, &ends);
             uint32_t off = 0;
             bool ok = true;
-            if (n_runs) off = pool_take(a, n_runs, chunk_off, chunk_left, ok, RUN_CHUNK_SMALL);
-            if (ok && n_runs) {
+            runs_fit(a, n_runs, ok);
+            if (ok && n_runs >= 2) off = pool_take(a, n_runs, chunk_off, chunk_left, ok, RUN_CHUNK_SMALL);
+            if (ok && n_runs >= 2) {
                 if (n_runs <= rcap) { cp_n = n_runs; cp_off = off; }
                 else narrow_walk(w, a.runs + off, n_runs);
             }
-            a.out[ti] = TaskOut{score, m, n, off, ok ? n_runs : 0, ends};
+            a.out[ti] = task_out(score, off, ok ? n_runs : 0, ends.first, ends.last, 0);
         }
         __builtin_amdgcn_s_waitcnt(0);
         __builtin_amdgcn_wave_barrier();
@@ -1159,7 +1169,7 @@
             const int hf = l & 1;
             if (l < 2 && (hf ? liveB : liveA)) {
                 const Task &t = hf ? tB : tA;
-                a.out[hf ? tiB : tiA] = TaskOut{(hf ? endB : endA) + a.match * t.trim, t.m, t.n, 0, 0, 0};
+                a.out[hf ? tiB : tiA] = task_out((hf ? endB : endA) + a.match * t.trim, 0, 0, 0, 0, 0);
             }
             __builtin_amdgcn_wave_barrier();
             continue;
@@ -1173,17 +1183,18 @@
         if (walker) {
             const NarrowWalk w{&s_pl[wv][0][0][0][0] + hf * (N_PLANES * NR_CHUNKS * 64), NR_CHUNKS, g * 16, wm, wn, wd, NARROW_W - 1, false, wtrim};
             WalkScore ws{a.match, a.mismatch, a.go, a.ge, 0};
-            uint32_t ends = 0;
+            RunEnds ends{0, 0};
             const uint32_t n_runs = narrow_walk(w, nullptr, 0, rbuf, rcap, &ws, &ends);
             uint32_t off = 0;
             bool ok = true;
-            if (n_runs) off = pool_take(a, n_runs, chunk_off, chunk_left, ok, RUN_CHUNK_SMALL);
-            if (ok && n_runs) {
+            runs_fit(a, n_runs, ok);
+            if (ok && n_runs >= 2) off = pool_take(a, n_runs, chunk_off, chunk_left, ok, RUN_CHUNK_SMALL);
+            if (ok && n_runs >= 2) {
                 if (n_runs <= rcap) { cp_n = n_runs; cp_off = off; }
                 else narrow_walk(w, a.runs + off, n_runs);
             }
             const int score = amb ? (hf ? endB : endA) + a.match * wtrim : ws.total;
-            a.out[hf ? tiB : tiA] = TaskOut{score, wm, wn, off, ok ? n_runs : 0, ends};
+            a.out[hf ? tiB : tiA] = task_out(score, off, ok ? n_runs : 0, ends.first, ends.last, 0);
         }
         __builtin_amdgcn_s_waitcnt(0);
         __builtin_amdgcn_wave_barrier();
@@ -1279,13 +1290,13 @@
 
 template <bool TWO>
 __device__ uint32_t wide_walk(const uint32_t *pl, int chunks, int m0, int n0, int dlo, bool keep_order, uint32_t *out, uint32_t total,
-                              uint32_t *buf, uint32_t cap, uint32_t *ends = nullptr, int max_it = 4 * (EXT_MAX + SEQ_T_MAX)) {
+                              uint32_t *buf, uint32_t cap, RunEnds *ends = nullptr, int max_it = 4 * (EXT_MAX + SEQ_T_MAX)) {
     auto word = [&](int plane, int c, int lane) { return pl[(plane * chunks + c) * 64 + lane]; };
     int i = m0, j = n0, state = 0;
     uint32_t cur_op = 0, cur_len = 0, n_runs = 0, e_first = 0, e_last = 0;
     auto put = [&]() {
-        if (!n_runs) e_first = cur_op;
-        e_last = cur_op;
+        if (!n_runs) e_first = cur_len << 4 | cur_op;
+        e_last = cur_len << 4 | cur_op;
         if (out) out[keep_order ? n_runs : total - 1 - n_runs] = cur_len << 4 | cur_op;
         else if (n_runs < cap) buf[n_runs] = cur_len << 4 | cur_op;
         ++n_runs;
@@ -1336,19 +1347,19 @@
         else { if (cur_len) put(); cur_op = op; cur_len = len; }
     }
     if (cur_len) put();
-    if (ends) *ends = keep_order ? end_codes(e_first, e_last) : end_codes(e_last, e_first);
+    if (ends) *ends = keep_order ? RunEnds{e_first, e_last} : RunEnds{e_last, e_first};
     return n_runs;
 }
 
 template <bool TWO, int W = BAND_W>
 __device__ uint32_t long_walk(const uint32_t *pl, int chunks, int m0, int n0, int dlo, bool keep_order, uint32_t *buf, uint32_t cap,
-                              uint32_t *ends, int max_it) {
+                              RunEnds *ends, int max_it) {
     auto word = [&](int plane, int c, int lane) { return pl[((size_t)plane * chunks + c) * W + lane]; };
     int i = m0, j = n0, state = 0;
     uint32_t cur_op = 0, cur_len = 0, n_runs = 0, e_first = 0, e_last = 0;
     auto put = [&]() {
-        if (!n_runs) e_first = cur_op;
-        e_last = cur_op;
+        if (!n_runs) e_first = cur_len << 4 | cur_op;
+        e_last = cur_len << 4 | cur_op;
         if (n_runs < cap) buf[n_runs] = cur_len << 4 | cur_op;
         ++n_runs;
     };
@@ -1403,7 +1414,7 @@
         else { if (cur_len) put(); cur_op = op; cur_len = len; }
     }
     if (cur_len) put();
-    if (ends) *ends = keep_order ? end_codes(e_first, e_last) : end_codes(e_last, e_first);
+    if (ends) *ends = keep_order ? RunEnds{e_first, e_last} : RunEnds{e_last, e_first};
     return n_runs;
 }
 
@@ -1426,11 +1437,11 @@
         const Task tk = a.tasks[ti];
         const int n = tk.n, dlo = tk.dlo;
         const int m = tk.m < n - dlo ? tk.m : n - dlo;
+        const int kind = tk.kind & 3;
         if (m <= 0 || n <= 0) {
-            if (lane == 0) a.out[ti] = TaskOut{0, 0, 0, 0, 0, 0};
+            if (lane == 0) { a.out[ti] = task_out(0, 0, 0, 0, 0, 0); put_ext_end(a, tk.piece, kind, 0, 0); }
             continue;
         }
-        const int kind = tk.kind & 3;
         bool ambig = false;
         {
             const bool rev = (tk.kind & TASK_REV) != 0, left = kind == 1;
@@ -1487,7 +1498,10 @@
         __builtin_amdgcn_s_waitcnt(0);
         __builtin_amdgcn_wave_barrier();
         if constexpr (!TB) {
-            if (lane == 0) a.out[ti] = TaskOut{score, ei, ej, 0, 0, kind != 0 && ei == end_row ? 0x80000000u : 0u};
+            if (lane == 0) {
+                a.out[ti] = task_out(score, 0, 0, 0, 0, kind != 0 && ei == end_row ? TASK_OUT_QEND : 0u);
+                put_ext_end(a, tk.piece, kind, ei, ej);
+            }
             continue;
         }
         uint32_t *rbuf = s_runs[wv];
@@ -1495,18 +1509,20 @@
         uint32_t cp_n = 0, cp_off = 0;
         if (lane == 0) {
             const uint32_t *planes = &pl[0][0][0];
-            uint32_t ends = 0;
+            RunEnds ends{0, 0};
             const uint32_t n_runs = two ? wide_walk<true>(planes, W_CHUNKS, ei, ej, dlo, kind == 1, nullptr, 0, rbuf, rcap, &ends)
                                         : wide_walk<false>(planes, W_CHUNKS, ei, ej, dlo, kind == 1, nullptr, 0, rbuf, rcap, &ends);
             uint32_t off = 0;
             bool ok = true;
-            if (n_runs) off = pool_take(a, n_runs, chunk_off, chunk_left, ok);
-            if (ok && n_runs) {
+            runs_fit(a, n_runs, ok);
+            if (ok && n_runs >= 2) off = pool_take(a, n_runs, chunk_off, chunk_left, ok);
+            if (ok && n_runs >= 2) {
                 if (n_runs <= rcap) { cp_n = n_runs; cp_off = off; }
                 else if (two) wide_walk<true>(planes, W_CHUNKS, ei, ej, dlo, kind == 1, a.runs + off, n_runs, nullptr, 0);
                 else wide_walk<false>(planes, W_CHUNKS, ei, ej, dlo, kind == 1, a.runs + off, n_runs, nullptr, 0);
             }
-            a.out[ti] = TaskOut{score, ei, ej, off, ok ? n_runs : 0, ends | (kind != 0 && ei == end_row ? 0x80000000u : 0u)};
+            a.out[ti] = task_out(score, off, ok ? n_runs : 0, ends.first, ends.last, kind != 0 && ei == end_row ? TASK_OUT_QEND : 0u);
+            put_ext_end(a, tk.piece, kind, ei, ej);
         }
         __builtin_amdgcn_s_waitcnt(0);
         __builtin_amdgcn_wave_barrier();
@@ -1556,7 +1572,8 @@
         const int chunks = (m + 31) >> 5;
         if (m <= 0 || n <= 0 || (TB && ((uint32_t)chunks > la.chunks_cap || (uint32_t)(m + n + 2) > la.runs_cap))) {
             if (lane == 0) {
-                a.out[ti] = TaskOut{0, 0, 0, 0, 0, 0};
+                a.out[ti] = task_out(0, 0, 0, 0, 0, 0);
+                put_ext_end(a, tk.piece, kind, 0, 0);
                 if (m > 0 && n > 0) *la.too_long = 1;
             }
             continue;
@@ -1692,17 +1709,21 @@
         const uint32_t flag = ext && ei == end_row ? 0x80000000u : 0u;
         if (lane == 0) atomicAdd(la.rows_run, (unsigned long long)rows_done);
         if constexpr (!TB) {
-            if (lane == 0) a.out[ti] = TaskOut{score, ei, ej, 0, 0, flag};
+            if (lane == 0) { a.out[ti] = task_out(score, 0, 0, 0, 0, flag); put_ext_end(a, tk.piece, kind, ei, ej); }
             continue;
         } else {
             __threadfence_block();
             __builtin_amdgcn_wave_barrier();
-            uint32_t n_runs = 0, off = 0, ends = 0;
+            uint32_t n_runs = 0, off = 0;
+            RunEnds ends{0, 0};
             bool ok = true;
             if (lane == 0) {
                 n_runs = long_walk<TWO>(pl, chunks, ei, ej, dlo, left, rs, la.runs_cap, &ends, 2 * (m + n) + 8);
-                if (n_runs) off = pool_take(a, n_runs, chunk_off, chunk_left, ok);
-                a.out[ti] = TaskOut{score, ei, ej, off, ok ? n_runs : 0, ends | flag};
+                runs_fit(a, n_runs, ok);
+                if (ok && n_runs >= 2) off = pool_take(a, n_runs, chunk_off, chunk_left, ok);
+                a.out[ti] = task_out(score, off, ok ? n_runs : 0, ends.first, ends.last, flag);
+                put_ext_end(a, tk.piece, kind, ei, ej);
+                if (n_runs < 2) n_runs = 0;
             }
             __threadfence_block();
             __builtin_amdgcn_wave_barrier();
@@ -1769,7 +1790,8 @@
         const int chunks = (m + 31) >> 5;
         if (live && (m <= 0 || n <= 0 || (TB && ((uint32_t)chunks > la.chunks_cap || (uint32_t)(m + n + 2) > la.runs_cap)))) {
             if (hl == 0) {
-                a.out[ti] = TaskOut{0, 0, 0, 0, 0, 0};
+                a.out[ti] = task_out(0, 0, 0, 0, 0, 0);
+                put_ext_end(a, tk.piece, kind, 0, 0);
                 if (m > 0 && n > 0) *la.too_long = 1;
             }
             live = false;
@@ -1923,17 +1945,21 @@
         const uint32_t flag = ext && ei == end_row ? 0x80000000u : 0u;
         if (live && hl == 0) atomicAdd(la.rows_run, (unsigned long long)m);
         if constexpr (!TB) {
-            if (live && hl == 0) a.out[ti] = TaskOut{score, ei, ej, 0, 0, flag};
+            if (live && hl == 0) { a.out[ti] = task_out(score, 0, 0, 0, 0, flag); put_ext_end(a, tk.piece, kind, ei, ej); }
             continue;
         } else {
             __threadfence_block();
             __builtin_amdgcn_wave_barrier();
-            uint32_t n_runs = 0, off = 0, ends = 0;
+            uint32_t n_runs = 0, off = 0;
+            RunEnds ends{0, 0};
             bool ok = true;
             if (live && hl == 0) {
                 n_runs = long_walk<TWO, HALF_W>(pl, chunks, ei, ej, dlo, left, rs, la.runs_cap, &ends, 2 * (m0 + n) + 8);
-                if (n_runs) off = pool_take(a, n_runs, chunk_off, chunk_left, ok);
-                a.out[ti] = TaskOut{score, ei, ej, off, ok ? n_runs : 0, ends | flag};
+                runs_fit(a, n_runs, ok);
+                if (ok && n_runs >= 2) off = pool_take(a, n_runs, chunk_off, chunk_left, ok);
+                a.out[ti] = task_out(score, off, ok ? n_runs : 0, ends.first, ends.last, flag);
+                put_ext_end(a, tk.piece, kind, ei, ej);
+                if (n_runs < 2) n_runs = 0;
             }
             __threadfence_block();
             __builtin_amdgcn_wave_barrier();
@@ -1991,8 +2017,9 @@
         const int out_score = ext ? best_s : score;
         uint32_t n_runs = ext ? nr_best : nr, last_op = ext ? last_op_best : (uint32_t)cur;
         if (!TB || take == 0) n_runs = 0;
+        const uint32_t pooled = n_runs >= 2 ? n_runs : 0u;
         uint32_t wave_total;
-        const uint32_t mine = wave_excl_sum_u32(n_runs, lane, wave_total);
+        const uint32_t mine = wave_excl_sum_u32(pooled, lane, wave_total);
         uint32_t base = 0;
         bool ok = true;
         if (wave_total) {
@@ -2000,7 +2027,8 @@
             base = (uint32_t)__shfl((int)base, 0, 64);
             ok = __shfl((int)ok, 0, 64) != 0;
         }
-        if (live && ok && n_runs) {
+        runs_fit(a, n_runs, ok);
+        if (live && ok && pooled) {
             uint32_t k = 0, len = 0;
             int op_cur = -1;
             uint32_t *dst = a.runs + base + mine;
@@ -2018,9 +2046,10 @@
             if (len) put();
         }
         if (live) {
-            const uint32_t ends = n_runs ? (left ? end_codes(last_op, first_op) : end_codes(first_op, last_op)) : 0u;
-            a.out[ti] = TaskOut{out_score, ext ? take : (int)tk.m, ext ? take : (int)tk.n, base + mine, ok ? n_runs : 0,
-                                ends | (ext && take == end_row ? 0x80000000u : 0u)};
+            const uint32_t lone = (uint32_t)take << 4;
+            a.out[ti] = task_out(out_score, base + mine, ok ? n_runs : 0, lone | (left ? last_op : first_op), lone | (left ? first_op : last_op),
+                                 ext && take == end_row ? TASK_OUT_QEND : 0u);
+            put_ext_end(a, tk.piece, kind, take, take);
         }
     }
 }
@@ -2030,6 +2059,7 @@
     const FixPt *fps;
     const uint32_t *task_off;
     const TaskOut *tout;
+    const ExtEnd *ext;
     const uint32_t *runs;
     size_t n_pieces;
     const uint32_t *qlen, *tlen, *rank_q, *rank_t, *chunk_of_t;
@@ -2067,25 +2097,28 @@
         uint32_t carry_code = 99;
         constexpr uint32_t NO_SLOT = 0xffffffffu;
         uint32_t open_idx = NO_SLOT, open_val = 0;
-        int ext_l_i = 0, ext_l_j = 0, ext_r_i = 0, ext_r_j = 0;
-        TaskOut r_next{0, 0, 0, 0, 0, 0};
+        bool keep_l = false, keep_r = false;
+        TaskOut r_next{0, 0, 0};
         if ((uint32_t)lane < n_tasks) r_next = to[lane];
         for (uint32_t t0 = 0; t0 < n_tasks; t0 += 64) {
             const uint32_t t = t0 + (uint32_t)lane;
             TaskOut r = r_next;
-            r_next = TaskOut{0, 0, 0, 0, 0, 0};
+            r_next = TaskOut{0, 0, 0};
             if (t + 64 < n_tasks) r_next = to[t + 64];
             bool keep = false;
             if (t < n_tasks) {
                 keep = true;
                 if (t == 0 || t == n_tasks - 1)
-                    keep = !(r.score + ((r.pad & 0x80000000u) ? a.end_bonus : 0) <= 0 || (r.n_runs == 0 && !bare));
-            }
-            if (keep && t == 0) { ext_l_i = r.bi; ext_l_j = r.bj; }
-            if (keep && t == n_tasks - 1 && t != 0) { ext_r_i = r.bi; ext_r_j = r.bj; }
+                    keep = !(r.score + (task_out_qend(r) ? a.end_bonus : 0) <= 0 || (task_out_n_runs(r) == 0 && !bare));
+            }
+            if (WRITE) {
+                const unsigned long long kept = __ballot(keep);
+                if (t0 == 0) keep_l = (kept & 1ull) != 0;
+                if (t0 + 64 >= n_tasks && n_tasks > 1) keep_r = (kept >> ((n_tasks - 1) & 63u) & 1ull) != 0;
+            }
             long long sc = keep ? r.score : 0;
-            const uint32_t nr = keep && !bare ? r.n_runs : 0;
-            const uint32_t first = r.pad & 15u, last = (r.pad >> 4) & 15u;
+            const uint32_t nr = keep && !bare ? task_out_n_runs(r) : 0;
+            const uint32_t first = task_out_first_code(r), last = task_out_last_code(r);
             const unsigned long long ne_mask = __ballot(nr != 0);
             const unsigned long long below = ne_mask & ((1ull << lane) - 1ull);
             const int prev_lane = below ? 63 - __clzll((long long)below) : 0;
@@ -2096,11 +2129,11 @@
             const uint32_t S = wave_excl_sum_u32(nr, lane, tot_runs);
             const uint32_t Mx = wave_excl_sum_u32(mrg ? 1u : 0u, lane, tot_mrg);
             if (WRITE) {
-                const uint32_t F = nr ? a.runs[r.runs_off] : 0u;
-                const uint32_t L = nr >= 2 ? a.runs[r.runs_off + nr - 1] : F;
+                const uint32_t F = nr >= 2 ? a.runs[r.runs] : (nr ? r.runs : 0u);
+                const uint32_t L = nr >= 2 ? a.runs[r.runs + nr - 1] : F;
                 uint32_t mid[ASM_MID];
 #pragma unroll
-                for (uint32_t u = 0; u < ASM_MID; ++u) mid[u] = u + 3 <= nr ? a.runs[r.runs_off + 1 + u] : 0u;
+                for (uint32_t u = 0; u < ASM_MID; ++u) mid[u] = u + 3 <= nr ? a.runs[r.runs + 1 + u] : 0u;
                 const uint32_t P = wave_prefix_sum_incl_dpp(mrg ? F >> 4 : 0u);
                 const bool opens = nr != 0 && (!mrg || nr >= 2);
                 const unsigned long long om = __ballot(opens);
@@ -2138,7 +2171,7 @@
                             put(base + 1 + u, mid[u]);
                         }
                     for (uint32_t x = 1 + ASM_MID; x + 1 < nr; ++x) {
-                        const uint32_t run = a.runs[r.runs_off + x];
+                        const uint32_t run = a.runs[r.runs + x];
                         blen += run >> 4;
                         if ((run & 15u) == OP_EQ) nmatch += run >> 4;
                         put(base + x, run);
@@ -2159,9 +2192,6 @@
             for (int o = 32; o > 0; o >>= 1) sc += __shfl_xor(sc, o, 64);
             score += sc;
         }
-        const int li = __shfl(ext_l_i, 0, 64), lj = __shfl(ext_l_j, 0, 64);
-        const int last_lane = (int)((n_tasks - 1) & 63u);
-        const int ri = __shfl(ext_r_i, last_lane, 64), rj = __shfl(ext_r_j, last_lane, 64);
         if (!WRITE) {
             if (lane == 0) {
                 const bool ok = (slots > 0 || bare) && score >= a.min_dp_score;
@@ -2175,6 +2205,8 @@
         for (int o = 32; o > 0; o >>= 1) { nmatch += __shfl_xor(nmatch, o, 64); blen += __shfl_xor(blen, o, 64); }
         if (lane == 0) {
             if (open_idx != NO_SLOT) w[open_idx] = open_val;
+            const ExtEnd e = a.ext[i];
+            const int li = keep_l ? e.li : 0, lj = keep_l ? e.lj : 0, ri = keep_r ? e.ri : 0, rj = keep_r ? e.rj : 0;
             const int qs = (int)fp[0].q - li, ts = (int)fp[0].t - lj;
             const int qe = (int)fp[p.n_fp - 1].q + ri, te = (int)fp[p.n_fp - 1].t + rj;
             const uint32_t ql = a.qlen[p.q];
@@ -2213,19 +2245,19 @@
     uint32_t slots = 0;
     uint32_t pend = 0;
     uint32_t carry_code = 99;
-    int li = 0, lj = 0, ri = 0, rj = 0;
+    bool keep_l = false, keep_r = false;
     for (uint32_t t = 0; t < n_tasks; ++t) {
         const TaskOut r = to[t];
         bool keep = true;
         if (t == 0 || t == n_tasks - 1)
-            keep = !(r.score + ((r.pad & 0x80000000u) ? a.end_bonus : 0) <= 0 || (r.n_runs == 0 && !bare));
+            keep = !(r.score + (task_out_qend(r) ? a.end_bonus : 0) <= 0 || (task_out_n_runs(r) == 0 && !bare));
         if (!keep) continue;
-        if (t == 0) { li = r.bi; lj = r.bj; }
-        else if (t == n_tasks - 1) { ri = r.bi; rj = r.bj; }
+        if (t == 0) keep_l = true;
+        else if (t == n_tasks - 1) keep_r = true;
         score += r.score;
-        const uint32_t nr = bare ? 0u : r.n_runs;
+        const uint32_t nr = bare ? 0u : task_out_n_runs(r);
         if (!nr) continue;
-        const uint32_t first = r.pad & 15u, last = (r.pad >> 4) & 15u;
+        const uint32_t first = task_out_first_code(r), last = task_out_last_code(r);
         const bool mrg = first == carry_code;
         carry_code = last;
         if (!WRITE) {
@@ -2233,7 +2265,7 @@
             continue;
         }
         for (uint32_t x = 0; x < nr; ++x) {
-            const uint32_t run = a.runs[r.runs_off + x];
+            const uint32_t run = nr == 1 ? r.runs : a.runs[r.runs + x];
             blen += run >> 4;
             if ((run & 15u) == OP_EQ) nmatch += run >> 4;
             if (x == 0 && mrg) pend += (run >> 4) << 4;
@@ -2251,6 +2283,8 @@
         return;
     }
     if (pend) w[slots++] = pend;
+    const ExtEnd e = a.ext[i];
+    const int li = keep_l ? e.li : 0, lj = keep_l ? e.lj : 0, ri = keep_r ? e.ri : 0, rj = keep_r ? e.rj : 0;
     const int qs = (int)fp[0].q - li, ts = (int)fp[0].t - lj;
     const int qe = (int)fp[p.n_fp - 1].q + ri, te = (int)fp[p.n_fp - 1].t + rj;
     const uint32_t ql = a.qlen[p.q];
@@ -2412,6 +2446,8 @@
                        ch.pieces.p, toff.p, P, d_qlen, d_tlen, in.Q->off.p, in.T->off.p, ch.fps.p, o.stub_oh, ext_rows(o), task_ref.p, pgeom.p);
     HIP_CHECK(hipGetLastError());
     DBuf<TaskOut> tout(NT);
+    DBuf<ExtEnd> ext_end(P);
+    ext_end.zero();
     DBuf<uint32_t> counters(2);
     DBuf<unsigned long long> astats(N_ALIGN_STATS);
     constexpr size_t MAX_BLOCKS = 256 * 16;
@@ -2420,7 +2456,7 @@
     size_t run_share = std::max<size_t>(NT * 12, 1 << 16);
     DBuf<uint32_t> runs;
     AsmArgs as{};
-    as.pieces = ch.pieces.p; as.fps = ch.fps.p; as.task_off = toff.p; as.tout = tout.p; as.n_pieces = P;
+    as.pieces = ch.pieces.p; as.fps = ch.fps.p; as.task_off = toff.p; as.tout = tout.p; as.ext = ext_end.p; as.n_pieces = P;
     as.min_dp_score = o.min_dp_score; as.end_bonus = o.end_bonus;
     as.qlen = d_qlen; as.tlen = d_tlen; as.rank_q = in.d_rank_q; as.rank_t = in.d_rank_t; as.chunk_of_t = in.d_chunk_of_t;
     as.pg = pgeom.p; as.stub_score = o.min_dp_score + std::max(0, o.end_bonus);
@@ -2536,7 +2572,7 @@
             for (int k = 1; k <= 2; ++k)
                 if (sane && o.end_bonus > 0 && k * U < G && k * U < o.end_bonus + o.match && k * U < 2 * G + o.match) aa.kext_bonus = k;
         }
-        aa.out = tout.p; aa.runs = runs.p; aa.cap_runs = (uint32_t)cap_runs; aa.counters = counters.p;
+        aa.out = tout.p; aa.ext = ext_end.p; aa.runs = runs.p; aa.cap_runs = (uint32_t)cap_runs; aa.counters = counters.p;
         as.runs = runs.p;
         aa.run_buf_cap = 0xffffffffu;
         if (const char *e = hook("HLMI_RUN_BUF_CAP")) aa.run_buf_cap = (uint32_t)std::max(0, atoi(e));
@@ -2839,6 +2875,7 @@
     {
         std::vector<unsigned long long> h = astats.download(N_ALIGN_STATS);
         stat_add("align_tasks_fast", (double)h[ST_FAST]);
+        stat_add("align_tasks_one_run", (double)h[ST_ONE_RUN]);
         stat_add("align_tasks_packed", (double)h[ST_PACKED]);
         stat_add("align_tasks_dp", (double)h[ST_DP]);
         stat_add("align_dp_rows", (double)h[ST_DP_ROWS]);
diff --git a/hylight_amd/csrc/task_out.h b/hylight_amd/csrc/task_out.h
--- /dev/null
+++ b/hylight_amd/csrc/task_out.h
@@ -0,0 +1,36 @@
+#pragma once
+
+#include <cstdint>
+
+#include "hd.h"
+
+namespace hlmi {
+
+struct TaskOut {
+    int32_t score;
+    uint32_t runs;
+    uint32_t meta;
+};
+static_assert(sizeof(TaskOut) == 12, "TaskOut is three words");
+
+constexpr uint32_t TASK_OUT_RUNS_BITS = 20;
+constexpr uint32_t TASK_OUT_RUNS_MAX = (1u << TASK_OUT_RUNS_BITS) - 1u;
+constexpr uint32_t TASK_OUT_QEND = 0x80000000u;
+
+HLMI_HD TaskOut task_out(int32_t score, uint32_t pool_off, uint32_t n_runs, uint32_t first_run, uint32_t last_run, uint32_t flag) {
+    TaskOut r;
+    r.score = score;
+    r.runs = n_runs == 1 ? first_run : (n_runs ? pool_off : 0u);
+    r.meta = n_runs | (n_runs ? (first_run & 15u) << 20 | (last_run & 15u) << 24 : 0u) | (flag & TASK_OUT_QEND);
+    return r;
+}
+HLMI_HD bool task_out_runs_fit(uint32_t n_runs) { return n_runs <= TASK_OUT_RUNS_MAX; }
+HLMI_HD uint32_t task_out_n_runs(const TaskOut &r) { return r.meta & TASK_OUT_RUNS_MAX; }
+HLMI_HD uint32_t task_out_first_code(const TaskOut &r) { return r.meta >> 20 & 15u; }
+HLMI_HD uint32_t task_out_last_code(const TaskOut &r) { return r.meta >> 24 & 15u; }
+HLMI_HD bool task_out_qend(const TaskOut &r) { return (r.meta & TASK_OUT_QEND) != 0; }
+
+struct ExtEnd { int32_t li, lj, ri, rj; };
+static_assert(sizeof(ExtEnd) == 16, "ExtEnd is four words");
+
+}
```
